# ltronchin/LatentAugment

Hardware: AMD Instinct MI355X
Metric: augmented images/sec (256^2, 20 latent steps) (higher is better)
Workload: dtype f32 (scaled split-fp16x2 on fp16 MFMA, fp32 accumulate); 1 GPU; SG2 config-f 256x256 2-ch, random-init G, batch=8/GPU, 20 latent steps; global_batch=8, parallelism=dp1

## Files before the change

### include/latentaug_hip.h

```cpp
#ifndef LATENTAUG_HIP_H
#define LATENTAUG_HIP_H

#include <stddef.h>

#ifdef __cplusplus
extern "C" {
#endif

#ifndef LA_STREAM_T
#define LA_STREAM_T
typedef struct ihipStream_t* la_stream_t;
#endif

#define LA_OK 0
#define LA_ERR_ARG (-1)
#define LA_ERR_HIP (-2)
#define LA_ERR_WORKSPACE (-3)

#define LA_ACT_LINEAR 1
#define LA_ACT_RELU 2
#define LA_ACT_LRELU 3

const char* la_last_error(void);
int la_abi_version(void);


int la_bias_act_f32(const float* x, const float* b, float* y, long n, long stepb, int nb, int act, float alpha,
                    float gain, float clamp, la_stream_t stream);

int la_bias_act_grad_f32(const float* dy, const float* yref, float* dx, float* db, long n, long stepb, int nb, int act,
                         float alpha, float gain, float clamp, la_stream_t stream);

int la_bias_act_ex_f32(const float* x, const float* b, const float* xref, const float* yref, const float* dy, float* out, long n,
                       long stepb, int nb, int grad, int act, float alpha, float gain, float clamp, la_stream_t stream);
int la_bias_sum_f32(const float* dx, float* db, long n, long stepb, int nb, la_stream_t stream);
int la_bias_act_ex_f16(const unsigned short* x, const unsigned short* b, const unsigned short* xref, const unsigned short* yref,
                       const unsigned short* dy, unsigned short* out, long n, long stepb, int nb, int grad, int act, float alpha, float gain,
                       float clamp, la_stream_t stream);
int la_bias_sum_f16(const unsigned short* dx, unsigned short* db, long n, long stepb, int nb, la_stream_t stream);
int la_bias_act_ex_f64(const double* x, const double* b, const double* xref, const double* yref, const double* dy, double* out, long n,
                       long stepb, int nb, int grad, int act, double alpha, double gain, double clamp, la_stream_t stream);
int la_bias_sum_f64(const double* dx, double* db, long n, long stepb, int nb, la_stream_t stream);

int la_upfirdn2d_out_size(int in_size, int up, int down, int pad0, int pad1, int taps);
int la_upfirdn2d_f32(const float* x, const float* f_host, float* y, int N, int C, int H, int W, int fh, int fw, int upx,
                     int upy, int downx, int downy, int padx0, int padx1, int pady0, int pady1, int flip, float gain,
                     la_stream_t stream);
int la_upfirdn2d_f16(const unsigned short* x, const float* f_host, unsigned short* y, int N, int C, int H, int W, int fh, int fw,
                     int upx, int upy, int downx, int downy, int padx0, int padx1, int pady0, int pady1, int flip, float gain,
                     la_stream_t stream);
int la_upfirdn2d_f64(const double* x, const float* f_host, double* y, int N, int C, int H, int W, int fh, int fw, int upx, int upy,
                     int downx, int downy, int padx0, int padx1, int pady0, int pady1, int flip, double gain, la_stream_t stream);

int la_filtered_lrelu_f32(const float* x, const float* fu, const float* fd, const float* b, const unsigned char* si, unsigned char* so,
                          float* y, int N, int C, int H, int W, int fu_h, int fu_w, int fd_h, int fd_w, int up, int down, int px0, int px1,
                          int py0, int py1, int sx, int sy, float gain, float slope, float clamp, int flip, int write_signs,
                          la_stream_t stream);
int la_filtered_lrelu_act_f32(float* x, const unsigned char* si, unsigned char* so, int N, int C, int H, int W, int sx, int sy, float gain,
                              float slope, float clamp, int write_signs, la_stream_t stream);
int la_filtered_lrelu_out_size(int in_size, int up, int down, int pad0, int pad1, int fu_taps, int fd_taps);
int la_filtered_lrelu_sign_shape(int H, int W, int fu_h, int fu_w, int fd_h, int fd_w, int up, int down, int px0, int px1, int py0, int py1,
                                 int* rows, int* row_bytes);


int la_conv2d_f32(const float* x, const float* w, float* y, void* ws, size_t ws_bytes, int B, int Cin, int H, int W, int Cout, int kh, int kw,
                  int Hout, int Wout, int stride, int pady, int padx, int groups, int flip_weight, int transpose, la_stream_t stream);
int la_conv2d_wgrad_f32(const float* x, const float* dy, float* dw, void* ws, size_t ws_bytes, int B, int Cin, int H, int W, int Cout,
                        int kh, int kw, int Hout, int Wout, int stride, int pady, int padx, int groups, int flip_weight, int transpose,
                        la_stream_t stream);
size_t la_conv2d_workspace_bytes(int op, int B, int Cin, int H, int W, int Cout, int kh, int kw, int Hout, int Wout, int stride, int groups,
                                 int transpose);
int la_conv2d_uses_engine(int op, int cout, int kh, int kw, int stride, int groups);
int la_conv2d_wgrad_slices(int B, int Cin, int H, int W, int Cout, int kh, int kw, int Hout, int Wout, int stride, int groups, int transpose);


int la_grid_sample_f32(const float* x, const float* grid, float* y, int N, int C, int H, int W, int Ho, int Wo, la_stream_t stream);
int la_grid_sample_f16(const unsigned short* x, const unsigned short* grid, unsigned short* y, int N, int C, int H, int W, int Ho, int Wo,
                       la_stream_t stream);
int la_grid_sample_f64(const double* x, const double* grid, double* y, int N, int C, int H, int W, int Ho, int Wo, la_stream_t stream);
int la_grid_sample_grad_f32(const float* dy, const float* x, const float* grid, float* dx, float* dgrid, int N, int C, int H, int W, int Ho,
                            int Wo, la_stream_t stream);
int la_grid_sample_grad_f16(const unsigned short* dy, const unsigned short* x, const unsigned short* grid, unsigned short* dx,
                            unsigned short* dgrid, float* ws, int N, int C, int H, int W, int Ho, int Wo, la_stream_t stream);
int la_grid_sample_grad_f64(const double* dy, const double* x, const double* grid, double* dx, double* dgrid, int N, int C, int H, int W,
                            int Ho, int Wo, la_stream_t stream);
long la_grid_sample_grad_workspace_floats(int N, int C, int H, int W);

int la_fma_f32(const float* a, const float* b, const float* c, float* y, const long* shape_host, const long* astride_host,
               const long* bstride_host, const long* cstride_host, la_stream_t stream);
int la_unbroadcast_sum_f32(const float* x, float* out, const long* shape_host, const long* out_shape_host, la_stream_t stream);


int la_pack_conv_weights_f32(const float* w, float* wf, float* wb, float* wsq, int cout, int cin, int ktaps,
                             la_stream_t stream);

int la_modconv3x3_fwd_f32(const float* x, long x_bstride, const float* wf, const void* wq, int precision, const float* s, int s_stride, const float* d,
                          int d_stride, const float* noise, long noise_bstride, float noise_strength, const float* bias,
                          int act, float alpha, float gain, float clamp, float* y, void* ws, size_t ws_bytes, int B, int cin, int cout, int res,
                          la_stream_t stream);

int la_modconv3x3_up2_fwd_f32(const float* x, long x_bstride, const float* wf, const void* wq, int precision, const float* s, int s_stride,
                              const float* d, int d_stride, const float* noise, long noise_bstride, float noise_strength,
                              const float* bias, int act, float alpha, float gain, float clamp, const float* fir_host,
                              float* scratch, float* y, void* ws, size_t ws_bytes, int B, int cin, int cout, int res, la_stream_t stream);

int la_modconv3x3_bwd_f32(const float* gz, const float* wb, const void* wq, int precision, const float* s, int s_stride, const float* xin,
                          long xin_bstride, float* gx, float* ds_part, void* ws, size_t ws_bytes, int B, int cin, int cout, int res,
                          la_stream_t stream);
int la_modconv3x3_up2_bwd_f32(const float* gz, const float* wb, const void* wq, int precision, const float* s, int s_stride, const float* xin,
                              long xin_bstride, const float* fir_host, float* scratch, float* gx, float* ds_part, void* ws, size_t ws_bytes, int B,
                              int cin, int cout, int res, la_stream_t stream);
int la_modconv_ds_tiles(int grid_res);
size_t la_modconv_workspace_bytes(int B, int cin, int cout, int res, int up);
#define LA_PREC_F32 0
#define LA_PREC_BF16X3 1
#define LA_PREC_BF16X2 2
#define LA_PREC_F16X2 3
size_t la_modconv_bf16_pack_bytes(int cin, int cout, int transpose, int nterm);
int la_pack_conv_weights_bf16_f32(const float* w, void* out, int cout, int cin, int ktaps, int transpose, int nterm,
                                  la_stream_t stream);


long la_pairwise_l2_workspace_floats(int n, long m);
int la_pairwise_l2_f32(const float* X, int n, const float* Y, long m, long K, float* D, float* mean_out,
                       float* workspace, la_stream_t stream);

int la_center_crop_f32(const float* src, float* dst, long planes, int R, int cc, int off, la_stream_t stream);

int la_adam_step_f32(float* p, const float* g, float* m, float* v, long n, int step, float lr, float beta1, float beta2,
                     float eps, la_stream_t stream);

int la_noise_normal_f32(float* out, long rows, long row_elems, unsigned long long seed, unsigned layer, long row0, la_stream_t stream);


int la_noise_uniform_f32(float* out, long rows, long row_elems, unsigned long long seed, unsigned stream_id, long row0, la_stream_t stream);

int la_elastic_field_f32(const float* noise, const float* taps_host, int ntaps, float alpha_x, float alpha_y, float* disp, float* ws, int B, int H,
                         int W, la_stream_t stream);

int la_warp_affine_f32(const float* x, const float* minv, const unsigned char* apply, float* y, int B, int C, int H, int W, int mode,
                       la_stream_t stream);

int la_warp_elastic_f32(const float* x, const float* disp, const unsigned char* apply, float* y, int B, int C, int H, int W, int mode,
                        la_stream_t stream);

typedef struct la_synth la_synth;
int la_synth_num_ws(int img_resolution);
int la_synth_num_params(int img_resolution);
size_t la_synth_workspace_bytes(int img_resolution, int img_channels, int w_dim, const int* channels, int max_batch);
int la_synth_create(int img_resolution, int img_channels, int w_dim, const int* channels, float conv_clamp,
                    const float* const* params, int nparams, const float* noise_strength_host, int nlayers,
                    const float* fir_host, int fir_h, int fir_w, int max_batch, void* workspace, size_t workspace_bytes,
                    la_stream_t stream, la_synth** out);
void la_synth_destroy(la_synth* h);
int la_synth_set_precision(la_synth* h, int precision);
int la_synth_set_operand_scale(la_synth* h, int from_data);
int la_synth_set_row_window(la_synth* h, int row_lo, int row_hi);
int la_synth_set_col_window(la_synth* h, int col_lo, int col_hi);
int la_synth_get_precision(const la_synth* h);
int la_synth_forward(la_synth* h, const float* ws, long ws_bstride, long ws_lstride, int B, int noise_mode,
                     const float* const* noises, float* img_out, la_stream_t stream);
int la_synth_backward(la_synth* h, const float* g_img, float* dws, la_stream_t stream);
const float* la_synth_image(const la_synth* h);
const float* la_synth_block_image(const la_synth* h, int block);
const float* la_synth_layer_output(const la_synth* h, int layer);
const float* la_synth_styles(const la_synth* h);
const float* la_synth_style_grads(const la_synth* h);
int la_synth_style_rows(const la_synth* h);

int la_fc_f32(const float* x, const float* W, const float* bias, float* y, int B, int in, int out, float lr_mul, int act,
              float alpha, float gain, la_stream_t stream);
int la_mapping_forward_f32(const float* z, int B, int z_dim, int w_dim, int num_layers, const float* const* weights,
                           const float* const* biases, float lr_mul, const float* w_avg, float truncation_psi,
                           int num_ws, float* tmp, float* ws_out, la_stream_t stream);

typedef struct la_disc la_disc;
int la_disc_num_params(int img_resolution);
size_t la_disc_workspace_bytes(int img_resolution, int img_channels, const int* channels, int max_batch);
int la_disc_create(int img_resolution, int img_channels, const int* channels, float conv_clamp, const float* const* params,
                   int nparams, const float* fir_host, int mbstd_group_size, int max_batch, void* workspace,
                   size_t workspace_bytes, la_stream_t stream, la_disc** out);
void la_disc_destroy(la_disc* h);
int la_disc_set_precision(la_disc* h, int precision);
int la_disc_forward(la_disc* h, const float* img, int B, la_stream_t stream);
int la_disc_loss(la_disc* h, float w_disc, int norm_batch, float* loss_out, la_stream_t stream);
int la_disc_backward(la_disc* h, const float* dlogits, float* g_img, int accumulate, la_stream_t stream);
const float* la_disc_logits(const la_disc* h);

#define LA_FEAT_CONV_RELU 0
#define LA_FEAT_TAP 1
#define LA_FEAT_MAXPOOL2 2
#define LA_FEAT_AVGPOOL2 3
#define LA_FEAT_FC_RELU 4
#define LA_FEAT_FC 5
typedef struct la_feat_op { int kind, cin, cout; } la_feat_op;
typedef struct la_feat la_feat;
size_t la_feat_workspace_bytes(int nops, const la_feat_op* ops, int in_ch, int in_res, int max_batch);
int la_feat_create(int nops, const la_feat_op* ops, const float* const* params, int nparams, int in_ch, int in_res,
                   int max_batch, void* workspace, size_t workspace_bytes, la_stream_t stream, la_feat** out);
void la_feat_destroy(la_feat* h);
int la_feat_num_features(const la_feat* h);
int la_feat_set_precision(la_feat* h, int precision);
int la_feat_forward(la_feat* h, const float* x, int N, float* feat_out, la_stream_t stream);
int la_feat_backward(la_feat* h, const float* gfeat, float* gx, la_stream_t stream);
int la_crop_repeat_f32(const float* img, float* xc, int B, int imgc, int R, int S, int y0, int x0, int rep, float scale,
                       float shift, la_stream_t stream);
int la_crop_repeat_grad_f32(const float* gxc, float* g_img, int B, int imgc, int R, int S, int y0, int x0, int rep,
                            float scale, la_stream_t stream);

#define LA_DET_AREA 0
#define LA_DET_BILINEAR 1
int la_detector_prep_f32(const float* img, float* out, int N, int C, int H, int W, int S, int rep, int mode, int quantize,
                         const float* scale, const float* shift, la_stream_t stream);
size_t la_fc_workspace_bytes(long N, long K, long O);
int la_fc_bias_act_f32(const float* x, const float* w, const float* b, float* y, long N, long K, long O, int act,
                       void* workspace, size_t workspace_bytes, la_stream_t stream);

typedef struct la_opt_config {
    int steps;
    float lr;
    float beta1, beta2, eps;
    float w_latent, w_pix, w_disc, w_lpips;
    int criterion_mode;
    int soft_aug;
    float alpha;
    int loop_noise_mode;
    int final_noise_mode;
    int norm_batch;
    int crop, crop_off;
} la_opt_config;
typedef struct la_latent_opt la_latent_opt;
size_t la_latent_opt_workspace_bytes(int img_resolution, int img_channels, int w_dim, const la_opt_config* cfg, long Mw,
                                     long Mx, int max_batch);
int la_latent_opt_create(la_synth* g, int img_resolution, int img_channels, int w_dim, const la_opt_config* cfg,
                         const float* bankW, long Mw, const float* bankXc, long Mx, int max_batch, void* workspace,
                         size_t workspace_bytes, la_latent_opt** out);
size_t la_latent_opt_workspace_bytes_ex(int img_resolution, int img_channels, int w_dim, const la_opt_config* cfg, long Mw,
                                        long Mx, int max_batch, int latent_space);
int la_latent_opt_create_ex(la_synth* g, int img_resolution, int img_channels, int w_dim, const la_opt_config* cfg,
                            const float* bankW, long Mw, const float* bankXc, long Mx, int max_batch, int latent_space,
                            void* workspace, size_t workspace_bytes, la_latent_opt** out);
void la_latent_opt_destroy(la_latent_opt* h);
int la_latent_opt_set_disc(la_latent_opt* h, la_disc* d);
size_t la_latent_opt_lpips_workspace_bytes(int img_channels, int F, int S, long Mf, int max_batch);
int la_latent_opt_set_lpips(la_latent_opt* h, la_feat* f, const float* bankF, long Mf, int S, float pre_scale,
                            float pre_shift, void* ws, size_t ws_bytes);
int la_latent_opt_set_lpips_preproc(la_latent_opt* h, const float* scale, const float* shift, int n);
int la_latent_opt_set_crop_pos(la_latent_opt* h, int x, int y);
int la_latent_opt_set_graph(la_latent_opt* h, int enable);
int la_latent_opt_graph_state(const la_latent_opt* h);
int la_latent_opt_set_trace(la_latent_opt* h, float* w_trace, float* img_trace);
int la_latent_opt_set_grad_trace(la_latent_opt* h, float* dw_trace);
int la_latent_opt_set_overlap(la_latent_opt* h, int enable);
int la_latent_opt_set_row_window(la_latent_opt* h, int row_lo, int row_hi);
int la_latent_opt_set_col_window(la_latent_opt* h, int col_lo, int col_hi);
int la_latent_opt_set_time_trace(la_latent_opt* h, int enable);
int la_latent_opt_get_times(la_latent_opt* h, float* ms);
int la_latent_opt_invalidate_banks(la_latent_opt* h);
int la_latent_opt_run(la_latent_opt* h, const float* w0, int B, const float* const* final_noises, float* img_out,
                      float* w_aug_out, float* losses_out, la_stream_t stream);

int la_feature_moments_f64(const float* x, long n, int D, double* raw_mean, double* raw_cov, la_stream_t stream);
size_t la_pr_workspace_floats(long nr, long nc);
int la_cdist_f16(const void* rows, long nr, const void* cols, long nc, int D, float* dist, float* ws, la_stream_t stream);
int la_pr_kth_f16(const void* rows, long nr, const void* cols, long nc, int D, int nhood_size, float* kth, float* ws,
                  la_stream_t stream);
int la_pr_member_f16(const void* rows, long nr, const void* cols, long nc, int D, const float* radius, unsigned char* member,
                     float* ws, la_stream_t stream);

size_t la_kid_workspace_bytes(long S, long mx, long my);
int la_kid_poly3_f32(const float* x, long nx, const float* y, long ny, int D, const int* ix, const int* iy, long S, long mx, long my,
                     double* sums, double* mmd2, double* kid, void* ws, size_t ws_bytes, la_stream_t stream);

size_t la_dc_workspace_bytes(long ng, long nr);
int la_dc_col_splits(long ng, long nr);
int la_dc_count_f16(const void* gen, long ng, const void* real, long nr, int D, const float* radius, int* count, float* nearest,
                    void* ws, size_t ws_bytes, la_stream_t stream);

int la_prof_begin(void);
int la_prof_end(double* total_ms, long* launches, double* flops, double* bytes);
int la_prof_set_stride(int stride);
long la_prof_total_launches(void);
int la_prof_num_classes(void);
int la_prof_end_classes(double* ms, long* launches, double* flops, double* bytes, int nclass);

#ifdef __cplusplus
}
#endif
#endif
```

### latentaugment_amd/csrc/la_conv.h

```cpp
#pragma once
#include <stddef.h>
#include <string.h>

#include "la_common.h"
#include "la_launch_args.h"

#define LA_EPI_RAW 0
#define LA_EPI_FWD 1
#define LA_EPI_BWD 2
#define LA_CONV_MAX_TAPS 9
#define LA_CONV_MAX_PHASES 4
#define LA_CONV_PHASE_TAPS 4

struct LaRgbFuse {
    int imgc;
    const float* w; const float* s; int s_stride; const float* bias; const float* skip;
    float* rgb_pre; float* img; float clamp;
};
struct LaSeamFuse {
    const float* demod; int demod_stride;
    const float* bias;
    const float* noise; long noise_bstride; float noise_strength;
    int act; float alpha, gain, clamp;
    float* ddn_part;
    float* pmax;
    float* xs_out;
    float xs_mult;
    int imgc;
    const float* g_img; const float* rgb_pre; float rgb_clamp;
    const float* wrgb; const float* s_rgb; int s_rgb_stride;
    float* dweff_part;
};

struct LaConvArgs {
    const float* in;
    const float* wgt;
    float* out;
    const float* in_scale;
    long in_bstride;
    int scale_stride;
    const float* in_mask_y;
    int in_mask_act; float in_mask_alpha, in_mask_gain, in_mask_clamp;
    float in_gain;
    int B, C, M, Hin, Win, Hout, Wout;
    int Gy, Gx;
    int in_sy, in_sx;
    int out_sy, out_sx, out_oy, out_ox;
    int out_pitch; long out_plane;
    int ntaps;
    int tap_dy[LA_CONV_MAX_TAPS], tap_dx[LA_CONV_MAX_TAPS], tap_w[LA_CONV_MAX_TAPS];
    int epi;
    const float* demod;
    int demod_stride;
    const float* noise;
    long noise_bstride;
    float noise_strength;
    const float* bias;
    int act;
    float alpha, gain, clamp;
    const float* addend;
    float* out2;
    float* fwd_xs_out;
    const float* fwd_xs_mult;
    const float* out_scale;
    int oscale_stride;
    const float* xin;
    long xin_bstride;
    float* ds_part;
    int tiles_per_sample;
    LaSeamFuse seam;
    LaRgbFuse rgb;
    void* ws;
    size_t ws_bytes;
    float* splitk_ws;
    int ksplit;
    const float* in_pmax;
    int in_pmax_nseg;
    const void* in_q;
    int precision;
    const void* wgt_bf16;
    long wgt_bf16_term_elems;
    const float* acc_scale_x;
    int acc_scale_fan;
    const float* acc_scale_w;
    int row_lo, row_hi;
    int col_lo, col_hi;
    int in_row_lo, in_row_hi;
#ifdef LA_DEV
    int dbg_stamp;
#endif
    int nphase;
    struct Phase {
        int Gy, Gx, out_oy, out_ox, ntaps; int tap_dy[LA_CONV_PHASE_TAPS], tap_dx[LA_CONV_PHASE_TAPS], tap_w[LA_CONV_PHASE_TAPS];
        int tile0;
        long ws_off;
    } ph[LA_CONV_MAX_PHASES];
};
static_assert(sizeof(LaConvArgs) == 1096 && offsetof(LaConvArgs, seam) == 416 && offsetof(LaConvArgs, rgb) == 568 && offsetof(LaConvArgs, ws) == 640,
              "LaConvArgs: an embedded record moved a kernel-parameter field");

static inline void la_conv_args_init(LaConvArgs& a) {
    memset(&a, 0, sizeof(a));
    a.in_sy = a.in_sx = a.out_sy = a.out_sx = 1;
    a.clamp = -1.f; a.gain = 1.f; a.act = LA_ACT_LINEAR;
}
static inline void la_conv_taps_kxk(LaConvArgs& a, int k, bool backward) {
    a.ntaps = k * k;
    for (int t = 0; t < a.ntaps; ++t) {
        const int dy = t / k - k / 2, dx = t % k - k / 2;
        a.tap_dy[t] = backward ? -dy : dy; a.tap_dx[t] = backward ? -dx : dx; a.tap_w[t] = t;
    }
}
static inline void la_conv_taps_3x3(LaConvArgs& a, bool backward) { la_conv_taps_kxk(a, 3, backward); }
static inline void la_conv_taps_3x3_corner(LaConvArgs& a) {
    a.ntaps = 9;
    for (int t = 0; t < 9; ++t) { a.tap_dy[t] = t / 3; a.tap_dx[t] = t % 3; a.tap_w[t] = t; }
}
static inline void la_conv_up2_phase(LaConvArgs& a, int hin, int py, int px, int ox_step, bool merged) {
    a.out_oy = py; a.out_ox = px * ox_step;
    a.Gy = py ? hin : hin + 1; a.Gx = px ? hin : hin + 1;
    int nt = 0;
    for (int ky = py; ky < 3; ky += 2)
        for (int kx = px; kx < 3; kx += 2) { a.tap_dy[nt] = -(ky / 2); a.tap_dx[nt] = -(kx / 2); a.tap_w[nt] = ky * 3 + kx; ++nt; }
    a.ntaps = nt;
    if (!merged) return;
    LaConvArgs::Phase& P = a.ph[a.nphase++];
    P.Gy = a.Gy; P.Gx = a.Gx; P.out_oy = py; P.out_ox = a.out_ox; P.ntaps = nt;
    for (int t = 0; t < nt; ++t) { P.tap_dy[t] = a.tap_dy[t]; P.tap_dx[t] = a.tap_dx[t]; P.tap_w[t] = a.tap_w[t]; }
}

int la_conv_flat_launch(const LaConvArgs& as, int MTsel, dim3 grid, bool split, hipStream_t stream);
int la_conv_halo_launch(const LaConvArgs& as, int MTsel, dim3 grid, hipStream_t stream);

long la_conv_bf16_pack_elems(int M, int C, int ktaps);
int la_pack_conv_weights_bf16(const float* w, void* out, int cout, int cin, int ktaps, int transpose, int nterm,
                              hipStream_t stream, float scale = 1.f, int m_pad = 0);
int la_conv_bf16_dispatch(const LaConvArgs& as, int MTsel, dim3 grid, bool split, hipStream_t stream);

long la_conv_splitk_floats(int B, int M, int C, int Gy, int Gx, int precision);
long la_conv_splitk_floats_phases(int B, int M, int C, int nphase, const int* Gy, const int* Gx, int precision);
size_t la_conv_presplit_bytes(int B, int C, int Hin, int Win);
size_t la_conv_split_pack_bytes(int M, int C, int ktaps);
int la_conv_prepare_input(LaConvArgs& a, hipStream_t stream);
int la_conv_act_grad_segments(long HW);
int la_conv_act_grad_pmax(const float* dy, const float* yref, float* dx, float* pm, int B, int C, long HW, int act, float alpha, float gain,
                          float clamp, hipStream_t stream);
int la_conv_xscale_from_pmax(const float* pmax, int nseg, const float* scale, int scale_stride, float mult, float* xscale, int B, int C,
                             hipStream_t stream);
int la_absmax_bits(const float* w, long n, unsigned* amax_bits, hipStream_t stream);
bool la_conv_bf16_uses_halo(const LaConvArgs& a);

int la_conv_tiles_per_sample(int Gy, int Gx);
int la_conv_launch(const LaConvArgs& a, hipStream_t stream);
```

### latentaugment_amd/csrc/la_conv.hip

```cpp
#include "la_conv.h"
#include <stdlib.h>
#include "la_conv_device.h"
#include <type_traits>

#define KC 16

int la_conv_tiles_per_sample(int Gy, int Gx) { return la_cdiv((long)Gy * Gx, NT); }

#define SPLITK_MAX_G 1156
static int choose_ksplit(bool bf, long tiles, int nck, float taps, double out_bytes) {
    int ks;
    if (bf) {
        float best = 1e30f;
        ks = 1;
        for (int k = 1; k <= nck && k <= 16; ++k) {
            const int per = la_cdiv(nck, k);
            const int kk = la_cdiv(nck, per);
            if (kk != k) continue;
            const float slots = (float)(tiles * kk) / 512.f;
            const float rounds = slots <= 1.f ? 1.f : slots;
            float cost = rounds * ((float)per * taps * 1.7f + 10.f);
            if (kk > 1) cost += 5.f + (float)((kk + 1) * out_bytes / 3.5e6);
            if (cost < best - 1e-3f) { best = cost; ks = kk; }
        }
        return ks;
    }
    ks = la_cdiv(768, tiles);
    if (ks > nck) ks = nck;
    if (ks < 2) return 1;
    const int per = la_cdiv(nck, ks);
    return la_cdiv(nck, per);
}

long la_conv_splitk_floats_phases(int B, int M, int C, int nphase, const int* Gy, const int* Gx, int precision) {
    const bool bf = precision != LA_PREC_F32;
    const int nck = la_cdiv(C, bf ? 32 : KC);
    if (nck < 2 || nphase < 1 || (nphase > 1 && !bf)) return 0;
    const int mtiles = la_cdiv(M, M >= 128 ? 128 : 64);
    long tiles = 0, Gsum = 0;
    for (int p = 0; p < nphase; ++p) {
        const long G = (long)Gy[p] * Gx[p];
        if (G > SPLITK_MAX_G) return 0;
        tiles += la_cdiv((long)B * G, NT);
        Gsum += G;
    }
    int ks = choose_ksplit(bf, tiles * mtiles, nck, nphase > 1 ? 2.25f : 9.f, 4.0 * B * M * (double)Gsum);
    const int ks1 = choose_ksplit(bf, tiles * mtiles, nck, 1.f, 4.0 * B * M * (double)Gsum);
    if (ks1 > ks) ks = ks1;
    return ks >= 2 ? (long)ks * B * M * Gsum : 0;
}
long la_conv_splitk_floats(int B, int M, int C, int Gy, int Gx, int precision) {
    return la_conv_splitk_floats_phases(B, M, C, 1, &Gy, &Gx, precision);
}

template <int MT, bool SPLIT>
__global__ __launch_bounds__(256) void la_conv_igemm_kernel(LaConvArgs a) {
    constexpr int TM = MT / 64;
    constexpr int A_F4 = (KC * MT / 4) / 256;
    __shared__ __attribute__((aligned(16))) float As[2][KC][MT];
    __shared__ __attribute__((aligned(16))) float Bs[2][KC][NT];
    __shared__ float red[4][MT];

    const int tid = threadIdx.x;
    const int lane = tid & 63, wid = tid >> 6;
    const int wm = wid >> 1, wn = wid & 1;
    int ntile = blockIdx.x;
    if (!SPLIT && (gridDim.x & 7) == 0) ntile = (blockIdx.x & 7) * (gridDim.x >> 3) + (blockIdx.x >> 3);
    const int m0 = blockIdx.y * MT;
    const int G = a.Gy * a.Gx;
    const int Ntot = SPLIT ? a.B * G : G;

    const int n_l = tid & (NT - 1);
    const int khalf = tid >> 7;
    const int nidx_l = ntile * NT + n_l;
    const bool nvalid = nidx_l < Ntot;
    int b_l = SPLIT ? (nvalid ? nidx_l / G : 0) : (int)blockIdx.z;
    const int g_l = SPLIT ? nidx_l - b_l * G : nidx_l;
    const int gy_l = nvalid ? g_l / a.Gx : 0;
    const int gx_l = nvalid ? g_l - gy_l * a.Gx : 0;
    const int iy0 = gy_l * a.in_sy, ix0 = gx_l * a.in_sx;
    const long HWin = (long)a.Hin * a.Win;
    const float* in_b = a.in + (long)b_l * a.in_bstride;
    const float* sc_b = a.in_scale ? a.in_scale + (long)b_l * a.scale_stride : nullptr;

    const int nck = (a.C + KC - 1) / KC;
    int ck_beg = 0, ck_end = nck;
    if (SPLIT) {
        const int per = (nck + a.ksplit - 1) / a.ksplit;
        ck_beg = blockIdx.z * per;
        ck_end = ck_beg + per < nck ? ck_beg + per : nck;
    }
    const int ci_beg = ck_beg * a.ntaps, ci_end = ck_end * a.ntaps;

    float breg[KC / 2];
    float4 areg[A_F4];

    auto prefetch = [&](int ci) {
        const int cc = ci / a.ntaps;
        const int t = ci - cc * a.ntaps;
        const int c0 = cc * KC;
        const int iy = iy0 + a.tap_dy[t], ix = ix0 + a.tap_dx[t];
        const bool ok = nvalid && iy >= 0 && iy < a.Hin && ix >= 0 && ix < a.Win;
        const long off = (long)iy * a.Win + ix;
#pragma unroll
        for (int j = 0; j < KC / 2; ++j) {
            const int c = c0 + khalf + 2 * j;
            float v = 0.f;
            if (ok && c < a.C) {
                v = in_b[(long)c * HWin + off];
                if (sc_b) v *= sc_b[c];
            }
            breg[j] = v;
        }
        const float* wslab = a.wgt + (long)a.tap_w[t] * a.C * a.M;
#pragma unroll
        for (int j = 0; j < A_F4; ++j) {
            const int idx = tid + 256 * j;
            const int row = idx / (MT / 4), col = (idx - row * (MT / 4)) * 4;
            const int c = c0 + row, m = m0 + col;
            float4 v = make_float4(0.f, 0.f, 0.f, 0.f);
            if (c < a.C && m < a.M) v = *reinterpret_cast<const float4*>(wslab + (long)c * a.M + m);
            areg[j] = v;
        }
    };
    auto stage = [&](int buf) {
#pragma unroll
        for (int j = 0; j < KC / 2; ++j) Bs[buf][khalf + 2 * j][n_l] = breg[j];
#pragma unroll
        for (int j = 0; j < A_F4; ++j) {
            const int idx = tid + 256 * j;
            const int row = idx / (MT / 4), col = (idx - row * (MT / 4)) * 4;
            *reinterpret_cast<float4*>(&As[buf][row][col]) = areg[j];
        }
    };

    f32x16 acc[TM][2];
#pragma unroll
    for (int i = 0; i < TM; ++i)
#pragma unroll
        for (int j = 0; j < 2; ++j)
#pragma unroll
            for (int r = 0; r < 16; ++r) acc[i][j][r] = 0.f;

    const int l31 = lane & 31, lh = lane >> 5;
    if (ci_beg < ci_end) {
        prefetch(ci_beg);
        stage(0);
    }
    __syncthreads();
    for (int ci = ci_beg; ci < ci_end; ++ci) {
        const int buf = (ci - ci_beg) & 1;
        if (ci + 1 < ci_end) prefetch(ci + 1);
#pragma unroll
        for (int kp = 0; kp < KC / 2; ++kp) {
            float av[TM], bv[2];
#pragma unroll
            for (int i = 0; i < TM; ++i) av[i] = As[buf][2 * kp + lh][wm * (MT / 2) + i * 32 + l31];
#pragma unroll
            for (int j = 0; j < 2; ++j) bv[j] = Bs[buf][2 * kp + lh][wn * 64 + j * 32 + l31];
#pragma unroll
            for (int i = 0; i < TM; ++i)
#pragma unroll
                for (int j = 0; j < 2; ++j)
                    acc[i][j] = __builtin_amdgcn_mfma_f32_32x32x2f32(av[i], bv[j], acc[i][j], 0, 0, 0);
        }
        if (ci + 1 < ci_end) stage(buf ^ 1);
        __syncthreads();
    }

    la_conv_epilogue<MT, SPLIT>(a, acc, red, ntile, m0, G, Ntot);
}

template <int PPB>
__global__ __launch_bounds__(256) void la_conv_splitk_finish_kernel(LaConvArgs a_in) {
    __shared__ float wpart[4];
    LaConvArgs a = a_in;
    if (a_in.nphase > 0) {
        const LaConvArgs::Phase& P = a_in.ph[blockIdx.z];
        a.Gy = P.Gy; a.Gx = P.Gx; a.out_oy = P.out_oy; a.out_ox = P.out_ox;
        a.splitk_ws = a_in.splitk_ws + P.ws_off;
    }
    constexpr int T = 256 / PPB;
    const int lane = threadIdx.x & 63;
    const int tp = threadIdx.x % T;
    const int m = blockIdx.x * PPB + threadIdx.x / T;
    const int b = blockIdx.y;
    const bool live = m < a.M;
    if (!live && PPB > 1) return;
    const int G = a.Gy * a.Gx;
    const int wpitch = (a.epi == LA_EPI_RAW && a.out_pitch > 0) ? a.out_pitch : a.Wout;
    const long HWout = (a.epi == LA_EPI_RAW && a.out_plane > 0) ? a.out_plane : (long)a.Hout * a.Wout;
    const long slice = (long)a.B * a.M * G;
    const float* wsp = a.splitk_ws + ((long)b * a.M + m) * G;
    float* out_p = a.out + ((long)b * a.M + m) * HWout;
    const float dmv = (a.epi == LA_EPI_FWD && a.demod) ? a.demod[(long)b * a.demod_stride + m] : 1.f;
    const float bv = (a.epi == LA_EPI_FWD && a.bias) ? a.bias[m] : 0.f;
    const float sc = (a.epi == LA_EPI_BWD && a.out_scale) ? a.out_scale[(long)b * a.oscale_stride + m] : 1.f;
    const float* xin_p = (a.epi == LA_EPI_BWD && a.xin) ? a.xin + (long)b * a.xin_bstride + (long)m * HWout : nullptr;
    const bool seam = a.epi == LA_EPI_BWD && a.seam.ddn_part != nullptr && xin_p != nullptr;
    const float dm0 = (seam && a.seam.demod) ? a.seam.demod[(long)b * a.seam.demod_stride + m] : 1.f;
    const float b0 = (seam && a.seam.bias) ? a.seam.bias[m] : 0.f;
    float part = 0.f, dd = 0.f, mx = 0.f;
    float* xs_row = (seam && a.seam.xs_out && lane == 0 && (PPB > 1 || threadIdx.x == 0)) ? a.seam.xs_out + (long)b * LA_XS_FAN + la_xs_sub((int)(threadIdx.x >> 6) * 5) : nullptr;
    float ymax = 0.f;
    if (a.epi == LA_EPI_FWD && a.fwd_xs_out && lane == 0) xs_row = a.fwd_xs_out + (long)b * LA_XS_FAN + la_xs_sub((int)(threadIdx.x >> 6) * 5);
    const float xs_seen = xs_row ? la_xs_peek(xs_row) : 0.f;
    const int imgc = seam ? (a.seam.imgc < 4 ? a.seam.imgc : 4) : 0;
    float we[4] = {0.f, 0.f, 0.f, 0.f}, dwe[4] = {0.f, 0.f, 0.f, 0.f};
    for (int c = 0; c < imgc; ++c) we[c] = a.seam.wrgb[(long)c * a.M + m] * a.seam.s_rgb[(long)b * a.seam.s_rgb_stride + m];
    auto run = [&](auto vec_tag) {
        constexpr int VEC = decltype(vec_tag)::value;
        typedef float vf __attribute__((ext_vector_type(VEC)));
        auto ld = [](const float* p) { return *reinterpret_cast<const vf*>(p); };
        for (int g = tp * VEC; g < G; g += T * VEC) {
            auto add = [](vf& s, const vf& p) {
#pragma unroll
                for (int e = 0; e < VEC; ++e) s[e] += p[e];
            };
            vf acc = ld(wsp + g);
            int k = 1;
            for (; k + 7 < a.ksplit; k += 8) {
                vf p[8];
#pragma unroll
                for (int u = 0; u < 8; ++u) p[u] = ld(wsp + (long)(k + u) * slice + g);
#pragma unroll
                for (int u = 0; u < 8; ++u) add(acc, p[u]);
            }
            if (k + 3 < a.ksplit) {
                vf p[4];
#pragma unroll
                for (int u = 0; u < 4; ++u) p[u] = ld(wsp + (long)(k + u) * slice + g);
#pragma unroll
                for (int u = 0; u < 4; ++u) add(acc, p[u]);
                k += 4;
            }
            for (; k < a.ksplit; ++k) { const vf p = ld(wsp + (long)k * slice + g); add(acc, p); }
            const int gy = g / a.Gx, gx = g - gy * a.Gx;
            const long pos = (long)(gy * a.out_sy + a.out_oy) * wpitch + gx * a.out_sx + a.out_ox;
            float v[VEC];
#pragma unroll
            for (int e = 0; e < VEC; ++e) v[e] = VEC == 1 ? acc[0] : acc[e];
            if (a.epi == LA_EPI_FWD) {
                vf nz = 0.f;
                if (a.noise) nz = ld(a.noise + (long)b * a.noise_bstride + pos);
#pragma unroll
                for (int e = 0; e < VEC; ++e) v[e] = la_conv_epi_fwd(a, v[e], dmv, nz[e] * a.noise_strength, bv);
                if (a.out2) {
                    const long o2 = ((long)b * a.M + m) * HWout + pos;
                    vf ad = 0.f;
                    if (a.addend) ad = ld(a.addend + o2);
                    vf w;
#pragma unroll
                    for (int e = 0; e < VEC; ++e) { w[e] = v[e] + ad[e]; ymax = fmaxf(ymax, fabsf(w[e])); }
                    *reinterpret_cast<vf*>(a.out2 + o2) = w;
                } else {
#pragma unroll
                    for (int e = 0; e < VEC; ++e) ymax = fmaxf(ymax, fabsf(v[e]));
                }
            } else if (a.epi == LA_EPI_BWD) {
                vf y = 0.f;
                if (xin_p) y = ld(xin_p + pos);
                vf gv[4], nz0 = 0.f;
#pragma unroll
                for (int c = 0; c < 4; ++c) {
                    gv[c] = 0.f;
                    if (c < imgc) {
                        const long o = ((long)b * imgc + c) * HWout + pos;
                        gv[c] = ld(a.seam.g_img + o);
                        if (a.seam.rgb_clamp >= 0.f) {
                            const vf pre = ld(a.seam.rgb_pre + o);
#pragma unroll
                            for (int e = 0; e < VEC; ++e) if (fabsf(pre[e]) > a.seam.rgb_clamp) gv[c][e] = 0.f;
                        }
                    }
                }
                if (seam && a.seam.noise) {
                    nz0 = ld(a.seam.noise + (long)b * a.seam.noise_bstride + pos);
#pragma unroll
                    for (int e = 0; e < VEC; ++e) nz0[e] *= a.seam.noise_strength;
                }
#pragma unroll
                for (int e = 0; e < VEC; ++e) {
                    part += v[e] * y[e];
                    v[e] *= sc;
#pragma unroll
                    for (int c = 0; c < 4; ++c)
                        if (c < imgc) { v[e] += we[c] * gv[c][e]; dwe[c] += gv[c][e] * y[e]; }
                    if (seam) {
                        const float g1 = v[e] * la_act_bwd_from_y(y[e], a.seam.act, a.seam.alpha, a.seam.gain, a.seam.clamp);
                        dd += g1 * (la_act_inv(y[e], a.seam.act, a.seam.alpha, a.seam.gain) - b0 - nz0[e]);
                        v[e] = g1 * dm0;
                        mx = fmaxf(mx, fabsf(v[e]));
                    }
                }
            }
            vf w;
#pragma unroll
            for (int e = 0; e < VEC; ++e) w[e] = v[e];
            *reinterpret_cast<vf*>(out_p + pos) = w;
        }
    };
    {
        size_t al = (size_t)a.splitk_ws | (size_t)a.out | (size_t)a.out2 | (size_t)a.addend | (size_t)a.noise | (size_t)a.xin;
        if (seam) al |= (size_t)a.seam.noise | (size_t)(imgc ? a.seam.g_img : nullptr) | (size_t)(imgc ? a.seam.rgb_pre : nullptr);
        const bool vec4 = a.out_sx == 1 && ((a.Gx | wpitch | a.out_ox) & 3) == 0 && ((HWout | a.noise_bstride | a.seam.noise_bstride | a.xin_bstride) & 3) == 0 &&
                          (al & 15) == 0 && (a_in.nphase == 0 || (a_in.ph[blockIdx.z].ws_off & 3) == 0);
        if (vec4) run(std::integral_constant<int, 4>{});
        else run(std::integral_constant<int, 1>{});
    }
    if (a.epi == LA_EPI_FWD && a.fwd_xs_out) {
#pragma unroll
        for (int o = 32; o > 0; o >>= 1) ymax = fmaxf(ymax, __shfl_xor(ymax, o, 64));
// ... 175 lines not shown
```

### latentaugment_amd/csrc/la_latent_opt.hip

```cpp
#include "la_common.h"

#include <math.h>
#include <stdlib.h>
#include <string.h>

#include "la_conv.h"
#include "la_criteria.h"
#include "la_feat.h"

struct la_latent_opt {
    la_synth* g;
    la_disc* d;
    la_opt_config cfg;
    int R, imgc, wdim, num_ws, maxB;
    int wplus;
    const float* bankW; long Mw;
    const float* bankX; long Mx;
    float *w_opt, *m, *v, *dw, *dws, *g_img, *colsumW, *colsumX, *yx, *yy, *xx, *xc, *losses;
    int colsums_valid;
    la_feat* f;
    const float* bankF; long Mf; int F, S, crop_x, crop_y;
    float pre_scale[4], pre_shift[4];
    float *l_xc, *l_feat, *l_gfeat, *l_gxc, *l_colsum, *l_yx, *l_yy, *l_xx;
    int l_colsum_valid;
    float* adam_tab;
    float* adam_tab_host;
    int adam_tab_valid;
    int* step_ctr;
    int* crop_dev;
    float* trace_dw;
    int graph_mode;
    int graph_B;
    int graph_win;
    int graph_refused;
    hipGraph_t graph;
    hipGraphExec_t graph_exec;
    hipGraph_t seg_graph[4];
    hipGraphExec_t seg_exec[4];
    int seg_valid;
    hipStream_t cap_stream;
    float* trace_w;
    float* trace_img;
    int wcol_lo, wcol_hi;
    int win_lo, win_hi;
    int overlap;
    hipStream_t side_stream;
    hipEvent_t ev_fork, ev_join;
    int time_trace, tev_steps;
    hipEvent_t* tev;
};
#define LA_TEV 7

static size_t carve(la_latent_opt* h, char* base) {
    LaCarver c{base};
    const size_t B = h->maxB, wd = h->wdim, cc2 = (size_t)h->cfg.crop * h->cfg.crop;
    const size_t wl = h->wplus ? (size_t)h->num_ws * wd : wd;
    h->w_opt = c.take(B * wl); h->m = c.take(B * wl); h->v = c.take(B * wl); h->dw = c.take(B * wl);
    h->dws = c.take(B * h->num_ws * wd);
    h->g_img = c.take(B * h->imgc * (size_t)h->R * h->R);
    h->colsumW = c.take((size_t)h->num_ws * wd);
    h->colsumX = c.take((size_t)h->imgc * cc2);
    const size_t mm = (size_t)(h->Mw > h->Mx ? h->Mw : h->Mx);
    h->yx = c.take(LA_YX_FLOATS(mm ? mm : 1, B)); h->yy = c.take(LA_YY_FLOATS(mm ? mm : 1)); h->xx = c.take(LA_XX_FLOATS(B));
    h->xc = c.take(B * h->imgc * cc2);
    h->losses = c.take((size_t)(h->cfg.steps > 0 ? h->cfg.steps : 1) * 4);
    h->adam_tab = c.take((size_t)(h->cfg.steps > 0 ? h->cfg.steps : 1) * 2);
    h->step_ctr = reinterpret_cast<int*>(c.take(16));
    h->crop_dev = h->step_ctr + 4;
    return c.off;
}

static size_t carve_lpips(la_latent_opt* h, char* base) {
    LaCarver c{base};
    const size_t n = (size_t)h->imgc * h->maxB;
    h->l_xc = c.take(n * 3 * h->S * h->S); h->l_gxc = c.take(n * 3 * h->S * h->S);
    h->l_feat = c.take(n * h->F); h->l_gfeat = c.take(n * h->F);
    h->l_colsum = c.take((size_t)h->imgc * h->F);
    h->l_yx = c.take(LA_YX_FLOATS(h->Mf, h->maxB)); h->l_yy = c.take(LA_YY_FLOATS(h->Mf)); h->l_xx = c.take(LA_XX_FLOATS(h->maxB));
    return c.off;
}

extern "C" size_t la_latent_opt_workspace_bytes_ex(int img_resolution, int img_channels, int w_dim, const la_opt_config* cfg,
                                                   long Mw, long Mx, int max_batch, int latent_space) {
    if (!cfg || (latent_space != 0 && latent_space != 1)) return 0;
    la_latent_opt h; memset(&h, 0, sizeof(h));
    h.cfg = *cfg; h.R = img_resolution; h.imgc = img_channels; h.wdim = w_dim; h.num_ws = la_synth_num_ws(img_resolution);
    h.maxB = max_batch; h.Mw = Mw; h.Mx = Mx; h.wplus = latent_space;
    return carve(&h, nullptr);
}

extern "C" size_t la_latent_opt_workspace_bytes(int img_resolution, int img_channels, int w_dim, const la_opt_config* cfg,
                                                long Mw, long Mx, int max_batch) {
    return la_latent_opt_workspace_bytes_ex(img_resolution, img_channels, w_dim, cfg, Mw, Mx, max_batch, 0);
}

extern "C" int la_latent_opt_create(la_synth* g, int img_resolution, int img_channels, int w_dim, const la_opt_config* cfg,
                                    const float* bankW, long Mw, const float* bankXc, long Mx, int max_batch,
                                    void* workspace, size_t workspace_bytes, la_latent_opt** out) {
    return la_latent_opt_create_ex(g, img_resolution, img_channels, w_dim, cfg, bankW, Mw, bankXc, Mx, max_batch, 0, workspace,
                                   workspace_bytes, out);
}

extern "C" int la_latent_opt_create_ex(la_synth* g, int img_resolution, int img_channels, int w_dim, const la_opt_config* cfg,
                                       const float* bankW, long Mw, const float* bankXc, long Mx, int max_batch, int latent_space,
                                       void* workspace, size_t workspace_bytes, la_latent_opt** out) {
    LA_CHECK_ARG(latent_space == 0 || latent_space == 1, "latent_opt_create: latent_space must be 0 (W) or 1 (W+)");
    LA_CHECK_ARG(latent_space == 0 || w_dim % 4 == 0, "latent_opt_create: W+ needs w_dim % 4 == 0");
    LA_CHECK_ARG(g && cfg && workspace && out, "latent_opt_create: null pointer");
    LA_CHECK_ARG(cfg->steps >= 0, "latent_opt_create: negative step count");
    LA_CHECK_ARG(cfg->w_latent == 0.f || (bankW && Mw >= 1), "latent_opt_create: w_latent > 0 needs the latent bank W");
    LA_CHECK_ARG(cfg->w_pix == 0.f || (bankXc && Mx >= 1), "latent_opt_create: w_pix > 0 needs the cropped image bank X");
    LA_CHECK_ARG(cfg->crop >= 1 && cfg->crop_off >= 0 && cfg->crop + cfg->crop_off <= img_resolution,
                 "latent_opt_create: centre crop does not fit the image");
    LA_CHECK_ARG(cfg->criterion_mode == 0 || cfg->criterion_mode == 1, "latent_opt_create: criterion_mode must be 0 or 1");
    la_latent_opt* h = (la_latent_opt*)malloc(sizeof(la_latent_opt));
    LA_CHECK_ARG(h, "latent_opt_create: out of host memory");
    memset(h, 0, sizeof(*h));
    h->g = g; h->cfg = *cfg; h->R = img_resolution; h->imgc = img_channels; h->wdim = w_dim;
    h->num_ws = la_synth_num_ws(img_resolution); h->maxB = max_batch; h->wplus = latent_space;
    h->bankW = bankW; h->Mw = cfg->w_latent != 0.f ? Mw : 0; h->bankX = bankXc; h->Mx = cfg->w_pix != 0.f ? Mx : 0;
    const size_t need = carve(h, (char*)workspace);
    if (need > workspace_bytes) { free(h); la_set_error("latent_opt_create: workspace too small"); return LA_ERR_WORKSPACE; }
    h->adam_tab_host = (float*)malloc(sizeof(float) * 2 * (size_t)(cfg->steps > 0 ? cfg->steps : 1));
    if (!h->adam_tab_host) { free(h); la_set_error("latent_opt_create: out of host memory"); return LA_ERR_ARG; }
    la_adam_fill_table(h->adam_tab_host, cfg->steps, cfg->beta1, cfg->beta2);
    h->graph_mode = 1;
    h->overlap = 2;
    h->win_lo = h->win_hi = 0; h->wcol_lo = h->wcol_hi = 0;
    *out = h;
    return LA_OK;
}

static void drop_graph(la_latent_opt* h) {
    if (h->graph_exec) { (void)hipGraphExecDestroy(h->graph_exec); h->graph_exec = nullptr; }
    if (h->graph) { (void)hipGraphDestroy(h->graph); h->graph = nullptr; }
    for (int k = 0; k < 4; ++k) {
        if (h->seg_exec[k]) { (void)hipGraphExecDestroy(h->seg_exec[k]); h->seg_exec[k] = nullptr; }
        if (h->seg_graph[k]) { (void)hipGraphDestroy(h->seg_graph[k]); h->seg_graph[k] = nullptr; }
    }
    h->seg_valid = 0;
    h->graph_B = 0; h->graph_win = 0;
}

extern "C" void la_latent_opt_destroy(la_latent_opt* h) {
    if (!h) return;
    drop_graph(h);
    if (h->tev) { for (int i = 0; i < h->tev_steps * LA_TEV; ++i) (void)hipEventDestroy(h->tev[i]); free(h->tev); }
    if (h->ev_fork) (void)hipEventDestroy(h->ev_fork);
    if (h->ev_join) (void)hipEventDestroy(h->ev_join);
    if (h->side_stream) (void)hipStreamDestroy(h->side_stream);
    if (h->cap_stream) (void)hipStreamDestroy(h->cap_stream);
    free(h->adam_tab_host);
    free(h);
}

extern "C" int la_latent_opt_set_overlap(la_latent_opt* h, int enable) {
    LA_CHECK_ARG(h, "latent_opt_set_overlap: null handle");
    const int mode = enable < 0 ? 0 : (enable > 2 ? 2 : enable);
    h->overlap = mode;
    drop_graph(h);
    return LA_OK;
}

extern "C" int la_latent_opt_set_row_window(la_latent_opt* h, int row_lo, int row_hi) {
    LA_CHECK_ARG(h && row_lo >= 0 && (row_hi == 0 ? row_lo == 0 : (row_hi > row_lo && row_hi <= h->R)), "latent_opt_set_row_window: bad window");
    if (row_lo != h->win_lo || row_hi != h->win_hi) drop_graph(h);
    h->win_lo = row_lo; h->win_hi = row_hi;
    return LA_OK;
}

extern "C" int la_latent_opt_set_col_window(la_latent_opt* h, int col_lo, int col_hi) {
    LA_CHECK_ARG(h && col_lo >= 0 && (col_hi == 0 ? col_lo == 0 : (col_hi > col_lo && col_hi <= h->R)), "latent_opt_set_col_window: bad window");
    if (col_lo != h->wcol_lo || col_hi != h->wcol_hi) drop_graph(h);
    h->wcol_lo = col_lo; h->wcol_hi = col_hi;
    return LA_OK;
}

extern "C" int la_latent_opt_set_trace(la_latent_opt* h, float* w_trace, float* img_trace) {
    LA_CHECK_ARG(h, "latent_opt_set_trace: null handle");
    h->trace_w = w_trace; h->trace_img = img_trace;
    return LA_OK;
}

extern "C" int la_latent_opt_set_time_trace(la_latent_opt* h, int enable) {
    LA_CHECK_ARG(h, "latent_opt_set_time_trace: null handle");
    if (enable && !h->tev && h->cfg.steps > 0) {
        h->tev = (hipEvent_t*)malloc(sizeof(hipEvent_t) * (size_t)h->cfg.steps * LA_TEV);
        LA_CHECK_ARG(h->tev, "latent_opt_set_time_trace: out of host memory");
        for (int i = 0; i < h->cfg.steps * LA_TEV; ++i) LA_HIP(hipEventCreate(&h->tev[i]));
        h->tev_steps = h->cfg.steps;
    }
    h->time_trace = enable ? 1 : 0;
    return LA_OK;
}

extern "C" int la_latent_opt_get_times(la_latent_opt* h, float* ms) {
    LA_CHECK_ARG(h && ms && h->tev, "latent_opt_get_times: no time trace recorded");
    for (int s = 0; s < h->tev_steps; ++s) {
        hipEvent_t* e = h->tev + (size_t)s * LA_TEV;
        LA_HIP(hipEventSynchronize(e[LA_TEV - 1]));
        float t[LA_TEV - 1];
        for (int k = 0; k + 1 < LA_TEV; ++k) LA_HIP(hipEventElapsedTime(&t[k], e[k], e[k + 1]));
        float* o = ms + (size_t)s * 5;
        o[0] = t[1]; o[2] = t[2]; o[1] = t[3]; o[3] = t[4];
        LA_HIP(hipEventElapsedTime(&o[4], e[0], e[LA_TEV - 1]));
    }
    return LA_OK;
}

extern "C" int la_latent_opt_set_grad_trace(la_latent_opt* h, float* dw_trace) {
    LA_CHECK_ARG(h, "latent_opt_set_grad_trace: null handle");
    h->trace_dw = dw_trace;
    return LA_OK;
}

extern "C" int la_latent_opt_invalidate_banks(la_latent_opt* h) {
    LA_CHECK_ARG(h, "latent_opt_invalidate_banks: null handle");
    h->colsums_valid = 0;
    h->l_colsum_valid = 0;
    return LA_OK;
}

extern "C" int la_latent_opt_graph_state(const la_latent_opt* h) {
    if (!h) return 0;
    return (h->graph_exec || h->seg_valid) ? 1 : (h->graph_refused ? -1 : 0);
}

extern "C" int la_latent_opt_set_graph(la_latent_opt* h, int enable) {
    LA_CHECK_ARG(h, "latent_opt_set_graph: null handle");
    h->graph_mode = enable ? 1 : 0;
    h->graph_refused = 0;
    if (!enable) drop_graph(h);
    return LA_OK;
}

extern "C" int la_latent_opt_set_disc(la_latent_opt* h, la_disc* d) {
    LA_CHECK_ARG(h, "latent_opt_set_disc: null handle");
    h->d = d;
    drop_graph(h);
    return LA_OK;
}

extern "C" size_t la_latent_opt_lpips_workspace_bytes(int img_channels, int F, int S, long Mf, int max_batch) {
    la_latent_opt h; memset(&h, 0, sizeof(h));
    h.imgc = img_channels; h.F = F; h.S = S; h.Mf = Mf; h.maxB = max_batch;
    return carve_lpips(&h, nullptr);
}

extern "C" int la_latent_opt_set_lpips(la_latent_opt* h, la_feat* f, const float* bankF, long Mf, int S, float pre_scale,
                                       float pre_shift, void* ws, size_t ws_bytes) {
    LA_CHECK_ARG(h && f && bankF && Mf >= 1 && S >= 1 && ws, "latent_opt_set_lpips: bad arguments");
    const int F = la_feat_num_features(f);
    LA_CHECK_ARG(ws_bytes >= la_latent_opt_lpips_workspace_bytes(h->imgc, F, S, Mf, h->maxB), "latent_opt_set_lpips: workspace too small");
    h->f = f; h->bankF = bankF; h->Mf = Mf; h->F = F; h->S = S; for (int k = 0; k < 4; ++k) { h->pre_scale[k] = pre_scale; h->pre_shift[k] = pre_shift; }
    carve_lpips(h, (char*)ws);
    h->l_colsum_valid = 0;
    drop_graph(h);
    return LA_OK;
}

extern "C" int la_latent_opt_set_lpips_preproc(la_latent_opt* h, const float* scale, const float* shift, int n) {
    LA_CHECK_ARG(h && scale && shift && n >= 1 && n <= 4, "latent_opt_set_lpips_preproc: bad arguments");
    for (int k = 0; k < 4; ++k) { h->pre_scale[k] = scale[k < n ? k : n - 1]; h->pre_shift[k] = shift[k < n ? k : n - 1]; }
    drop_graph(h);
    return LA_OK;
}

extern "C" int la_latent_opt_set_crop_pos(la_latent_opt* h, int x, int y) {
    LA_CHECK_ARG(h && x >= 0 && y >= 0, "latent_opt_set_crop_pos: bad arguments");
    h->crop_x = x; h->crop_y = y;
    return LA_OK;
}

__global__ void la_lpips_gfeat_kernel(const float* __restrict__ feat, const float* __restrict__ colsum, float* __restrict__ g, int B,
                                      int F, float coef2, float mrows, long total) {
    const long i = (long)blockIdx.x * blockDim.x + threadIdx.x;
    if (i >= total) return;
    const long n = i / F; const int k = (int)(i - n * F);
    const int c = (int)(n / B);
    g[i] = coef2 * (mrows * feat[i] - colsum[(long)c * F + k]);
}

__global__ void la_set_int2_kernel(int* __restrict__ dst, int a, int b) { dst[0] = a; dst[1] = b; }

static int refresh_colsums(la_latent_opt* h, hipStream_t stream) {
    int rc;
    const long cc2 = (long)h->cfg.crop * h->cfg.crop;
    if (h->Mw && (rc = la_bank_colsum(h->bankW, h->Mw, (long)h->num_ws * h->wdim, h->colsumW, stream))) return rc;
    if (h->Mx)
        for (int c = 0; c < h->imgc; ++c)
            if ((rc = la_bank_colsum(h->bankX + (long)c * h->Mx * cc2, h->Mx, cc2, h->colsumX + (long)c * cc2, stream)))
                return rc;
    return LA_OK;
}

extern "C" int la_latent_opt_run(la_latent_opt* h, const float* w0, int B, const float* const* final_noises,
                                 float* img_out, float* w_aug_out, float* losses_out, hipStream_t stream) {
    LA_CHECK_ARG(h && w0 && img_out && w_aug_out, "latent_opt_run: null pointer");
    LA_CHECK_ARG(B >= 1 && B <= h->maxB, "latent_opt_run: batch exceeds max_batch");
    const la_opt_config& c = h->cfg;
    LA_CHECK_ARG(c.final_noise_mode != 2 || final_noises, "latent_opt_run: explicit final noise requested but not given");
    const int wd = h->wdim, cc = c.crop, off = c.crop_off;
    const long cc2 = (long)cc * cc;
    const long nw = (long)B * wd * (h->wplus ? h->num_ws : 1);
    const float nb = (float)(c.norm_batch > 0 ? c.norm_batch : B);
    int rc;
    LA_HIP(hipMemcpyAsync(h->w_opt, w0, nw * sizeof(float), hipMemcpyDeviceToDevice, stream));
    LA_HIP(hipMemsetAsync(h->m, 0, nw * sizeof(float), stream));
    LA_HIP(hipMemsetAsync(h->v, 0, nw * sizeof(float), stream));
    LA_HIP(hipMemsetAsync(h->step_ctr, 0, 16 * sizeof(int), stream));
    if (c.steps > 0 && !h->adam_tab_valid) {
        LA_HIP(hipMemcpyAsync(h->adam_tab, h->adam_tab_host, sizeof(float) * 2 * (size_t)c.steps, hipMemcpyHostToDevice, stream));
        LA_HIP(hipStreamSynchronize(stream));
        h->adam_tab_valid = 1;
    }
    hipLaunchKernelGGL(la_set_int2_kernel, dim3(1), dim3(1), 0, stream, h->crop_dev, h->crop_y, h->crop_x);
    const bool use_disc = c.w_disc != 0.f;
    LA_CHECK_ARG(!use_disc || h->d, "latent_opt_run: w_disc != 0 but no discriminator attached (la_latent_opt_set_disc)");
    const bool use_lpips = c.w_lpips != 0.f;
    LA_CHECK_ARG(!use_lpips || h->f, "latent_opt_run: w_lpips != 0 but no feature engine attached (la_latent_opt_set_lpips)");
    if (use_disc && use_lpips && h->overlap && !h->side_stream) {
        LA_HIP(hipStreamCreateWithFlags(&h->side_stream, hipStreamNonBlocking));
        LA_HIP(hipEventCreateWithFlags(&h->ev_fork, hipEventDisableTiming));
        LA_HIP(hipEventCreateWithFlags(&h->ev_join, hipEventDisableTiming));
    }
    LA_CHECK_ARG(!use_lpips || (h->crop_x + h->S <= h->R && h->crop_y + h->S <= h->R), "latent_opt_run: LPIPS crop outside the image");
    const bool img_crit = c.w_pix != 0.f || use_disc || use_lpips;
    const float lp_coef = use_lpips ? c.w_lpips / ((float)h->imgc * (float)h->Mf * nb) : 0.f;
    const bool want_losses = losses_out != nullptr;
    if (!h->colsums_valid) {
        if ((rc = refresh_colsums(h, stream))) return rc;
        h->colsums_valid = 1;
    }
    if (use_lpips && !h->l_colsum_valid) {
        for (int ch = 0; ch < h->imgc; ++ch)
            if ((rc = la_bank_colsum(h->bankF + (long)ch * h->Mf * h->F, h->Mf, h->F, h->l_colsum + (long)ch * h->F, stream))) return rc;
        h->l_colsum_valid = 1;
    }
    auto inside = [&](int y0, int y1, int x0, int x1) {
        return y0 >= h->win_lo && y1 <= h->win_hi && (h->wcol_hi <= 0 || (x0 >= h->wcol_lo && x1 <= h->wcol_hi));
    };
    const bool win_covers = (c.w_pix == 0.f || inside(off, off + cc, off, off + cc)) &&
                            (!use_lpips || inside(h->crop_y, h->crop_y + h->S, h->crop_x, h->crop_x + h->S));
    const bool windowed = h->win_hi > 0 && !use_disc && !h->trace_img && win_covers;
    struct WinGuard {
        la_synth* g; ~WinGuard() { (void)la_synth_set_row_window(g, 0, 0); (void)la_synth_set_col_window(g, 0, 0); }
    } win_guard{h->g};
    if ((rc = la_synth_set_row_window(h->g, windowed ? h->win_lo : 0, windowed ? h->win_hi : 0))) return rc;
    if ((rc = la_synth_set_col_window(h->g, windowed ? h->wcol_lo : 0, windowed ? h->wcol_hi : 0))) return rc;
    if (want_losses && c.steps > 0) LA_HIP(hipMemsetAsync(h->losses, 0, (size_t)c.steps * 4 * sizeof(float), stream));
    const float lat_coef = h->Mw ? c.w_latent / ((float)h->Mw * nb * (float)h->num_ws * (float)wd) : 0.f;
    const float pix_coef = h->Mx ? c.w_pix / ((float)h->imgc * (float)h->Mx * nb * (float)cc2) : 0.f;

    auto run_step = [&](float* L, hipStream_t st, int step_index = -1, int seg = 15) -> int {
        int rc;
        const bool segA = seg & 1, segP = seg & 2, segD = seg & 4, segZ = seg & 8;
        hipEvent_t* tev = (h->time_trace && h->tev && L && step_index >= 0 && step_index < h->tev_steps) ? h->tev + (size_t)step_index * LA_TEV : nullptr;
        auto mark = [&](int k) { if (tev) (void)hipEventRecord(tev[k], st); };
        const float* img = la_synth_image(h->g);
        if (segA) {
            mark(0);
            const long wb = h->wplus ? (long)h->num_ws * wd : wd, wl = h->wplus ? wd : 0;
            if ((rc = la_synth_forward(h->g, h->w_opt, wb, wl, B, c.loop_noise_mode, nullptr, nullptr, st))) return rc;
            img = la_synth_image(h->g);
            mark(1);
            if (L) {
                if (h->Mw && (rc = la_l2_mean_from_bank(h->bankW, h->Mw, (long)h->num_ws * wd, h->w_opt, B, wb, h->wplus ? 0 : wd, h->yx,
                                                        h->yy, h->xx, lat_coef, L + 0, 0, st)))
                    return rc;
            }
            mark(2);
            if (L) {
                if (h->Mx) {
                    if ((rc = la_center_crop_f32(img, h->xc, (long)B * h->imgc, h->R, cc, off, st))) return rc;
                    for (int ch = 0; ch < h->imgc; ++ch)
                        if ((rc = la_l2_mean_from_bank(h->bankX + (long)ch * h->Mx * cc2, h->Mx, cc2, h->xc + (long)ch * cc2, B,
                                                       (long)h->imgc * cc2, 0, h->yx, h->yy, h->xx, pix_coef, L + 1, ch > 0, st)))
                            return rc;
                }
            }
        }
        const float* dws = nullptr;
        if (img_crit) {
            if (segA) {
                if (c.w_pix != 0.f &&
                    (rc = la_pix_grad(img, h->colsumX, h->g_img, B, h->imgc, h->R, cc, off, -2.f * pix_coef, (float)h->Mx, st)))
                    return rc;
                mark(3);
            }
            const bool fork = seg == 15 && h->overlap == 2 && use_disc && use_lpips && !L && !tev && !la_prof_enabled() && h->side_stream && h->ev_fork && h->ev_join;
            hipStream_t sl = fork ? h->side_stream : st;
            if (fork) {
                LA_HIP(hipEventRecord(h->ev_fork, st));
                LA_HIP(hipStreamWaitEvent(h->side_stream, h->ev_fork, 0));
            }
            if (use_disc && segD) {
                if ((rc = la_disc_forward(h->d, img, B, st))) return rc;
                if ((rc = la_disc_loss(h->d, c.w_disc, c.norm_batch, L ? L + 2 : nullptr, st))) return rc;
                if ((rc = la_disc_backward(h->d, nullptr, h->g_img, c.w_pix != 0.f, st))) return rc;
            }
            if (segD) mark(4);
            if (use_lpips) {
                const int N = h->imgc * B;
                const long FF = h->F;
                if (segP) {
                    if (c.w_pix == 0.f && !use_disc) LA_HIP(hipMemsetAsync(h->g_img, 0, sizeof(float) * (size_t)B * h->imgc * h->R * h->R, st));
                    if ((rc = la_crop_repeat(img, h->l_xc, B, h->imgc, h->R, h->S, h->crop_y, h->crop_x, h->crop_dev, 3, h->pre_scale, h->pre_shift, sl))) return rc;
                    if ((rc = la_feat_forward(h->f, h->l_xc, N, h->l_feat, sl))) return rc;
                    if (L) {
                        for (int ch = 0; ch < h->imgc; ++ch)
                            if ((rc = la_l2_mean_from_bank(h->bankF + (long)ch * h->Mf * FF, h->Mf, FF, h->l_feat + (long)ch * B * FF, B, FF, 0,
                                                           h->l_yx, h->l_yy, h->l_xx, lp_coef, L + 3, ch > 0, st)))
                                return rc;
                    }
                    const long total = (long)N * FF;
                    hipLaunchKernelGGL(la_lpips_gfeat_kernel, dim3(la_cdiv(total, 256)), dim3(256), 0, sl, h->l_feat, h->l_colsum, h->l_gfeat,
                                       B, (int)FF, -2.f * lp_coef, (float)h->Mf, total);
                    if ((rc = la_feat_backward(h->f, h->l_gfeat, h->l_gxc, sl))) return rc;
                }
                if (fork) {
                    LA_HIP(hipEventRecord(h->ev_join, h->side_stream));
                    LA_HIP(hipStreamWaitEvent(st, h->ev_join, 0));
                }
                if (segZ && (rc = la_crop_repeat_grad(h->l_gxc, h->g_img, B, h->imgc, h->R, h->S, h->crop_y, h->crop_x, h->crop_dev, 3, h->pre_scale, st)))
                    return rc;
            }
            if (segZ) {
                mark(5);
                if ((rc = la_synth_backward(h->g, h->g_img, h->dws, st))) return rc;
            }
            dws = h->dws;
        } else if (segZ) { mark(3); mark(4); mark(5); }
        if (!segZ) return LA_OK;
        if (h->wplus)
            rc = la_wplus_step_tail(dws, h->Mw ? h->colsumW : nullptr, h->dw, h->w_opt, h->m, h->v, B, h->num_ws, wd, -2.f * lat_coef,
                                    (float)h->Mw, c.lr, c.beta1, c.beta2, c.eps, h->adam_tab, h->step_ctr, h->step_ctr + 8, st);
        else
            rc = la_step_tail(dws, h->Mw ? h->colsumW : nullptr, h->dw, h->w_opt, h->m, h->v, B, h->num_ws, wd, -2.f * lat_coef, (float)h->Mw,
                              c.lr, c.beta1, c.beta2, c.eps, h->adam_tab, h->step_ctr, h->step_ctr + 8, st);
        mark(6);
        return rc;
    };

    const bool tracing = h->trace_w || h->trace_img || h->trace_dw;
    const bool replay = h->graph_mode == 1 && !want_losses && !tracing && c.steps > 0 && !la_prof_enabled();
    int first_graph_step = 1;
    const bool split = replay && h->overlap == 1 && use_disc && use_lpips && h->side_stream && h->ev_fork && h->ev_join;
    auto capture = [&](int seg, hipGraph_t* g, hipGraphExec_t* e) -> bool {
        bool ok = hipStreamBeginCapture(h->cap_stream, hipStreamCaptureModeRelaxed) == hipSuccess;
        if (ok) {
            const int rcs = run_step(nullptr, h->cap_stream, -1, seg);
            const hipError_t er = hipStreamEndCapture(h->cap_stream, g);
            ok = rcs == LA_OK && er == hipSuccess && *g;
        }
        if (ok) ok = hipGraphInstantiate(e, *g, nullptr, nullptr, 0) == hipSuccess;
        return ok;
    };
    const bool have = split ? (h->seg_valid != 0) : (h->graph_exec != nullptr);
    if (replay && (!have || h->graph_B != B || h->graph_win != (int)windowed)) {
        drop_graph(h);
        if ((rc = run_step(nullptr, stream))) return rc;
        first_graph_step = 2;
        bool ok = c.steps >= 2;
        if (ok && !h->cap_stream) ok = hipStreamCreateWithFlags(&h->cap_stream, hipStreamNonBlocking) == hipSuccess;
        if (ok && split) {
            for (int k = 0; k < 4 && ok; ++k) ok = capture(1 << k, &h->seg_graph[k], &h->seg_exec[k]);
            if (ok) h->seg_valid = 1;
        } else if (ok) ok = capture(15, &h->graph, &h->graph_exec);
        if (ok) { h->graph_B = B; h->graph_win = (int)windowed; }
        else { drop_graph(h); (void)hipGetLastError(); if (c.steps >= 2) { h->graph_mode = 0; h->graph_refused = 1; } }
    }
    for (int step = first_graph_step; step <= c.steps; ++step) {
        if (replay && split && h->seg_valid && h->graph_B == B) {
            LA_HIP(hipGraphLaunch(h->seg_exec[0], stream));
            LA_HIP(hipEventRecord(h->ev_fork, stream));
            LA_HIP(hipStreamWaitEvent(h->side_stream, h->ev_fork, 0));
            LA_HIP(hipGraphLaunch(h->seg_exec[1], h->side_stream));
            LA_HIP(hipEventRecord(h->ev_join, h->side_stream));
            LA_HIP(hipGraphLaunch(h->seg_exec[2], stream));
            LA_HIP(hipStreamWaitEvent(stream, h->ev_join, 0));
            LA_HIP(hipGraphLaunch(h->seg_exec[3], stream));
        } else if (replay && !split && h->graph_exec && h->graph_B == B) LA_HIP(hipGraphLaunch(h->graph_exec, stream));
        else {
            if ((rc = run_step(want_losses ? h->losses + (size_t)(step - 1) * 4 : nullptr, stream, step - 1))) return rc;
            if (h->trace_img)
                LA_HIP(hipMemcpyAsync(h->trace_img + (size_t)(step - 1) * B * h->imgc * h->R * h->R, la_synth_image(h->g),
                                      sizeof(float) * (size_t)B * h->imgc * h->R * h->R, hipMemcpyDeviceToDevice, stream));
            if (h->trace_w) LA_HIP(hipMemcpyAsync(h->trace_w + (size_t)(step - 1) * nw, h->w_opt, sizeof(float) * nw, hipMemcpyDeviceToDevice, stream));
            if (h->trace_dw) LA_HIP(hipMemcpyAsync(h->trace_dw + (size_t)(step - 1) * nw, h->dw, sizeof(float) * nw, hipMemcpyDeviceToDevice, stream));
        }
    }
    if ((rc = h->wplus ? la_wplus_gate(h->w_opt, w0, w_aug_out, B, h->num_ws, wd, c.alpha, c.soft_aug, stream)
                       : la_broadcast_mix(h->w_opt, w0, w_aug_out, B, h->num_ws, wd, c.alpha, c.soft_aug, stream)))
        return rc;
    if ((rc = la_synth_set_row_window(h->g, 0, 0)) || (rc = la_synth_set_col_window(h->g, 0, 0))) return rc;
    if ((rc = la_synth_forward(h->g, w_aug_out, (long)h->num_ws * wd, wd, B, c.final_noise_mode, final_noises, img_out, stream)))
        return rc;
    if (losses_out && c.steps > 0)
        LA_HIP(hipMemcpyAsync(losses_out, h->losses, (size_t)c.steps * 4 * sizeof(float), hipMemcpyDeviceToDevice, stream));
    return LA_OK;
}
```

### latentaugment_amd/csrc/la_synth.hip

```cpp
#include "la_common.h"

#include <math.h>
#include <stdlib.h>
#include <string.h>

#include "la_conv.h"
#include "la_modconv.h"
#include "la_style.h"
#include "la_upfirdn2d.h"

#define MAX_BLOCKS 12

struct ConvLayer {
    int cin, cout, res, up, widx;
    const float *affine_w, *affine_b, *weight, *bias, *noise_const;
    float noise_strength;
    float *wf, *wb, *wsq;
    void *wqf, *wqb;
    float* y;
    float *dsp, *ddnp;
    int s_off, d_off, style_idx;
    const float* noise_used;
    long noise_bstride;
};

struct RgbLayer {
    int cin, res, widx;
    const float *affine_w, *affine_b, *weight, *bias;
    int s_off, style_idx;
    float *rgb_pre, *img, *g_img;
    float* dwep;
};

struct la_synth {
    int R, imgc, wdim, nblocks, num_ws, maxB;
    int channels[MAX_BLOCKS];
    float clamp;
    const float* cst;
    int nconv;
    ConvLayer conv[2 * MAX_BLOCKS];
    RgbLayer rgb[MAX_BLOCKS];
    float fir[16];
    LaStyleTable st;
    LaDemodTable dt;
    int S, Dt;
    float *s_all, *d_all, *ds_all;
    float *zT, *G0, *G1, *aff_part;
    void* cws;
    size_t cws_bytes;
    float* pmax;
    float* pmax3;
    float* pmax2;
    float* xs_fwd;
    float* xs_bwd;
    float* xs_mult;
    int lastB;
    int precision;
    float* final_img;
    int win_lo, win_hi;
    int wcol_lo, wcol_hi;
    int fw_c0, fw_c1;
    int fw_lo[2 * MAX_BLOCKS], fw_hi[2 * MAX_BLOCKS];
};

static LaLayerEpi layer_epi(const la_synth* h, const ConvLayer& L) {
    return LaLayerEpi{h->d_all + L.d_off, h->Dt, L.noise_used, L.noise_bstride, L.noise_strength, L.bias, LA_ACT_LRELU, 0.2f, sqrtf(2.f), h->clamp};
}
static LaModconv layer_conv(const la_synth* h, const ConvLayer& L, int B, bool backward) {
    return LaModconv{backward ? L.wb : L.wf, backward ? L.wqb : L.wqf, h->precision, h->s_all + L.s_off, h->S, B, L.cin, L.cout, L.res, h->cws, h->cws_bytes};
}
static LaRgbFuse layer_rgb(const la_synth* h, const RgbLayer& T, const float* skip, float* img) {
    return LaRgbFuse{h->imgc, T.weight, h->s_all + T.s_off, h->S, T.bias, skip, T.rgb_pre, img, h->clamp};
}

static inline int zt_xhalf(int res) { return (res / 2 + 1 + 3) & ~3; }
static int layout(la_synth* h, void* workspace, size_t cap, size_t* need) {
    LaCarver c{(char*)workspace, 0, cap};
    const size_t mb = h->maxB;
    size_t gmax = 0, ztmax = 0, dsp = 0, ddn = 0, dwe = 0;
    size_t skf = 0;
    for (int k = 0; k < h->nconv; ++k) {
        ConvLayer& L = h->conv[k];
        const size_t wn = (size_t)L.cin * L.cout;
        L.wf = c.take(9 * wn); L.wb = c.take(9 * wn); L.wsq = c.take(wn);
        L.wqf = c.take((la_modconv_bf16_pack_bytes(L.cin, L.cout, 0, 3) + 3) / 4);
        L.wqb = c.take((la_modconv_bf16_pack_bytes(L.cin, L.cout, 1, 3) + 3) / 4);
        const size_t hw = (size_t)L.res * L.res;
        L.y = c.take(mb * L.cout * hw);
        if (mb * L.cout * hw > gmax) gmax = mb * L.cout * hw;
        if (mb * L.cin * hw > gmax && !L.up) gmax = mb * L.cin * hw;
        if (L.up) {
            const size_t z = mb * L.cout * (size_t)(L.res + 1) * (size_t)(2 * zt_xhalf(L.res));
            if (z > ztmax) ztmax = z;
        }
        const int gin = L.up ? L.res / 2 : L.res;
        {
            const size_t sl0 = (size_t)la_seam_slabs((long)hw), t1 = (size_t)la_conv_tiles_per_sample(L.res, L.res);
            L.dsp = c.take(mb * L.cin * (size_t)la_conv_tiles_per_sample(gin, gin));
            L.ddnp = c.take(mb * L.cout * (sl0 > t1 ? sl0 : t1));
        }
        const size_t t = mb * L.cin * (size_t)la_conv_tiles_per_sample(gin, gin);
        if (t > dsp) dsp = t;
        const size_t sl = mb * L.cout * (size_t)la_seam_slabs((long)hw);
        if (sl > ddn) ddn = sl;
        const size_t sk = la_modconv_workspace_bytes((int)mb, L.cin, L.cout, L.res, L.up);
        if (sk > skf) skf = sk;
    }
    for (int k = 0; k < h->nblocks; ++k) {
        RgbLayer& T = h->rgb[k];
        const size_t hw = (size_t)T.res * T.res;
        T.rgb_pre = c.take(mb * h->imgc * hw);
        T.img = c.take(mb * h->imgc * hw);
        T.g_img = c.take(mb * h->imgc * hw);
        {
            const size_t sl0 = (size_t)la_seam_slabs((long)hw), t1 = (size_t)la_conv_tiles_per_sample(T.res, T.res);
            T.dwep = c.take(mb * h->imgc * T.cin * (sl0 > t1 ? sl0 : t1));
        }
        const size_t sl = mb * h->imgc * T.cin * (size_t)la_seam_slabs((long)hw);
        if (sl > dwe) dwe = sl;
    }
    h->s_all = c.take(mb * h->S);
    h->ds_all = c.take(mb * h->S);
    h->d_all = c.take(mb * h->Dt);
    h->zT = c.take(ztmax);
    h->G0 = c.take(gmax);
    h->G1 = c.take(gmax);
    h->aff_part = c.take((size_t)la_affine_bwd_chunks(h->st) * mb * h->wdim);
    h->cws = c.take((skf + 3) / 4);
    h->cws_bytes = skf;
    {
        size_t pmx = 0;
        for (int k = 0; k < h->nconv; ++k) {
            const ConvLayer& L = h->conv[k];
            const size_t a = (size_t)L.cout * (L.up ? la_fir4x4_segments(L.res, L.res) : 1), b2 = (size_t)L.cout * la_seam_slabs((long)L.res * L.res);
            if (a > pmx) pmx = a;
            if (b2 > pmx) pmx = b2;
        }
        h->pmax = c.take(mb * pmx);
    }
    {
        size_t f2 = 0;
        for (int k = 0; k < h->nconv; ++k) {
            const ConvLayer& L = h->conv[k];
            if (L.up) { const size_t n = mb * L.cout * (size_t)la_conv_tiles_per_sample(L.res, L.res); if (n > f2) f2 = n; }
        }
        h->pmax2 = c.take(f2 ? f2 : 16);
        size_t f3 = 0;
        for (int k = 0; k < h->nconv; ++k) {
            const ConvLayer& L = h->conv[k];
            if (!L.up) { const size_t n = mb * L.cout * (size_t)la_conv_tiles_per_sample(L.res, L.res); if (n > f3) f3 = n; }
        }
        h->pmax3 = c.take(f3 ? f3 : 16);
    }
    h->xs_fwd = c.take((size_t)h->nconv * mb * LA_XS_FAN);
    h->xs_bwd = c.take((size_t)h->nconv * mb * LA_XS_FAN);
    h->xs_mult = c.take((size_t)h->nconv * mb + 16);
    *need = c.off;
    return LA_OK;
}

static int describe(la_synth* h, int R, int imgc, int wdim, const int* channels, int maxB) {
    LA_CHECK_ARG(R >= 4 && (R & (R - 1)) == 0 && R <= 4096, "synth: resolution must be a power of two >= 4");
    LA_CHECK_ARG(imgc >= 1 && imgc <= 4, "synth: img_channels must be 1..4");
    LA_CHECK_ARG(wdim >= 1 && maxB >= 1, "synth: bad w_dim / batch");
    memset(h, 0, sizeof(*h));
    h->R = R; h->imgc = imgc; h->wdim = wdim; h->maxB = maxB;
    int nb = 0;
    for (int r = 4; r <= R; r *= 2) ++nb;
    LA_CHECK_ARG(nb <= MAX_BLOCKS, "synth: too many blocks");
    h->nblocks = nb;
    int nconv = 0, widx = 0, S = 0, Dt = 0, nst = 0;
    for (int k = 0; k < nb; ++k) {
        const int res = 4 << k;
        const int co = channels[k];
        LA_CHECK_ARG(co >= 4 && co % 4 == 0, "synth: channel counts must be multiples of 4");
        h->channels[k] = co;
        if (k > 0) {
            ConvLayer& L = h->conv[nconv++];
            L.cin = channels[k - 1]; L.cout = co; L.res = res; L.up = 1; L.widx = widx++;
        }
        ConvLayer& L1 = h->conv[nconv++];
        L1.cin = co; L1.cout = co; L1.res = res; L1.up = 0; L1.widx = widx++;
        RgbLayer& T = h->rgb[k];
        T.cin = co; T.res = res; T.widx = widx;
    }
    h->nconv = nconv;
    h->num_ws = widx + 1;
    LA_CHECK_ARG(nconv + nb <= LA_MAX_STYLE_LAYERS, "synth: too many style layers");
    for (int k = 0; k < nconv; ++k) {
        ConvLayer& L = h->conv[k];
        L.s_off = S; L.d_off = Dt; L.style_idx = nst;
        h->st.row_start[nst] = S; h->st.widx[nst] = L.widx; h->st.post_gain[nst] = 1.f;
        h->dt.row_start[k] = Dt; h->dt.cin[k] = L.cin; h->dt.s_off[k] = S;
        S += L.cin; Dt += L.cout; ++nst;
    }
    for (int k = 0; k < nb; ++k) {
        RgbLayer& T = h->rgb[k];
        T.s_off = S; T.style_idx = nst;
        h->st.row_start[nst] = S; h->st.widx[nst] = T.widx; h->st.post_gain[nst] = 1.f / sqrtf((float)T.cin);
        S += T.cin; ++nst;
    }
    h->st.nlayers = nst; h->st.total_rows = S; h->st.row_start[nst] = S;
    h->dt.nlayers = nconv; h->dt.total_rows = Dt; h->dt.row_start[nconv] = Dt;
    h->S = S; h->Dt = Dt;
    return LA_OK;
}

extern "C" int la_synth_num_ws(int img_resolution) {
    int nb = 0;
    for (int r = 4; r <= img_resolution; r *= 2) ++nb;
    return 2 * nb;
}

extern "C" int la_synth_num_params(int img_resolution) {
    int nb = 0;
    for (int r = 4; r <= img_resolution; r *= 2) ++nb;
    return 1 + 5 + 4 + (nb - 1) * 14;
}

extern "C" size_t la_synth_workspace_bytes(int img_resolution, int img_channels, int w_dim, const int* channels,
                                           int max_batch) {
    la_synth* h = (la_synth*)malloc(sizeof(la_synth));
    if (!h) return 0;
    size_t need = 0;
    if (describe(h, img_resolution, img_channels, w_dim, channels, max_batch) == LA_OK) layout(h, nullptr, 0, &need);
    free(h);
    return need;
}

extern "C" int la_synth_create(int img_resolution, int img_channels, int w_dim, const int* channels, float conv_clamp,
                               const float* const* params, int nparams, const float* noise_strength, int nlayers,
                               const float* fir_host, int fir_h, int fir_w, int max_batch, void* workspace,
                               size_t workspace_bytes, hipStream_t stream, la_synth** out) {
    LA_CHECK_ARG(params && noise_strength && fir_host && workspace && out, "synth_create: null pointer");
    LA_CHECK_ARG(fir_h == 4 && fir_w == 4, "synth_create: resample filter must be 4x4 (setup_filter([1,3,3,1]))");
    la_synth* h = (la_synth*)malloc(sizeof(la_synth));
    LA_CHECK_ARG(h, "synth_create: out of host memory");
    int rc = describe(h, img_resolution, img_channels, w_dim, channels, max_batch);
    if (rc) { free(h); return rc; }
    if (nparams != la_synth_num_params(img_resolution) || nlayers != h->nconv) {
        free(h); la_set_error("synth_create: parameter list length mismatch"); return LA_ERR_ARG;
    }
    for (int i = 0; i < nparams; ++i)
        if (!params[i]) { free(h); la_set_error("synth_create: null parameter tensor"); return LA_ERR_ARG; }
    size_t need = 0;
    layout(h, workspace, workspace_bytes, &need);
    if (need > workspace_bytes) { free(h); la_set_error("synth_create: workspace too small"); return LA_ERR_WORKSPACE; }
    h->clamp = conv_clamp;
    h->win_lo = h->win_hi = 0; h->wcol_lo = h->wcol_hi = 0; h->fw_c0 = h->fw_c1 = 0;
    if (hipMemsetAsync(workspace, 0, need, stream) != hipSuccess) { free(h); la_set_error("synth_create: clearing the workspace failed"); return LA_ERR_HIP; }
    memcpy(h->fir, fir_host, sizeof(float) * 16);
    int p = 0, ci = 0;
    for (int k = 0; k < h->nblocks; ++k) {
        if (k == 0) h->cst = params[p++];
        const int nl = (k == 0) ? 1 : 2;
        for (int q = 0; q < nl; ++q) {
            ConvLayer& L = h->conv[ci];
            L.affine_w = params[p++]; L.affine_b = params[p++]; L.weight = params[p++]; L.bias = params[p++];
            L.noise_const = params[p++];
            L.noise_strength = noise_strength[ci];
            h->st.aw[L.style_idx] = L.affine_w; h->st.ab[L.style_idx] = L.affine_b;
            h->dt.wsq[ci] = L.wsq;
            rc = la_pack_conv_weights(L.weight, L.wf, L.wb, L.wsq, L.cout, L.cin, 9, stream);
            if (!rc) rc = la_pack_conv_weights_bf16_f32(L.weight, L.wqf, L.cout, L.cin, 9, 0, 3, stream);
            if (!rc) rc = la_pack_conv_weights_bf16_f32(L.weight, L.wqb, L.cout, L.cin, 9, 1, 3, stream);
            if (rc) { free(h); return rc; }
            ++ci;
        }
        RgbLayer& T = h->rgb[k];
        T.affine_w = params[p++]; T.affine_b = params[p++]; T.weight = params[p++]; T.bias = params[p++];
        h->st.aw[T.style_idx] = T.affine_w; h->st.ab[T.style_idx] = T.affine_b;
    }
    h->lastB = 0;
    *out = h;
    return LA_OK;
}

extern "C" void la_synth_destroy(la_synth* h) { free(h); }

extern "C" int la_synth_set_precision(la_synth* h, int precision) {
    LA_CHECK_ARG(h && precision >= 0 && precision <= 3, "synth_set_precision: precision must be 0..3");
    h->precision = precision;
    return LA_OK;
}
extern "C" int la_synth_get_precision(const la_synth* h) { return h ? h->precision : -1; }
extern "C" int la_synth_set_operand_scale(la_synth* h, int from_data) {
    LA_CHECK_ARG(h && (from_data == 0 || from_data == 1), "synth_set_operand_scale: 0 or 1");
    return LA_OK;
}

extern "C" int la_synth_set_row_window(la_synth* h, int row_lo, int row_hi) {
    LA_CHECK_ARG(h && row_lo >= 0 && (row_hi == 0 ? row_lo == 0 : (row_hi > row_lo && row_hi <= h->R)), "synth_set_row_window: bad window");
    h->win_lo = row_lo; h->win_hi = row_hi;
    return LA_OK;
}

extern "C" int la_synth_set_col_window(la_synth* h, int col_lo, int col_hi) {
    LA_CHECK_ARG(h && col_lo >= 0 && (col_hi == 0 ? col_lo == 0 : (col_hi > col_lo && col_hi <= h->R)), "synth_set_col_window: bad window");
    h->wcol_lo = col_lo; h->wcol_hi = col_hi;
    return LA_OK;
}

#ifdef LA_DEV
extern "C" const float* la_synth_dev_zt(const la_synth* h) { return h ? h->zT : nullptr; }
#endif
extern "C" const float* la_synth_image(const la_synth* h) { return h ? h->final_img : nullptr; }
extern "C" const float* la_synth_block_image(const la_synth* h, int k) { return (h && k >= 0 && k < h->nblocks) ? h->rgb[k].img : nullptr; }
extern "C" const float* la_synth_layer_output(const la_synth* h, int k) { return (h && k >= 0 && k < h->nconv) ? h->conv[k].y : nullptr; }
extern "C" const float* la_synth_styles(const la_synth* h) { return h ? h->s_all : nullptr; }
extern "C" const float* la_synth_style_grads(const la_synth* h) { return h ? h->ds_all : nullptr; }
extern "C" int la_synth_style_rows(const la_synth* h) { return h ? h->S : 0; }

extern "C" int la_synth_forward(la_synth* h, const float* ws, long ws_bstride, long ws_lstride, int B, int noise_mode,
                                const float* const* noises, float* img_out, hipStream_t stream) {
    LA_CHECK_ARG(h && ws, "synth_forward: null pointer");
    LA_CHECK_ARG(B >= 1 && B <= h->maxB, "synth_forward: batch exceeds the max_batch the workspace was sized for");
    LA_CHECK_ARG(noise_mode >= 0 && noise_mode <= 2, "synth_forward: noise_mode must be 0 (none), 1 (const), 2 (explicit)");
    LA_CHECK_ARG(noise_mode != 2 || noises, "synth_forward: explicit noise requested but no noise tensors given");
    int rc;
    if ((rc = la_affine_forward(h->st, ws, ws_bstride, ws_lstride, B, h->wdim, h->s_all, stream))) return rc;
    if ((rc = la_demod_forward(h->dt, h->s_all, h->S, B, h->d_all, stream))) return rc;
    h->lastB = B;
    const bool f16 = h->precision == LA_PREC_F16X2;
    static const bool zt_dense = la_dev_env("LA_NO_ZT_PITCH") != nullptr;
    if (f16 && (rc = la_xscale_from_bounds(h->dt, h->s_all, h->S, h->cst, h->channels[0] * 16, h->xs_fwd, h->xs_mult, B, stream, h->xs_bwd))) return rc;
    auto fwd_row = [&](int conv_index) { return (f16 && conv_index < h->nconv) ? h->xs_fwd + (long)conv_index * B * LA_XS_FAN : nullptr; };
    auto fwd_mult = [&](int conv_index) { return (f16 && conv_index < h->nconv) ? h->xs_mult + (long)conv_index * B : nullptr; };
    int wlo[2 * MAX_BLOCKS], whi[2 * MAX_BLOCKS], ilo[MAX_BLOCKS], ihi[MAX_BLOCKS];
    for (int i = 0; i < h->nconv; ++i) wlo[i] = whi[i] = 0;
    for (int i = 0; i < MAX_BLOCKS; ++i) ilo[i] = ihi[i] = 0;
    if (h->win_hi > 0 && h->precision != LA_PREC_F32 && !zt_dense) {
        int img_lo = h->win_lo, img_hi = h->win_hi, up_lo = 0, up_hi = 0;
        for (int k = h->nblocks - 1, c1 = h->nconv - 1; k >= 1; --k, c1 -= 2) {
            const int res = 4 << k;
            if (res < 64) break;
            int lo = img_lo, hi = img_hi;
            if (up_hi > 0) { lo = up_lo < lo ? up_lo : lo; hi = up_hi > hi ? up_hi : hi; }
            la_span_tiles(lo, hi, 4, res);
            if (lo <= 0 && hi >= res) break;
            wlo[c1] = lo; whi[c1] = hi;
            ilo[k] = img_lo; ihi[k] = img_hi;
            int l0 = lo, h0 = hi;
            la_span_grow(l0, h0, 1, 1, res);
            wlo[c1 - 1] = l0; whi[c1 - 1] = h0;
            la_modconv3x3_up2_fwd_rows(res, l0, h0, &up_lo, &up_hi);
            img_lo = (img_lo - 2) >> 1; if (img_lo < 0) img_lo = 0;
            img_hi = (img_hi >> 1) + 1; if (img_hi > res / 2) img_hi = res / 2;
        }
    }
    for (int i = 0; i < h->nconv; ++i) { h->fw_lo[i] = wlo[i]; h->fw_hi[i] = whi[i]; }
    int c1lo = 0, c1hi = 0, c0lo = 0, c0hi = 0;
    h->fw_c0 = h->fw_c1 = 0;
    if (h->wcol_hi > 0 && whi[h->nconv - 1] > 0 && h->R >= 64) {
        c1lo = h->wcol_lo; c1hi = h->wcol_hi;
        la_span_tiles(c1lo, c1hi, 32, h->R);
        if (h->wcol_lo - 1 >= c1lo && h->wcol_hi + 1 <= c1hi && (c1lo > 0 || c1hi < h->R)) {
            c0lo = c1lo; c0hi = c1hi;
            la_span_grow(c0lo, c0hi, 1, 1, h->R);
            h->fw_c0 = c1lo; h->fw_c1 = c1hi;
        } else c1lo = c1hi = 0;
    }
    int ci = 0;
    const float* x = h->cst;
    long x_bstride = 0;
    for (int k = 0; k < h->nblocks; ++k) {
        const int res = 4 << k;
        const int nl = (k == 0) ? 1 : 2;
        RgbLayer& T = h->rgb[k];
        float* const rgb_dst = (k == h->nblocks - 1 && img_out) ? img_out : T.img;
        const bool fuse_rgb = la_modconv3x3_fwd_fuses_rgb(h->precision, B, h->conv[ci + nl - 1].cin, h->conv[ci + nl - 1].cout, res);
        const float* skip = nullptr;
        if (k > 0 && fuse_rgb) {
            RgbLayer& P = h->rgb[k - 1];
            if ((rc = la_upfirdn2d_ex(P.img, T.g_img, B, h->imgc, res / 2, res / 2, h->fir, la_fir_up2(), stream)))
                return rc;
            skip = T.g_img;
        }
        for (int q = 0; q < nl; ++q, ++ci) {
            ConvLayer& L = h->conv[ci];
            L.noise_used = nullptr; L.noise_bstride = 0;
            if (L.noise_strength != 0.f) {
                if (noise_mode == 1) L.noise_used = L.noise_const;
                else if (noise_mode == 2) { L.noise_used = noises[ci]; L.noise_bstride = (long)res * res; LA_CHECK_ARG(L.noise_used, "synth_forward: missing noise tensor"); }
            }
            const LaRgbFuse rf = layer_rgb(h, T, skip, rgb_dst);
            LaModconvFwdOpts o;
            o.xscale = fwd_row(ci); o.xs_out = fwd_row(ci + 1); o.xs_mult = fwd_mult(ci + 1);
            o.win.row_lo = wlo[ci]; o.win.row_hi = whi[ci];
            if (!L.up) {
                if (fuse_rgb && q == nl - 1) o.rgb = &rf;
                if (ci == h->nconv - 1) { o.win.col_lo = c1lo; o.win.col_hi = c1hi; }
                rc = la_modconv3x3_fwd_ex(x, x_bstride, layer_conv(h, L, B, false), layer_epi(h, L), L.y, stream, o);
            } else {
                if (!zt_dense) { o.scratch_pitch = 2 * zt_xhalf(res); o.scratch_xhalf = zt_xhalf(res); }
                if (ci == h->nconv - 2) { o.win.col_lo = c0lo; o.win.col_hi = c0hi; }
                rc = la_modconv3x3_up2_fwd_ex(x, x_bstride, layer_conv(h, L, B, false), layer_epi(h, L), h->fir, h->zT, L.y, stream, o);
            }
            if (rc) return rc;
            x = L.y; x_bstride = (long)L.cout * res * res;
        }
        if (!fuse_rgb) {
            const float* skip_lo = k > 0 ? h->rgb[k - 1].img : nullptr;
            const bool iw = ihi[k] > 0 && (long)res * res > 4096;
            if ((rc = la_torgb_forward(x, layer_rgb(h, T, nullptr, rgb_dst), B, T.cin, res, res, stream, nullptr, iw ? ilo[k] : 0, iw ? ihi[k] : 0,
                                       skip_lo, h->fir)))
                return rc;
        }
        if (k == h->nblocks - 1) h->final_img = rgb_dst;
    }
    return LA_OK;
}

extern "C" int la_synth_backward(la_synth* h, const float* g_img, float* dws, hipStream_t stream) {
    LA_CHECK_ARG(h && g_img && dws, "synth_backward: null pointer");
    LA_CHECK_ARG(h->lastB >= 1, "synth_backward: no forward pass to differentiate");
    const int B = h->lastB;
    int rc;
    const float* gi = g_img;
    int ci = h->nconv - 1;
    const float* gx_next = nullptr;
    LaStyleFinish fin; memset(&fin, 0, sizeof(fin));
    fin.imgc = h->imgc; fin.d_stride = h->Dt; fin.s_stride = h->S; fin.ds_stride = h->S;
    auto fin_conv = [&](const ConvLayer& L, int ntiles, int nslabs) {
        LaStyleFinish::Conv& c = fin.conv[fin.nconv++];
        c.ds_part = L.dsp; c.ddn_part = L.ddnp; c.d = h->d_all + L.d_off; c.s = h->s_all + L.s_off; c.wsq = L.wsq;
        c.ds_out = h->ds_all + L.s_off; c.ntiles = ntiles; c.nslabs = nslabs; c.cin = L.cin; c.cout = L.cout;
    };
    static const bool no_fuse = la_dev_env("LA_NO_SEAM_FUSE") != nullptr;
    static const bool no_fuse2 = la_dev_env("LA_NO_SEAM2_FUSE") != nullptr;
    const bool f16 = h->precision == LA_PREC_F32 ? false : h->precision == LA_PREC_F16X2;
    static const bool no_xs = la_dev_env("LA_NO_XS_HANDOFF") != nullptr;
    const bool xs_hand = f16 && !no_xs;
    const float up_mult = la_modconv_up2_bwd_xs_mult(h->fir);
    auto xs_slot = [&](int conv_index) { return xs_hand ? h->xs_bwd + (long)conv_index * B * LA_XS_FAN : nullptr; };
    bool seam2_done = false;
    bool pyramid_done = false;
    const bool bw = xs_hand && !no_fuse && !no_fuse2 && h->precision != LA_PREC_F32;
    for (int k = h->nblocks - 1; k >= 0; --k) {
        const int res = 4 << k;
        const long HW = (long)res * res;
        const bool win = bw && k > 0 && h->fw_hi[ci] > 0;
        LaBwdRows rw1 = {}, rw0 = {};
        if (win && k == h->nblocks - 1 && h->fw_c1 > 0) {
            rw1.out.col_lo = rw0.in.col_lo = h->fw_c0; rw1.out.col_hi = rw0.in.col_hi = h->fw_c1;
        }
        if (win) {
            rw1.in.row_lo = h->fw_lo[ci]; rw1.in.row_hi = h->fw_hi[ci];
            rw1.out.row_lo = h->fw_lo[ci - 1]; rw1.out.row_hi = h->fw_hi[ci - 1];
            la_span_tiles(rw1.out.row_lo, rw1.out.row_hi, 4, res);
            rw0.in.row_lo = rw1.out.row_lo; rw0.in.row_hi = rw1.out.row_hi;
            if (ci - 2 >= 0 && h->fw_hi[ci - 2] > 0) { rw0.out.row_lo = h->fw_lo[ci - 2]; rw0.out.row_hi = h->fw_hi[ci - 2]; }
        }
        RgbLayer& T = h->rgb[k];
        ConvLayer& L1 = h->conv[ci];
        const int slabs = la_seam_slabs(HW);
        const int tiles1 = la_modconv_ds_tiles(res);
        const int nseg1 = seam2_done ? tiles1 : slabs;
        LaSeamArgs s;
        if (!seam2_done) {
            memset(&s, 0, sizeof(s));
            s.y = L1.y; s.gx_next = gx_next; s.gz = h->G0; s.HW = HW; s.C = L1.cout;
            la_seam_set_epi(s, layer_epi(h, L1));
            s.ddn_part = L1.ddnp;
            s.g_img = gi; s.rgb_pre = T.rgb_pre; s.rgb_clamp = h->clamp; s.wrgb = T.weight;
            s.s_rgb = h->s_all + T.s_off; s.s_stride = h->S; s.dweff_part = T.dwep;
            if (xs_hand) { s.xs_out = xs_slot(ci); s.xs_mult = 1.f; }
            else if (f16) s.pmax_out = h->pmax;
            if (win) { s.p_lo = (long)rw1.in.row_lo * res; s.p_hi = (long)rw1.in.row_hi * res; }
            if ((rc = la_seam_backward(s, B, h->imgc, stream))) return rc;
        }
        {
            LaStyleFinish::Rgb& r = fin.rgb[fin.nrgb++];
            r.dweff_part = T.dwep; r.wrgb = T.weight; r.ds_out = h->ds_all + T.s_off; r.nslabs = nseg1; r.C = T.cin;
        }
        const bool fuse_seam = k > 0 && h->precision != LA_PREC_F32 && !no_fuse;
        {
            const float* xin = (k == 0) ? h->cst : h->conv[ci - 1].y;
            const long xin_bs = (k == 0) ? 0 : (long)L1.cin * HW;
            LaSeamFuse sf; memset(&sf, 0, sizeof(sf));
            if (fuse_seam) {
                const ConvLayer& L0f = h->conv[ci - 1];
                la_seam_set_epi(sf, layer_epi(h, L0f));
                sf.ddn_part = L0f.ddnp;
                sf.pmax = f16 ? h->pmax2 : nullptr;
                if (xs_hand) { sf.xs_out = xs_slot(ci - 1); sf.xs_mult = up_mult; }
            }
            LaModconvBwdOpts o;
            o.in_pmax = f16 ? (seam2_done ? h->pmax3 : h->pmax) : nullptr; o.in_nseg = nseg1;
            o.seam = fuse_seam ? &sf : nullptr; o.xscale = xs_slot(ci); o.rows = win ? &rw1 : nullptr;
            if ((rc = la_modconv3x3_bwd_ex(h->G0, layer_conv(h, L1, B, true), xin, xin_bs, h->G1, L1.dsp, stream, o))) return rc;
            fin_conv(L1, tiles1, nseg1);
        }
        --ci;
        if (k == 0) break;
        ConvLayer& L0 = h->conv[ci];
        if (!fuse_seam) {
            memset(&s, 0, sizeof(s));
            s.y = L0.y; s.gx_next = h->G1; s.gz = h->G1; s.HW = HW; s.C = L0.cout;
            la_seam_set_epi(s, layer_epi(h, L0));
            s.ddn_part = L0.ddnp;
            if (xs_hand) { s.xs_out = xs_slot(ci); s.xs_mult = up_mult; }
            else if (f16) s.pmax_out = h->pmax;
            if ((rc = la_seam_backward(s, B, 0, stream))) return rc;
        }
        RgbLayer& P = h->rgb[k - 1];
        if (!pyramid_done) {
            if ((rc = la_upfirdn2d_ex(gi, P.g_img, B, h->imgc, res, res, h->fir, la_fir_down2_adjoint(), stream))) return rc;
            if (k >= 2 && res / 2 <= 256) {
                float* outs[MAX_BLOCKS];
                for (int q = k - 2; q >= 0; --q) outs[k - 2 - q] = h->rgb[q].g_img;
                if ((rc = la_image_grad_pyramid(P.g_img, outs, k - 1, B * h->imgc, res / 2, h->fir, stream))) return rc;
                pyramid_done = true;
            }
        }
        const bool fuse_seam2 = h->precision != LA_PREC_F32 && !no_fuse2;
        {
            const int hin = res / 2;
            const int tiles = la_modconv_ds_tiles(hin);
            const int nseg0 = fuse_seam ? tiles1 : slabs;
            LaSeamFuse sf2; memset(&sf2, 0, sizeof(sf2));
            if (fuse_seam2) {
                const ConvLayer& Lb = h->conv[ci - 1];
                la_seam_set_epi(sf2, layer_epi(h, Lb));
                sf2.ddn_part = Lb.ddnp;
                sf2.pmax = f16 ? h->pmax3 : nullptr;
                if (xs_hand) { sf2.xs_out = xs_slot(ci - 1); sf2.xs_mult = 1.f; }
                sf2.imgc = h->imgc; sf2.g_img = P.g_img; sf2.rgb_pre = P.rgb_pre; sf2.rgb_clamp = h->clamp;
                sf2.wrgb = P.weight; sf2.s_rgb = h->s_all + P.s_off; sf2.s_rgb_stride = h->S; sf2.dweff_part = P.dwep;
            }
            LaModconvBwdOpts o;
            o.in_pmax = f16 ? (fuse_seam ? h->pmax2 : h->pmax) : nullptr; o.in_nseg = nseg0;
            o.seam = fuse_seam2 ? &sf2 : nullptr; o.xscale = xs_slot(ci); o.rows = win ? &rw0 : nullptr;
            if ((rc = la_modconv3x3_up2_bwd_ex(h->G1, layer_conv(h, L0, B, true), h->conv[ci - 1].y, (long)L0.cin * hin * hin, h->fir, h->zT, h->G0, L0.dsp,
                                               stream, o)))
                return rc;
            fin_conv(L0, tiles, nseg0);
        }
        --ci;
        gx_next = h->G0;
        gi = P.g_img;
        seam2_done = fuse_seam2;
    }
    if ((rc = la_style_backward_all(fin, B, stream))) return rc;
    return la_affine_backward(h->st, h->ds_all, B, h->wdim, dws, h->num_ws, h->aff_part, stream);
}
```

### latentaugment_amd/latent_aug.py

```python
import ctypes as C
import math
import os
import random

import numpy as np
import torch

from . import _lib
from .synthesis import DiscriminatorEngine, FeatureEngine, MappingEngine, SynthesisEngine


def center_crop_geometry(load_size):
    crop = int(np.sqrt((load_size * load_size) / 2))
    return crop, int(round((load_size - crop) / 2.0))


def get_params(load_size, crop_size, preprocess='center_random_crop'):
    assert preprocess in ['center_random_crop', 'random_crop']
    new = load_size
    if preprocess == 'center_random_crop':
        new = int(np.sqrt((load_size * load_size) / 2))
    x = random.randint(0, max(0, new - crop_size))
    y = random.randint(0, max(0, new - crop_size))
    return {'crop_pos': (x, y)}


def write_png_gray(path, a):
    import struct
    import zlib
    a = np.ascontiguousarray(a, dtype=np.uint8)
    h, w = a.shape
    raw = b''.join(b'\x00' + a[y].tobytes() for y in range(h))

    def chunk(tag, data):
        return struct.pack('>I', len(data)) + tag + data + struct.pack('>I', zlib.crc32(tag + data) & 0xffffffff)
    with open(path, 'wb') as f:
        f.write(b'\x89PNG\r\n\x1a\n' + chunk(b'IHDR', struct.pack('>IIBBBBB', w, h, 8, 0, 0, 0, 0)) + chunk(b'IDAT', zlib.compress(raw, 6)) +
                chunk(b'IEND', b''))


def _preproc3(p):
    scale, shift = p
    scale = tuple(float(v) for v in scale) if hasattr(scale, '__len__') else (float(scale),) * 3
    shift = tuple(float(v) for v in shift) if hasattr(shift, '__len__') else (float(shift),) * 3
    assert len(scale) == 3 and len(shift) == 3
    return scale, shift


def write_curve_png(path, values, width=480, height=320, margin=24):
    v = np.asarray(list(values), dtype=np.float64)
    img = np.full([height, width], 255, dtype=np.uint8)
    x0, x1, y0, y1 = margin, width - margin - 1, margin, height - margin - 1
    img[y0, x0:x1 + 1] = img[y1, x0:x1 + 1] = 0
    img[y0:y1 + 1, x0] = img[y0:y1 + 1, x1] = 0
    if v.size and np.isfinite(v).any():
        v = np.where(np.isfinite(v), v, np.nan)
        lo, hi = float(np.nanmin(v)), float(np.nanmax(v))
        span = hi - lo if hi > lo else 1.0
        xs = np.full(v.size, (x0 + x1) // 2) if v.size == 1 else np.round(x0 + 4 + (x1 - x0 - 8) * np.arange(v.size) / (v.size - 1)).astype(int)
        ys = np.round(y1 - 4 - (y1 - y0 - 8) * (np.nan_to_num(v, nan=lo) - lo) / span).astype(int)
        for i in range(v.size):
            img[max(ys[i] - 2, 0):ys[i] + 3, max(xs[i] - 2, 0):xs[i] + 3] = 0
            if i + 1 < v.size:
                n = int(max(abs(xs[i + 1] - xs[i]), abs(ys[i + 1] - ys[i]), 1))
                for t in range(n + 1):
                    img[int(round(ys[i] + (ys[i + 1] - ys[i]) * t / n)), int(round(xs[i] + (xs[i + 1] - xs[i]) * t / n))] = 64
    write_png_gray(path, img)


def shard_bounds(batch, world_size, rank):
    per = (batch + world_size - 1) // world_size
    lo = min(rank * per, batch)
    hi = min(lo + per, batch)
    return lo, hi, per


def sharded(group=None):
    import torch.distributed as dist
    if not (dist.is_available() and dist.is_initialized()):
        return False
    return dist.get_world_size(group) > 1 or os.environ.get('LATENTAUG_FORCE_SHARDED') == '1'


def gather_shards(local, per, batch, group=None):
    import torch.distributed as dist
    world = dist.get_world_size(group)
    dev = local.device
    stage = dev.type == 'cuda' and dist.get_backend(group) == 'gloo'
    pad = torch.zeros([per] + list(local.shape[1:]), dtype=local.dtype, device='cpu' if stage else dev)
    pad[:local.shape[0]] = local
    out = torch.empty([world * per] + list(local.shape[1:]), dtype=local.dtype, device=pad.device)
    dist.all_gather_into_tensor(out, pad, group=group)
    return out[:batch].to(dev)


def broadcast_controls(crop_pos, group=None, device=None, host_group=None):
    import torch.distributed as dist
    ctl = [None]
    if dist.get_rank(group) == 0:
        ctl[0] = (int(crop_pos[0]), int(crop_pos[1]), random.getrandbits(48))
    src = dist.get_global_rank(group, 0) if group is not None else 0
    if host_group is not None:
        dist.broadcast_object_list(ctl, src=src, group=host_group, device=torch.device('cpu'))
        return ctl[0]
    on_host = dist.get_backend(group) == 'gloo' or device is None
    dist.broadcast_object_list(ctl, src=src, group=group, device=torch.device('cpu') if on_host else device)
    return ctl[0]


def host_control_group(group=None, device=None):
    import torch.distributed as dist
    if group is not None or dist.get_backend() == 'gloo' or os.environ.get('LATENTAUG_CTL_DEVICE') == '1':
        return None
    if not dist.is_gloo_available():
        return None
    try:
        g = dist.new_group(backend='gloo')
    except Exception as e:
        print(f'[latentaugment_amd] no gloo control group ({type(e).__name__}: {e}); control broadcast stays on the device path')
        g = None
    ok = torch.tensor([1 if g is not None else 0], device=device if device is not None else torch.device('cuda', torch.cuda.current_device()), dtype=torch.int32)
    dist.all_reduce(ok, op=dist.ReduceOp.MIN)
    return g if int(ok.item()) == 1 else None


class InMemoryLatentCodes:

    def __init__(self, codes):
        self.codes = dict(codes)

    def lookup(self, fname):
        return np.asarray(self.codes[fname], dtype=np.float32)


LATENT_SPACES = {'w': 0, 'w+': 1}


class LatentAug:
    def __init__(self, phase, opt, save_dir, gpu_ids, generator=None, discriminator=None, banks=None, latent_codes=None,
                 feature_net=None, group=None, _shared=None):
        self.save_dir = save_dir
        self.phase = phase
        self.group = group
        self._ctl_group = None
        if not gpu_ids:
            raise _lib.LatentAugHipError(
                'LatentAug (MI355X path) needs a GPU id in gpu_ids_aug; the CPU restatement lives in oracle/ and is '
                'test infrastructure only')
        if len(gpu_ids) > 1:
            raise _lib.LatentAugHipError(
                'one process drives one GPU: launch one rank per GPU (torch.distributed / RCCL) instead of passing '
                'several gpu_ids to a single process')
        self.device = torch.device('cuda', gpu_ids[0])
        self.res = opt.img_resolution
        self.batch_size = opt.batch_size
        self.modalities = [m for m in str(opt.modalities_aug).split(',') if m]
        self.num_epochs = opt.opt_num_epochs
        self.opt_lr = opt.opt_lr
        self.truncation_psi = opt.truncation_psi
        self.w_pix, self.w_lpips, self.w_latent, self.w_disc = opt.w_pix, opt.w_lpips, opt.w_latent, opt.w_disc
        self.crop_size = opt.crop_size_aug
        self.preprocess = opt.preprocess_aug
        self.soft_aug, self.alpha = bool(opt.soft_aug), opt.alpha
        self.verbose_log = opt.verbose_log
        self.criterion_mode = getattr(opt, 'criterion_mode', 'gemm')
        self.final_noise_mode = getattr(opt, 'final_noise_mode', 'random')
        self.precision = getattr(opt, 'precision', 'f16x2')
        space = getattr(opt, 'latent_space', None)
        self.latent_space = 'w' if space is None else str(space).lower()
        if self.latent_space not in LATENT_SPACES:
            raise _lib.LatentAugHipError(f'opt.latent_space = {space!r}: expected one of {sorted(LATENT_SPACES)}')
        self.wplus = self.latent_space == 'w+'
        self._script_path = None
        if self.w_lpips > 0 and feature_net is None:
            cands = [getattr(opt, 'lpips_script_path', None)]
            if getattr(opt, 'lpips_script', 'lpips_script') == 'lpips_script' and getattr(opt, 'model_dir', None):
                cands.append(os.path.join(opt.model_dir, 'vgg16.pt'))
            self._script_path = next((c for c in cands if c and os.path.isfile(c)), None)
            if self._script_path is None:
                raise NotImplementedError(
                    'w_lpips > 0 needs `feature_net=` (op list for synthesis.FeatureEngine, e.g. vgg16_lpips_ops(...)) or a local copy '
                    "of NVIDIA's TorchScript vgg16.pt at opt.lpips_script_path / <model_dir>/vgg16.pt (the reference downloads it, "
                    "util_latent_aug.py:36; there is no network here), and banks['fea'] or the interim image zip to build them from")
        if generator is None:
            from . import formats
            path = formats.find_network_pkl(opt.model_dir, opt.dataset_aug, opt.dataset_name_aug, self.modalities,
                                            opt.exp_stylegan, opt.network_pkl_stylegan)
            print(f'Loading stylegan from "{path}"...')
            nets_ = formats.load_network_pkl(path)
            generator = nets_['G_ema']
            if discriminator is None:
                discriminator = nets_.get('D')
        max_local = self.batch_size
        try:
            import torch.distributed as dist
            if sharded(group):
                max_local = (self.batch_size + dist.get_world_size(group) - 1) // dist.get_world_size(group)
        except (RuntimeError, ValueError):
            pass
        max_local = int(getattr(opt, 'max_local_batch', 0) or max_local)
        self.engine = SynthesisEngine.from_generator(generator, self.device, max_local, precision=self.precision)
        assert self.engine.img_resolution == self.res, 'opt.img_resolution does not match the generator'
        assert self.engine.img_channels == len(self.modalities), 'one image channel per modality expected'
        self.num_ws, self.w_dim = self.engine.num_ws, self.engine.w_dim
        self.z_dim = getattr(generator, 'z_dim', self.w_dim)
        self._generator = generator
        self._mapping = None
        self.stats_dataset_w = latent_codes
        self.stats_loss = {}
        self.stats_time = {}
        self._verbose_flag = bool(opt.verbose_log)

        if banks is None and _shared is None and getattr(opt, 'interim_dir', None) and getattr(opt, 'dataset_aug', None):
            from . import formats
            root = os.path.join(opt.interim_dir, opt.dataset_aug)
            cache_dir = os.path.join(root, 'cache_dir')
            banks = {}
            wzip = os.path.join(root, str(getattr(opt, 'dataset_w_name', '')) + '.zip')
            if self.stats_dataset_w is None and os.path.isfile(wzip):
                self.stats_dataset_w = formats.LatentCodeDataset(os.path.join(root, opt.dataset_w_name + '.zip'),
                                                                 split=self.phase, w_dim=self.w_dim, num_ws=self.num_ws)
            if self.w_latent > 0:
                banks['W'] = formats.compute_stats(self.stats_dataset_w, 'latent', cache_dir, step=opt.step_w).get_all_torch()
            if self.w_pix > 0:
                ds = formats.ImgDataset(os.path.join(root, opt.dataset_name_aug + '.zip'), split=self.phase,
                                        modalities=self.modalities, resolution=self.res)
                banks['X'] = formats.compute_stats(ds, 'img', cache_dir, step=opt.step_img).get_all_torch()
        banks = banks or {}
        if _shared is not None:
            banks = dict(_shared['banks'])
        lib = _lib.load()
        self._lib = lib
        crop, off = center_crop_geometry(self.res)
        self.center_crop, self.center_off = crop, off
        self.W = None
        self.Xc = None
        Mw = Mx = 0
        if self.w_latent > 0:
            W = banks['W'].to(device=self.device, dtype=torch.float32).contiguous()
            assert W.shape[1:] == (self.num_ws, self.w_dim)
            self.W, Mw = W, W.shape[0]
        if self.w_pix > 0 and _shared is not None:
            self.Xc = _shared['Xc']
            Mx = self.Xc.shape[1]
        elif self.w_pix > 0:
            X = banks['X'].to(device=self.device, dtype=torch.float32).contiguous()
            assert X.shape[1:] == (len(self.modalities), self.res, self.res)
            Mx = X.shape[0]
            xc = torch.empty([Mx, X.shape[1], crop, crop], device=self.device, dtype=torch.float32)
            with torch.cuda.device(self.device):
                _lib.check(lib.la_center_crop_f32(_lib.ptr(X), _lib.ptr(xc), Mx * X.shape[1], self.res, crop, off,
                                                  _lib.stream_ptr()), 'la_center_crop')
            self.Xc = xc.permute(1, 0, 2, 3).contiguous()
            del X, xc
        cfg = _lib.OptConfig(steps=int(self.num_epochs), lr=float(self.opt_lr), beta1=0.9, beta2=0.999, eps=1e-8,
                             w_latent=float(self.w_latent), w_pix=float(self.w_pix), w_disc=float(self.w_disc),
                             w_lpips=float(self.w_lpips),
                             criterion_mode={'gemm': 0, 'collapsed': 1}[self.criterion_mode],
                             soft_aug=int(self.soft_aug), alpha=float(self.alpha), loop_noise_mode=1,
                             final_noise_mode={'none': 0, 'const': 1, 'random': 2}[self.final_noise_mode],
                             norm_batch=int(getattr(opt, 'norm_batch', 0) or 0), crop=crop, crop_off=off)
        self._cfg = cfg
        space = LATENT_SPACES[self.latent_space]
        nbytes = lib.la_latent_opt_workspace_bytes_ex(self.res, self.engine.img_channels, self.w_dim, C.byref(cfg), Mw, Mx,
                                                      max_local, space)
        self._workspace = torch.empty([max(nbytes, 64)], dtype=torch.uint8, device=self.device)
        h = C.c_void_p()
        _lib.check(lib.la_latent_opt_create_ex(self.engine.handle, self.res, self.engine.img_channels, self.w_dim,
                                               C.byref(cfg), _lib.ptr(self.W), Mw, _lib.ptr(self.Xc), Mx, max_local, space,
                                               _lib.ptr(self._workspace), self._workspace.numel(), C.byref(h)),
                   'la_latent_opt_create')
        self._h = h
        self._max_local = max_local
        self._opt, self._discriminator, self._feature_net = opt, discriminator, feature_net
        self.stream_lanes = getattr(opt, 'stream_lanes', 'auto')
        assert self.stream_lanes in ('auto', 1, 2), "opt.stream_lanes: 'auto', 1 or 2"
        self._lanes = None
        self._lane_stream = None
        self.lanes_active = False
        self.lanes_concurrent = True
        self._lanes_check = bool(getattr(opt, 'lanes_selfcheck', True))
        self.lanes_selfcheck = None
        self.hip_graph = bool(getattr(opt, 'hip_graph', True))
        _lib.check(lib.la_latent_opt_set_graph(h, int(self.hip_graph)), 'la_latent_opt_set_graph')
        oc = getattr(opt, 'overlap_criteria', True)
        self.overlap_criteria = int(oc) if not isinstance(oc, bool) else (2 if oc else 0)
        _lib.check(lib.la_latent_opt_set_overlap(h, self.overlap_criteria), 'la_latent_opt_set_overlap')
        self.loop_window = None
        if getattr(opt, 'loop_window', True) and self.w_disc <= 0 and (self.w_pix > 0 or self.w_lpips > 0) and \
                (self.w_lpips <= 0 or self.preprocess in ('center_crop', 'center_random_crop')):
            self.loop_window = (off, off + crop)
            _lib.check(lib.la_latent_opt_set_row_window(h, off, off + crop), 'la_latent_opt_set_row_window')
            if getattr(opt, 'loop_window_columns', True):
                _lib.check(lib.la_latent_opt_set_col_window(h, off, off + crop), 'la_latent_opt_set_col_window')
        self.disc = None
        if self.w_disc > 0:
            if discriminator is None:
                raise _lib.LatentAugHipError('w_disc > 0 needs the discriminator (pass `discriminator=` or a network pickle)')
            self.disc = DiscriminatorEngine(discriminator, self.device, max_local, precision=self.precision)
            assert self.disc.img_resolution == self.res and self.disc.img_channels == self.engine.img_channels
            _lib.check(lib.la_latent_opt_set_disc(h, self.disc.handle), 'la_latent_opt_set_disc')

        self.feat = None
        if self.w_lpips > 0:
            imgc = self.engine.img_channels
            if feature_net is not None:
                self.feat = FeatureEngine(feature_net, self.device, in_res=self.crop_size, max_batch=imgc * max_local,
                                          precision=self.precision)
            else:
                print(f'Loading VGG16 from: {self._script_path}')
                self.feat = FeatureEngine.from_torchscript(self._script_path, self.device, in_res=self.crop_size,
                                                           max_batch=imgc * max_local, precision=self.precision)
                if not hasattr(opt, 'lpips_preproc'):
                    opt.lpips_preproc = (self.feat.pre_scale, self.feat.pre_shift)
            if 'fea' not in banks:
                if not (getattr(opt, 'interim_dir', None) and getattr(opt, 'dataset_aug', None)):
                    raise _lib.LatentAugHipError("w_lpips > 0 needs banks['fea'] or the interim image zip to build them from")
                banks['fea'] = self._build_feature_banks(opt)
            fea = banks['fea']
            assert len(fea) == imgc
            if _shared is not None and _shared.get('Fbank') is not None:
                self.Fbank = _shared['Fbank']
            else:
                self.Fbank = torch.stack([t.to(device=self.device, dtype=torch.float32) for t in fea]).contiguous()
            assert self.Fbank.shape[2] == self.feat.num_features, 'feature bank does not match the feature net'
            Mf = self.Fbank.shape[1]
            scale, shift = _preproc3(getattr(opt, 'lpips_preproc', (1.0, 0.0)))
            nb = lib.la_latent_opt_lpips_workspace_bytes(imgc, self.feat.num_features, self.crop_size, Mf, max_local)
            self._lpips_ws = torch.empty([nb], dtype=torch.uint8, device=self.device)
            _lib.check(lib.la_latent_opt_set_lpips(h, self.feat.handle, _lib.ptr(self.Fbank), Mf, self.crop_size, float(scale[0]),
                                                   float(shift[0]), _lib.ptr(self._lpips_ws), nb), 'la_latent_opt_set_lpips')
            _lib.check(lib.la_latent_opt_set_lpips_preproc(h, (C.c_float * 3)(*scale), (C.c_float * 3)(*shift), 3),
                       'la_latent_opt_set_lpips_preproc')
        if _shared is None and self.lanes_eligible(self._max_local):
            self.build_lanes()

    def _build_feature_banks(self, opt):
        from . import formats
        root = os.path.join(opt.interim_dir, opt.dataset_aug)
        ds = formats.ImgDataset(os.path.join(root, opt.dataset_name_aug + '.zip'), split=self.phase, modalities=self.modalities,
                                resolution=self.res)
        raw = getattr(opt, 'lpips_bank_range', 'unit') == 'raw'
        scale, shift = _preproc3(getattr(opt, 'lpips_preproc', (1.0, 0.0)))
        sc_t = torch.tensor(scale, device=self.device).reshape(1, 3, 1, 1)
        sh_t = torch.tensor(shift, device=self.device).reshape(1, 3, 1, 1)
        out = []
        for mode_id, mode in enumerate(self.modalities):
            def feature_fn(x, mode_id=mode_id):
                t = torch.from_numpy(x[:, mode_id:mode_id + 1]).to(self.device)
                if not raw:
                    t = t / 127.5 - 1
                ax, ay = self.crop_window(get_params(self.res, self.crop_size, self.preprocess)['crop_pos'])
                t = t[:, :, ay:ay + self.crop_size, ax:ax + self.crop_size].repeat(1, 3, 1, 1) * sc_t + sh_t
                return self.feat.forward(t.contiguous()).cpu().numpy()
            tag = f'{mode}-{self.crop_size}'
            if not (raw and (scale, shift) == ((1.0,) * 3, (0.0,) * 3) and getattr(opt, 'lpips_cache_compat', False)):
                def fmt(v):
                    return f'{v[0]:g}' if v[0] == v[1] == v[2] else '_'.join(f'{t:g}' for t in v)
                tag += f"-{'raw' if raw else 'unit'}-s{fmt(scale)}-b{fmt(shift)}-w{self.feat.weights_digest}"
            st = formats.compute_stats(ds, 'features_jit', os.path.join(root, 'cache_dir'), cache_tag=tag,
                                       step=opt.step_img, feature_fn=feature_fn)
            out.append(st.get_all_torch())
        return out

    def __del__(self):
        h = getattr(self, '_h', None)
        if h:
            self._lib.la_latent_opt_destroy(h)
            self._h = None

    def broadcasting(self, latent):
        return latent.repeat([1, self.num_ws, 1])

    @staticmethod
    def reverse_broadcasting(latent):
        return latent[:, :1, :]

    def crop_window(self, crop_pos):
        x1, y1 = crop_pos
        off = self.center_off if self.preprocess in ('center_crop', 'center_random_crop') else 0
        return off + int(x1), off + int(y1)

    @property
    def latent_rows(self):
        return self.num_ws if self.wplus else 1

    def run_local(self, w, final_noises=None, want_losses=False, crop_pos=None, trace=None, out=None):
        if self.feat is not None:
            if crop_pos is None:
                crop_pos = getattr(self, 'crop_params', None)
                crop_pos = crop_pos['crop_pos'] if crop_pos else get_params(self.res, self.crop_size, self.preprocess)['crop_pos']
            ax, ay = self.crop_window(crop_pos)
            _lib.check(self._lib.la_latent_opt_set_crop_pos(self._h, ax, ay), 'la_latent_opt_set_crop_pos')
        w = w.to(device=self.device, dtype=torch.float32).contiguous()
        b = w.shape[0]
        assert w.ndim == 3 and w.shape[1:] == (self.latent_rows, self.w_dim), \
            f'latent_space {self.latent_space!r} takes w [b, {self.latent_rows}, {self.w_dim}], got {tuple(w.shape)}'
        if out is not None:
            img, w_aug = out
            assert img.shape == (b, self.engine.img_channels, self.res, self.res) and w_aug.shape == (b, self.num_ws, self.w_dim)
            assert img.is_contiguous() and w_aug.is_contiguous() and img.dtype == w_aug.dtype == torch.float32
        else:
            img = torch.empty([b, self.engine.img_channels, self.res, self.res], device=self.device, dtype=torch.float32)
            w_aug = torch.empty([b, self.num_ws, self.w_dim], device=self.device, dtype=torch.float32)
        losses = torch.zeros([max(self.num_epochs, 1), 4], device=self.device) if want_losses else None
        fn = None
        if self._cfg.final_noise_mode == 2:
            if final_noises is None:
                final_noises = self.engine.make_noises(b)
            fn = self.engine.noise_pointer_array(final_noises)
        tw = ti = tg = None
        want_img = trace is not None and 'img' in trace.get('want', ('w', 'img'))
        if trace is not None and self.num_epochs > 0:
            wshape = [self.num_epochs, b] + ([self.num_ws] if self.wplus else []) + [self.w_dim]
            tw = torch.empty(wshape, device=self.device, dtype=torch.float32)
            if want_img:
                ti = torch.empty([self.num_epochs, b, self.engine.img_channels, self.res, self.res], device=self.device, dtype=torch.float32)
            if 'grad' in trace.get('want', ()):
                tg = torch.empty(wshape, device=self.device, dtype=torch.float32)
        with torch.cuda.device(self.device):
            if tw is not None:
                _lib.check(self._lib.la_latent_opt_set_trace(self._h, _lib.ptr(tw), _lib.ptr(ti)), 'la_latent_opt_set_trace')
                _lib.check(self._lib.la_latent_opt_set_grad_trace(self._h, _lib.ptr(tg)), 'la_latent_opt_set_grad_trace')
            try:
                _lib.check(self._lib.la_latent_opt_run(self._h, _lib.ptr(w), b, fn, _lib.ptr(img), _lib.ptr(w_aug),
                                                       _lib.ptr(losses), _lib.stream_ptr()), 'la_latent_opt_run')
            finally:
                if tw is not None:
                    _lib.check(self._lib.la_latent_opt_set_trace(self._h, None, None), 'la_latent_opt_set_trace')
                    _lib.check(self._lib.la_latent_opt_set_grad_trace(self._h, None), 'la_latent_opt_set_grad_trace')
        if tw is not None:
            trace['w'] = tw
            if ti is not None:
                trace['img'] = ti
            if tg is not None:
                trace['grad'] = tg
        self._keep = final_noises
        return img, w_aug, losses

    def lanes_eligible(self, b):
        if self.stream_lanes == 1 or b != self._max_local or b < 4 or b % 2:
            return False
        if self.w_disc > 0 and b % 8:
            return False
        if self.stream_lanes == 2 or self.w_lpips <= 0:
            return True
        return self.w_disc > 0 and self.overlap_criteria >= 1

    def build_lanes(self):
        import copy
        half = self._max_local // 2
        opt = copy.copy(self._opt)
        opt.batch_size, opt.max_local_batch, opt.norm_batch = half, half, self._max_local
        opt.verbose_log, opt.stream_lanes = False, 1
        opt.overlap_criteria = 1 if self.overlap_criteria == 2 else self.overlap_criteria
        shared = {'banks': {'W': self.W, 'fea': list(self.Fbank) if self.feat is not None else None}, 'Xc': self.Xc,
                  'Fbank': self.Fbank if self.feat is not None else None}
        self._lanes = [LatentAug(self.phase, opt, self.save_dir, [self.device.index], generator=self._generator,
                                 discriminator=self._discriminator, banks={}, latent_codes=self.stats_dataset_w,
                                 feature_net=self._feature_net, _shared=shared) for _ in range(2)]
        self._lane_stream = torch.cuda.Stream(device=self.device)

    def run_lanes(self, w, final_noises=None, crop_pos=None, concurrent=True):
        if self._lanes is None:
            self.build_lanes()
        w = w.to(device=self.device, dtype=torch.float32).contiguous()
        b = w.shape[0]
        assert b == self._max_local and b % 2 == 0, 'stream lanes take the full (even) local batch'
        if crop_pos is None and self.feat is not None:
            crop_pos = getattr(self, 'crop_params', None)
            crop_pos = crop_pos['crop_pos'] if crop_pos else get_params(self.res, self.crop_size, self.preprocess)['crop_pos']
        if self._cfg.final_noise_mode == 2 and final_noises is None:
            final_noises = self.engine.make_noises(b)
        parts, outs, fns = [], [], []
        for k in (0, 1):
            parts.append(w[k::2].contiguous())
            outs.append((torch.empty([b // 2, self.engine.img_channels, self.res, self.res], device=self.device, dtype=torch.float32),
                         torch.empty([b // 2, self.num_ws, self.w_dim], device=self.device, dtype=torch.float32)))
            fns.append([t[k::2].contiguous() if t is not None else None for t in final_noises] if final_noises is not None else None)
        main = torch.cuda.current_stream(self.device)
        side = self._lane_stream if concurrent else main
        if concurrent:
            side.wait_stream(main)
        self._lanes[0].run_local(parts[0], fns[0], crop_pos=crop_pos, out=outs[0])
        with torch.cuda.stream(side):
            self._lanes[1].run_local(parts[1], fns[1], crop_pos=crop_pos, out=outs[1])
        if concurrent:
            main.wait_stream(side)
        img = torch.empty([b, self.engine.img_channels, self.res, self.res], device=self.device, dtype=torch.float32)
        w_aug = torch.empty([b, self.num_ws, self.w_dim], device=self.device, dtype=torch.float32)
        for k in (0, 1):
            img[k::2] = outs[k][0]
            w_aug[k::2] = outs[k][1]
        self._keep_lanes = (parts, outs, fns)
        return img, w_aug, None

    def run_batch(self, w, final_noises=None):
        self.lanes_active = self.lanes_eligible(w.shape[0])
        if not self.lanes_active:
            return self.run_local(w, final_noises)
        if self.lanes_selfcheck is None and self.lanes_concurrent:
            return self._lanes_first_batch(w, final_noises)
        return self.run_lanes(w, final_noises, concurrent=self.lanes_concurrent)

    def _lanes_first_batch(self, w, final_noises):
        if not self._lanes_check:
            self.lanes_selfcheck = 'off'
            return self.run_lanes(w, final_noises, concurrent=True)
        if self._lanes is None:
            self.build_lanes()
        if self._cfg.final_noise_mode == 2 and final_noises is None:
            final_noises = self.engine.make_noises(w.shape[0])
        crop_pos = None
        if self.feat is not None:
            cp = getattr(self, 'crop_params', None)
            crop_pos = cp['crop_pos'] if cp else get_params(self.res, self.crop_size, self.preprocess)['crop_pos']
        ref_img, ref_w, _ = self.run_lanes(w, final_noises, crop_pos=crop_pos, concurrent=False)
        img, w_aug, _ = self.run_lanes(w, final_noises, crop_pos=crop_pos, concurrent=True)
        if torch.equal(img, ref_img) and torch.equal(w_aug, ref_w):
            self.lanes_selfcheck = 'bit-identical'
            return img, w_aug, None
        import warnings
        dw = float((w_aug - ref_w).abs().max())
        self.lanes_selfcheck = 'differs: lanes serial from now on'
        self.lanes_concurrent = False
        warnings.warn(f'latentaugment_amd: the two stream lanes side by side did not reproduce the lanes one after the other on the first '
                      f'batch (max |dw| {dw:.3e}); this handle runs them one after the other from now on (opt.stream_lanes = 1 avoids the '
                      f'lanes altogether)')
        return ref_img, ref_w, None

    def _log_first_batch(self, losses, elapsed, trace, fname, times=None):
        import json
        import pickle
        L = losses.cpu().numpy()
        active = [('loss_latent', 0, self._cfg.w_latent), ('loss_disc', 2, self._cfg.w_disc), ('loss_pix', 1, self._cfg.w_pix),
                  ('loss_lpips', 3, self._cfg.w_lpips)]
        for e in range(self.num_epochs):
            st = {name: float(L[e, col]) for name, col, wgt in active if wgt > 0}
            st['loss'] = float(-L[e, 0] - L[e, 1] - L[e, 3] + L[e, 2])
            self.stats_loss[f'epoch_{e}'] = st
            if times is not None:
                self.stats_time[f'epoch_{e}'] = {'time_latent': float(times[e, 0]), 'time_disc': float(times[e, 1]), 'time_pix': float(times[e, 2]),
                                                 'time_lpips': float(times[e, 3]), 'time_epoch': float(times[e, 4])}
            else:
                self.stats_time[f'epoch_{e}'] = {'time_epoch': elapsed / max(self.num_epochs, 1)}
            desc = ''.join(f'{k} {v:<4.2f} ' for k, v in st.items()) + '||| ' + ''.join(f'{k} {v:<4.3f} ' for k, v in self.stats_time[f'epoch_{e}'].items())
            print(f'epoch {e + 1:>4d}/{self.num_epochs}, {desc}')
        if self.save_dir and self.num_epochs > 0:
            os.makedirs(self.save_dir, exist_ok=True)
            for stats, title in ((self.stats_loss, 'losses'), (self.stats_time, 'times [s]')):
                ticks = list(stats.values())
                for key in ticks[0].keys():
                    write_curve_png(os.path.join(self.save_dir, f'{title}_{key}.png'), [x[key] for x in ticks])
                with open(os.path.join(self.save_dir, f'{title}.jsonl'), 'w') as f:
                    f.write(json.dumps(stats, indent=2) + '\n')
            if trace and 'w' in trace and fname:
                base = os.path.splitext(os.path.basename(str(fname[0])))[0]
                tw, ti = trace['w'].cpu().numpy(), trace['img'].cpu().numpy()
                w_in = trace.get('w_in')
                for e in range(self.num_epochs):
                    with open(os.path.join(self.save_dir, f'w_{base}_{e}.pkl'), 'wb') as f:
                        pickle.dump((w_in if w_in is not None else tw[e]).squeeze(), f, pickle.HIGHEST_PROTOCOL)
                    with open(os.path.join(self.save_dir, f'w_opt_{base}_{e}.pkl'), 'wb') as f:
                        pickle.dump(tw[e].squeeze(), f, pickle.HIGHEST_PROTOCOL)
                    if ti.shape[2] >= 2:
                        row = np.concatenate([ti[e, 0, 0], ti[e, 0, 1]], axis=1)
                    else:
                        row = ti[e, 0, 0]
                    row = ((np.clip(row, -1.0, 1.0) + 1) / 2 * 255.0).astype(np.uint8)
                    write_png_gray(os.path.join(self.save_dir, f'{base}_{e}.png'), row)

    def forward(self, w, fname=None, final_noises=None):
        if w.ndim == 2:
            w = self.z_to_w(w)
        self.crop_params = get_params(self.res, self.crop_size, self.preprocess)
        import torch.distributed as dist
        if sharded(self.group):
            B = w.shape[0]
            rank = dist.get_rank(self.group)
            lo, hi, per = shard_bounds(B, dist.get_world_size(self.group), rank)
            cx, cy, noise_seed = broadcast_controls(self.crop_params['crop_pos'], self.group, self.device, self._host_group())
            self._last_controls = (cx, cy, noise_seed)
            self.crop_params = {'crop_pos': (cx, cy)}
            timers = getattr(self, 'shard_timers', None)
            if timers is not None:
                ev = tuple(torch.cuda.Event(enable_timing=True) for _ in range(3))
                ev[0].record()
            if hi > lo:
                if final_noises is not None:
                    fn = [t[lo:hi].contiguous() if t is not None else None for t in final_noises]
                elif self._cfg.final_noise_mode == 2:
                    fn = self.engine.make_noises(B, batch_seed=noise_seed, rows=(lo, hi))
                else:
                    fn = None
                if self._verbose_flag and rank == 0:
                    img, w_aug = self._run_verbose(w[lo:hi], fn, fname[lo:hi] if fname is not None else None)
                else:
                    img, w_aug, _ = self.run_batch(w[lo:hi], fn)
                self._verbose_flag = False
            else:
                img = torch.empty([0, self.engine.img_channels, self.res, self.res], device=self.device)
                w_aug = torch.empty([0, self.num_ws, self.w_dim], device=self.device)
            flat = torch.cat([img.reshape(img.shape[0], -1), w_aug.reshape(w_aug.shape[0], -1)], dim=1)
            if timers is not None:
                ev[1].record()
            full = gather_shards(flat, per, B, self.group)
            if timers is not None:
                ev[2].record()
                timers.append(ev)
            n_img = self.engine.img_channels * self.res * self.res
            img = full[:, :n_img].reshape(B, self.engine.img_channels, self.res, self.res)
            w_aug = full[:, n_img:].reshape(B, self.num_ws, self.w_dim)
            return img, w_aug
        if self._verbose_flag:
            img, w_aug = self._run_verbose(w, final_noises, fname)
            self._verbose_flag = False
            return img, w_aug
        img, w_aug, _ = self.run_batch(w, final_noises)
        return img, w_aug

    def _run_verbose(self, w, final_noises, fname):
        import time
        trace = {} if w.shape[0] == 1 else None
        torch.cuda.synchronize(self.device)
        _lib.check(self._lib.la_latent_opt_set_time_trace(self._h, 1), 'la_latent_opt_set_time_trace')
        t0 = time.time()
        try:
            img, w_aug, losses = self.run_local(w, final_noises, want_losses=True, trace=trace)
            torch.cuda.synchronize(self.device)
            elapsed = time.time() - t0
            times = None
            if self.num_epochs > 0:
                buf = (C.c_float * (5 * self.num_epochs))()
                _lib.check(self._lib.la_latent_opt_get_times(self._h, buf), 'la_latent_opt_get_times')
                times = np.asarray(buf, dtype=np.float64).reshape(self.num_epochs, 5) * 1e-3
        finally:
            _lib.check(self._lib.la_latent_opt_set_time_trace(self._h, 0), 'la_latent_opt_set_time_trace')
        if trace is not None:
            trace['w_in'] = w.detach().cpu().numpy()
        self._log_first_batch(losses, elapsed, trace, fname, times)
        return img, w_aug

    def _host_group(self):
        if self._ctl_group is None:
            self._ctl_group = host_control_group(self.group, self.device) or False
        return self._ctl_group or None

    @property
    def graph_state(self):
        if self.lanes_active and self._lanes:
            return min(l.graph_state for l in self._lanes)
        return int(self._lib.la_latent_opt_graph_state(self._h))

    __call__ = forward

    @property
    def mapping(self):
        if self._mapping is None:
            self._mapping = MappingEngine(self._generator, self.device)
            self.z_dim = self._mapping.z_dim
        return self._mapping

    def z_to_w(self, z):
        ws = self.mapping.forward(z.to(self.device), self.num_ws, self.truncation_psi)
        return ws if self.wplus else self.reverse_broadcasting(ws)

    def forward_ganrand(self, z, noises=None):
        import torch.distributed as dist
        if sharded(self.group):
            B = z.shape[0]
            rank = dist.get_rank(self.group)
            lo, hi, per = shard_bounds(B, dist.get_world_size(self.group), rank)
            _, _, noise_seed = broadcast_controls((0, 0), self.group, self.device, self._host_group())
            gloo = dist.get_backend(self.group) == 'gloo'
            zb = z.detach().to('cpu' if gloo else self.device, torch.float32).contiguous()
            dist.broadcast(zb, src=dist.get_global_rank(self.group, 0) if self.group is not None else 0, group=self.group)
            n_img = self.engine.img_channels * self.res * self.res
            if hi > lo:
                ws = self.mapping.forward(zb[lo:hi].to(self.device), self.num_ws, self.truncation_psi)
                if noises is not None:
                    fn = [t[lo:hi].contiguous() if t is not None else None for t in noises]
                elif self.final_noise_mode == 'random':
                    fn = self.engine.make_noises(B, batch_seed=noise_seed, rows=(lo, hi))
                else:
                    fn = None
                img = self.engine.forward(ws, noise_mode=self.final_noise_mode, noises=fn)
                flat = torch.cat([img.reshape(hi - lo, -1), ws.reshape(hi - lo, -1)], dim=1)
            else:
                flat = torch.empty([0, n_img + self.num_ws * self.w_dim], device=self.device)
            full = gather_shards(flat, per, B, self.group)
            return (full[:, :n_img].reshape(B, self.engine.img_channels, self.res, self.res),
                    full[:, n_img:].reshape(B, self.num_ws, self.w_dim))
        ws = self.mapping.forward(z.to(self.device), self.num_ws, self.truncation_psi)
        img = self.engine.forward(ws, noise_mode=self.final_noise_mode, noises=noises)
        return img, ws


def define_latentaugment(module_name, phase, opt, save_dir, gpu_ids=[], **inject):
    if module_name == 'latent_aug':
        return LatentAug(phase, opt, save_dir, gpu_ids, **inject)
    raise NotImplementedError('Module name [%s] is not recognized' % module_name)
```

### latentaugment_amd/synthesis.py

```python
import ctypes as C
import math

import numpy as np
import torch

from . import _lib

_CONV_KEYS = ('affine.weight', 'affine.bias', 'weight', 'bias', 'noise_const')
_RGB_KEYS = ('affine.weight', 'affine.bias', 'weight', 'bias')
NOISE_MODES = {'none': 0, 'const': 1, 'random': 2}
PRECISIONS = {'f32': 0, 'bf16x3': 1, 'bf16x2': 2, 'f16x2': 3}


def _state_dict_of(G):
    sd = G if isinstance(G, dict) else G.state_dict()
    if any(k.startswith('synthesis.') for k in sd):
        sd = {k[len('synthesis.'):]: v for k, v in sd.items() if k.startswith('synthesis.')}
    return sd


class SynthesisEngine:
    def __init__(self, state_dict, device, max_batch, conv_clamp=256.0, precision='f32'):
        lib = _lib.load()
        self.device = torch.device(device)
        if self.device.type != 'cuda':
            raise _lib.LatentAugHipError('SynthesisEngine needs a ROCm device (no CPU fallback)')
        sd = state_dict
        res_list = sorted({int(k.split('.')[0][1:]) for k in sd if k.startswith('b')})
        assert res_list and res_list[0] == 4, 'expected synthesis blocks b4..bR'
        self.img_resolution = res_list[-1]
        self.block_resolutions = res_list
        self.channels = [int(sd[f'b{r}.conv1.weight'].shape[0]) for r in res_list]
        self.img_channels = int(sd[f'b{res_list[-1]}.torgb.weight'].shape[0])
        self.w_dim = int(sd['b4.conv1.affine.weight'].shape[1])
        self.num_ws = lib.la_synth_num_ws(self.img_resolution)
        self.max_batch = int(max_batch)
        self.conv_clamp = float(-1.0 if conv_clamp is None else conv_clamp)

        def dev(name):
            t = sd[name].detach().to(device=self.device, dtype=torch.float32).contiguous()
            self._keep.append(t)
            return t

        self._keep = []
        params = []
        strengths = []
        self.layer_resolutions = []
        for r in res_list:
            if r == 4:
                params.append(dev('b4.const'))
            layers = ('conv1',) if r == 4 else ('conv0', 'conv1')
            for ln in layers:
                for k in _CONV_KEYS:
                    params.append(dev(f'b{r}.{ln}.{k}'))
                strengths.append(float(sd[f'b{r}.{ln}.noise_strength']))
                self.layer_resolutions.append(r)
            for k in _RGB_KEYS:
                t = dev(f'b{r}.torgb.{k}')
                if k == 'weight':
                    t = t.reshape(t.shape[0], t.shape[1]).contiguous()
                    self._keep.append(t)
                params.append(t)
        fkey = f'b{res_list[-1]}.resample_filter'
        fir = sd[fkey].detach().cpu().float().numpy() if fkey in sd else None
        if fir is None:
            f1 = np.array([1, 3, 3, 1], dtype=np.float32)
            fir = np.outer(f1, f1) / 64.0
        assert fir.shape == (4, 4), 'resample filter must be the 4x4 setup_filter([1,3,3,1])'
        self._fir = np.ascontiguousarray(fir, dtype=np.float32)
        self.noise_strengths = strengths
        self.num_layers = len(strengths)

        chan = (C.c_int * len(self.channels))(*self.channels)
        nbytes = lib.la_synth_workspace_bytes(self.img_resolution, self.img_channels, self.w_dim, chan, self.max_batch)
        assert nbytes > 0
        self._workspace = torch.empty([nbytes], dtype=torch.uint8, device=self.device)
        self.workspace_bytes = nbytes
        pp = (C.c_void_p * len(params))(*[p.data_ptr() for p in params])
        ns = (C.c_float * len(strengths))(*strengths)
        h = C.c_void_p()
        with torch.cuda.device(self.device):
            _lib.check(lib.la_synth_create(self.img_resolution, self.img_channels, self.w_dim, chan, self.conv_clamp, pp,
                                           len(params), ns, len(strengths), self._fir.ctypes.data, 4, 4, self.max_batch,
                                           _lib.ptr(self._workspace), nbytes, _lib.stream_ptr(), C.byref(h)),
                       'la_synth_create')
        self._h = h
        self._lib = lib
        self.set_precision(precision)

    operand_scale = 'data (producer-lowered slot rows)'

    def operand_headroom(self, ws):
        ws = ws.to(self.device, torch.float32).contiguous()
        self.forward(ws, noise_mode='const')
        b = ws.shape[0]
        s = self.styles(b).abs()
        cins = [self.channels[0]] + [self.channels[self.block_resolutions.index(r)] for r in self.layer_resolutions[:-1]]
        ratio, off = float('inf'), cins[0]
        for k in range(1, len(self.layer_resolutions)):
            sk = s[:, off:off + cins[k]]
            xm = self.layer_output(k - 1, b).abs().amax(dim=(2, 3))
            r = (xm * sk).amax(dim=1) / (self.conv_clamp * sk.amax(dim=1)).clamp_min(1e-30)
            ratio = min(ratio, float(r.min()))
            off += cins[k]
        return ratio

    def set_precision(self, precision):
        _lib.check(self._lib.la_synth_set_precision(self._h, PRECISIONS[precision]), 'la_synth_set_precision')
        self.precision = precision

    @classmethod
    def from_generator(cls, G, device, max_batch, conv_clamp=None, precision='f32'):
        if conv_clamp is None and not isinstance(G, dict):
            try:
                conv_clamp = getattr(G.synthesis, f'b{G.img_resolution}').conv1.conv_clamp
            except AttributeError:
                conv_clamp = 256.0
        return cls(_state_dict_of(G), device, max_batch, conv_clamp=256.0 if conv_clamp is None else conv_clamp,
                   precision=precision)

    def __del__(self):
        h = getattr(self, '_h', None)
        if h:
            self._lib.la_synth_destroy(h)
            self._h = None

    @property
    def handle(self):
        return self._h

    def make_noises(self, batch, generator=None, batch_seed=None, rows=None):
        lo, hi = (0, batch) if rows is None else rows
        assert 0 <= lo <= hi <= batch
        out = []
        lib = _lib.load()
        for li, (r, ns) in enumerate(zip(self.layer_resolutions, self.noise_strengths)):
            if ns == 0.0:
                out.append(None)
            elif batch_seed is None:
                assert rows is None
                out.append(torch.randn([batch, r, r], device=self.device, generator=generator))
            else:
                t = torch.empty([hi - lo, r, r], device=self.device, dtype=torch.float32)
                with torch.cuda.device(self.device):
                    _lib.check(lib.la_noise_normal_f32(_lib.ptr(t), hi - lo, r * r, int(batch_seed) & 0xFFFFFFFFFFFFFFFF, li, lo,
                                                       _lib.stream_ptr()), 'la_noise_normal_f32')
                out.append(t)
        return out

    def noise_pointer_array(self, noises):
        if noises is None:
            return None
        assert len(noises) == self.num_layers
        for t, r, ns in zip(noises, self.layer_resolutions, self.noise_strengths):
            if t is None:
                assert ns == 0.0, 'a layer with noise_strength != 0 needs its noise tensor'
                continue
            assert t.is_cuda and t.dtype == torch.float32 and t.is_contiguous() and t.shape[-2:] == (r, r)
        return (C.c_void_p * len(noises))(*[t.data_ptr() if t is not None else None for t in noises])

    def forward(self, ws, noise_mode='const', noises=None, out=None):
        _lib.require_gpu(ws)
        ws = ws.contiguous().float()
        if ws.ndim == 2:
            ws = ws[:, None]
        B = ws.shape[0]
        assert ws.shape[2] == self.w_dim and ws.shape[1] in (1, self.num_ws)
        lstride = 0 if ws.shape[1] == 1 else self.w_dim
        mode = NOISE_MODES[noise_mode]
        if mode == 2 and noises is None:
            noises = self.make_noises(B)
        np_arr = self.noise_pointer_array(noises) if mode == 2 else None
        img = out if out is not None else torch.empty([B, self.img_channels, self.img_resolution, self.img_resolution],
                                                      device=self.device, dtype=torch.float32)
        with torch.cuda.device(self.device):
            _lib.check(self._lib.la_synth_forward(self._h, _lib.ptr(ws), ws.shape[1] * self.w_dim, lstride, B, mode, np_arr,
                                                  _lib.ptr(img), _lib.stream_ptr()), 'la_synth_forward')
        self._last_noises = noises
        return img

    def backward(self, g_img):
        g_img = g_img.contiguous().float()
        B = g_img.shape[0]
        dws = torch.empty([B, self.num_ws, self.w_dim], device=self.device, dtype=torch.float32)
        with torch.cuda.device(self.device):
            _lib.check(self._lib.la_synth_backward(self._h, _lib.ptr(g_img), _lib.ptr(dws), _lib.stream_ptr()),
                       'la_synth_backward')
        return dws

    def _view(self, p, shape):
        n = int(np.prod(shape))
        base = self._workspace.data_ptr()
        off = p - base
        assert 0 <= off and off + 4 * n <= self.workspace_bytes
        return self._workspace[off:off + 4 * n].view(torch.float32).reshape(shape)

    def layer_output(self, k, batch):
        r = self.layer_resolutions[k]
        block = self.block_resolutions.index(r)
        return self._view(self._lib.la_synth_layer_output(self._h, k), [batch, self.channels[block], r, r])

    def styles(self, batch):
        rows = self._lib.la_synth_style_rows(self._h)
        return self._view(self._lib.la_synth_styles(self._h), [batch, rows])

    def style_grads(self, batch):
        rows = self._lib.la_synth_style_rows(self._h)
        return self._view(self._lib.la_synth_style_grads(self._h), [batch, rows])


class _SynthesisFn(torch.autograd.Function):
    @staticmethod
    def forward(ctx, ws, engine, noise_mode, noises):
        ctx.engine = engine
        ctx.ws_shape = ws.shape
        return engine.forward(ws, noise_mode=noise_mode, noises=noises)

    @staticmethod
    def backward(ctx, g_img):
        dws = ctx.engine.backward(g_img)
        shape = ctx.ws_shape
        if len(shape) == 2:
            dws = dws.sum(dim=1)
        elif shape[1] == 1:
            dws = dws.sum(dim=1, keepdim=True)
        return dws, None, None, None


def synthesis(engine, ws, noise_mode='const', noises=None):
    return _SynthesisFn.apply(ws, engine, noise_mode, noises)


class MappingEngine:

    def __init__(self, G, device, lr_multiplier=0.01):
        self._lib = _lib.load()
        self.device = torch.device(device)
        sd = G if isinstance(G, dict) else G.state_dict()
        sd = {k[len('mapping.'):]: v for k, v in sd.items() if k.startswith('mapping.')}
        n = 0
        while f'fc{n}.weight' in sd:
            n += 1
        if n == 0:
            raise _lib.LatentAugHipError('generator has no mapping.fc* tensors: z input / rand_aug needs the mapping network')
        self.num_layers = n
        self.weights = [sd[f'fc{i}.weight'].detach().to(self.device, torch.float32).contiguous() for i in range(n)]
        self.biases = [sd[f'fc{i}.bias'].detach().to(self.device, torch.float32).contiguous() for i in range(n)]
        self.z_dim = int(self.weights[0].shape[1])
        self.w_dim = int(self.weights[-1].shape[0])
        self.w_avg = sd['w_avg'].detach().to(self.device, torch.float32).contiguous() if 'w_avg' in sd else None
        self.lr_multiplier = float(lr_multiplier)
        self._wp = (C.c_void_p * n)(*[t.data_ptr() for t in self.weights])
        self._bp = (C.c_void_p * n)(*[t.data_ptr() for t in self.biases])

    def forward(self, z, num_ws, truncation_psi=1.0):
        _lib.require_gpu(z)
        z = z.contiguous().float()
        B = z.shape[0]
        assert z.shape[1] == self.z_dim
        tmp = torch.empty([2 * B * max(self.z_dim, self.w_dim)], device=self.device, dtype=torch.float32)
        ws = torch.empty([B, num_ws, self.w_dim], device=self.device, dtype=torch.float32)
        with torch.cuda.device(self.device):
            _lib.check(self._lib.la_mapping_forward_f32(_lib.ptr(z), B, self.z_dim, self.w_dim, self.num_layers, self._wp,
                                                        self._bp, self.lr_multiplier, _lib.ptr(self.w_avg),
                                                        float(truncation_psi), num_ws, _lib.ptr(tmp), _lib.ptr(ws),
                                                        _lib.stream_ptr()), 'la_mapping_forward')
        return ws


class DiscriminatorEngine:

    def __init__(self, D, device, max_batch, conv_clamp=256.0, precision='f32', mbstd_group_size=4):
        lib = _lib.load()
        self._lib = lib
        self.device = torch.device(device)
        if self.device.type != 'cuda':
            raise _lib.LatentAugHipError('DiscriminatorEngine needs a ROCm device (no CPU fallback)')
        sd = D if isinstance(D, dict) else D.state_dict()
        res_list = sorted({int(k.split('.')[0][1:]) for k in sd if k.startswith('b') and k.split('.')[0][1:].isdigit()})
        assert res_list[0] == 4 and len(res_list) >= 2, 'expected discriminator blocks b4..bR'
        R = res_list[-1]
        self.img_resolution = R
        self.img_channels = int(sd[f'b{R}.fromrgb.weight'].shape[1])
        ch = {r: int(sd[f'b{r}.conv0.weight'].shape[1]) for r in res_list if r > 4}
        ch[4] = int(sd['b4.conv.weight'].shape[0])
        self.channels = [ch[r] for r in res_list]
        self._keep = []

        def dev(name):
            t = sd[name].detach().to(device=self.device, dtype=torch.float32).contiguous()
            self._keep.append(t)
            return t

        params = []
        for r in reversed(res_list[1:]):
            if r == R:
                params += [dev(f'b{r}.fromrgb.weight'), dev(f'b{r}.fromrgb.bias')]
            params += [dev(f'b{r}.conv0.weight'), dev(f'b{r}.conv0.bias'), dev(f'b{r}.conv1.weight'), dev(f'b{r}.conv1.bias'),
                       dev(f'b{r}.skip.weight')]
        params += [dev('b4.conv.weight'), dev('b4.conv.bias'), dev('b4.fc.weight'), dev('b4.fc.bias'), dev('b4.out.weight'),
                   dev('b4.out.bias')]
        assert len(params) == lib.la_disc_num_params(R)
        f1 = np.array([1, 3, 3, 1], dtype=np.float32)
        self._fir = np.ascontiguousarray(np.outer(f1, f1) / 64.0, dtype=np.float32)
        chan = (C.c_int * len(self.channels))(*self.channels)
        self.max_batch = int(max_batch)
        nbytes = lib.la_disc_workspace_bytes(R, self.img_channels, chan, self.max_batch)
        assert nbytes > 0
        self._workspace = torch.empty([nbytes], dtype=torch.uint8, device=self.device)
        pp = (C.c_void_p * len(params))(*[p.data_ptr() for p in params])
        h = C.c_void_p()
        clamp = float(-1.0 if conv_clamp is None else conv_clamp)
        with torch.cuda.device(self.device):
            _lib.check(lib.la_disc_create(R, self.img_channels, chan, clamp, pp, len(params), self._fir.ctypes.data,
                                          int(mbstd_group_size), self.max_batch, _lib.ptr(self._workspace), nbytes,
                                          _lib.stream_ptr(), C.byref(h)), 'la_disc_create')
        self._h = h
        _lib.check(lib.la_disc_set_precision(h, PRECISIONS[precision]), 'la_disc_set_precision')

    def __del__(self):
        h = getattr(self, '_h', None)
        if h:
            self._lib.la_disc_destroy(h)
            self._h = None

    @property
    def handle(self):
        return self._h

    def forward(self, img):
        _lib.require_gpu(img)
        img = img.contiguous().float()
        B = img.shape[0]
        with torch.cuda.device(self.device):
            _lib.check(self._lib.la_disc_forward(self._h, _lib.ptr(img), B, _lib.stream_ptr()), 'la_disc_forward')
            p = self._lib.la_disc_logits(self._h)
            off = p - self._workspace.data_ptr()
            return self._workspace[off:off + 4 * B].view(torch.float32).clone().reshape(B, 1)

    def backward(self, dlogits):
        dl = dlogits.contiguous().float().reshape(-1)
        B = dl.shape[0]
        g = torch.empty([B, self.img_channels, self.img_resolution, self.img_resolution], device=self.device)
        with torch.cuda.device(self.device):
            _lib.check(self._lib.la_disc_backward(self._h, _lib.ptr(dl), _lib.ptr(g), 0, _lib.stream_ptr()), 'la_disc_backward')
        return g


FEAT_CONV, FEAT_TAP, FEAT_MAXPOOL, FEAT_AVGPOOL, FEAT_FC_RELU, FEAT_FC = 0, 1, 2, 3, 4, 5
RESIZE_MODES = {'area': 0, 'bilinear': 1}


class FeatureEngine:

    def __init__(self, ops, device, in_res, max_batch, in_ch=3, precision='f32'):
        lib = _lib.load()
        self._lib = lib
        self.device = torch.device(device)
        if self.device.type != 'cuda':
            raise _lib.LatentAugHipError('FeatureEngine needs a ROCm device (no CPU fallback)')
        self._keep = []
        desc, params = [], []
        c = in_ch
        for op in ops:
            if op[0] == 'conv':
                w = op[1].detach().to(self.device, torch.float32).contiguous()
                b = op[2].detach().to(self.device, torch.float32).contiguous()
                assert w.shape[1] == c and w.shape[2:] == (3, 3)
                desc.append(_lib.FeatOp(FEAT_CONV, c, w.shape[0]))
                c = w.shape[0]
                params += [w, b]
            elif op[0] == 'tap':
                lin = op[1].detach().to(self.device, torch.float32).contiguous()
                assert lin.shape == (c,)
                desc.append(_lib.FeatOp(FEAT_TAP, c, c))
                params.append(lin)
            elif op[0] in ('maxpool', 'avgpool'):
                desc.append(_lib.FeatOp(FEAT_MAXPOOL if op[0] == 'maxpool' else FEAT_AVGPOOL, c, c))
            elif op[0] == 'fc':
                w = op[1].detach().to(self.device, torch.float32).contiguous()
                b = op[2].detach().to(self.device, torch.float32).contiguous()
                assert w.ndim == 2 and b.shape == (w.shape[0],)
                desc.append(_lib.FeatOp(FEAT_FC_RELU if op[3] else FEAT_FC, w.shape[1], w.shape[0]))
                c = w.shape[0]
                params += [w, b]
            else:
                raise ValueError(op[0])
        self._keep = params
        import hashlib
        hsh = hashlib.sha1()
        for op in ops:
            hsh.update(op[0].encode())
            for t in op[1:]:
                hsh.update(t.detach().to('cpu', torch.float32).contiguous().numpy().tobytes() if torch.is_tensor(t) else repr(t).encode())
        self.weights_digest = hsh.hexdigest()[:10]
        self.in_ch, self.in_res, self.max_batch = in_ch, in_res, int(max_batch)
        arr = (_lib.FeatOp * len(desc))(*desc)
        nbytes = lib.la_feat_workspace_bytes(len(desc), arr, in_ch, in_res, self.max_batch)
        assert nbytes > 0, 'invalid feature-net description: ' + (lib.la_last_error() or b'?').decode()
        self._workspace = torch.empty([nbytes], dtype=torch.uint8, device=self.device)
        pp = (C.c_void_p * len(params))(*[p.data_ptr() for p in params])
        h = C.c_void_p()
        with torch.cuda.device(self.device):
            _lib.check(lib.la_feat_create(len(desc), arr, pp, len(params), in_ch, in_res, self.max_batch,
                                          _lib.ptr(self._workspace), nbytes, _lib.stream_ptr(), C.byref(h)), 'la_feat_create')
        self._h = h
        self.num_features = lib.la_feat_num_features(h)
        _lib.check(lib.la_feat_set_precision(h, PRECISIONS[precision]), 'la_feat_set_precision')

    @classmethod
    def from_torchscript(cls, src, device, in_res, max_batch, precision='f32', probe_seed=0, rtol=2e-3):
        cands = vgg16_from_torchscript(src)
        g = torch.Generator().manual_seed(probe_seed)
        probe = torch.rand([2, 1, in_res, in_res], generator=g).repeat(1, 3, 1, 1) * 255.0
        with torch.no_grad():
            try:
                want = cands[0].source(probe, resize_images=False, return_lpips=True)
            except (RuntimeError, TypeError):
                want = cands[0].source(probe)
        want = want.reshape(2, -1).to(torch.float32)
        errs = []
        for c in cands:
            eng = cls(c.ops, device, in_res, max_batch=max(max_batch, 2), precision='f32')
            if eng.num_features != want.shape[1]:
                errs.append(float('inf'))
                continue
            x = probe * torch.tensor(c.pre_scale).reshape(1, 3, 1, 1) + torch.tensor(c.pre_shift).reshape(1, 3, 1, 1)
            got = eng.forward(x.to(eng.device)).cpu()
            err = float((got - want).norm() / want.norm().clamp_min(1e-30))
            errs.append(err)
            if err <= rtol:
                if precision != 'f32' or max_batch != eng.max_batch:
                    eng = cls(c.ops, device, in_res, max_batch=max_batch, precision=precision)
                eng.pre_scale, eng.pre_shift, eng.lin_is_sqrt = c.pre_scale, c.pre_shift, c.lin_is_sqrt
                return eng
            del eng
        raise _lib.LatentAugHipError('TorchScript feature net: no mapping of its tensors onto the VGG16-LPIPS op list reproduces the '
                                     f"module's own output (relative errors of the candidates: {errs}); refusing to guess")

    def __del__(self):
        h = getattr(self, '_h', None)
        if h:
            self._lib.la_feat_destroy(h)
            self._h = None

    @property
    def handle(self):
        return self._h

    def forward(self, x):
        _lib.require_gpu(x)
        x = x.contiguous().float()
        N = x.shape[0]
        assert x.shape[1:] == (self.in_ch, self.in_res, self.in_res)
        f = torch.empty([N, self.num_features], device=self.device, dtype=torch.float32)
        with torch.cuda.device(self.device):
            _lib.check(self._lib.la_feat_forward(self._h, _lib.ptr(x), N, _lib.ptr(f), _lib.stream_ptr()), 'la_feat_forward')
        self._x = x
        return f

    def backward(self, gfeat):
        gfeat = gfeat.contiguous().float()
        gx = torch.empty_like(self._x)
        with torch.cuda.device(self.device):
            _lib.check(self._lib.la_feat_backward(self._h, _lib.ptr(gfeat), _lib.ptr(gx), _lib.stream_ptr()), 'la_feat_backward')
        return gx


def vgg16_lpips_ops(state_dict, lins):
    conv_ids = [0, 2, 5, 7, 10, 12, 14, 17, 19, 21, 24, 26, 28]
    tap_after = {2: 0, 7: 1, 14: 2, 21: 3, 28: 4}
    pool_after = {2, 7, 14, 21}
    ops = []
    for i in conv_ids:
        ops.append(('conv', state_dict[f'features.{i}.weight'], state_dict[f'features.{i}.bias']))
        if i in tap_after:
            ops.append(('tap', lins[tap_after[i]]))
        if i in pool_after:
            ops.append(('maxpool',))
    return ops


class ScriptedFeatureNet:

    def __init__(self, ops, pre_scale, pre_shift, lin_is_sqrt, source):
        self.ops, self.pre_scale, self.pre_shift, self.lin_is_sqrt, self.source = ops, pre_scale, pre_shift, lin_is_sqrt, source


def _script_tensors(module):
    sd = module.state_dict()
    return [(k, v.detach().to('cpu', torch.float32)) for k, v in sd.items() if torch.is_tensor(v) and v.is_floating_point()]


def vgg16_from_torchscript(src, map_location='cpu'):
    module = src if isinstance(src, torch.jit.ScriptModule) else torch.jit.load(src, map_location=map_location)
    module = module.eval()
    items = _script_tensors(module)
    convs, used = [], set()
    for idx, (k, v) in enumerate(items):
        if v.ndim == 4 and v.shape[2:] == (3, 3):
            bias = None
            cand = k[:-len('weight')] + 'bias' if k.endswith('weight') else None
            for j, (kj, vj) in enumerate(items):
                if j in used or vj.ndim != 1 or vj.shape[0] != v.shape[0]:
                    continue
                if (cand is not None and kj == cand) or (cand is None and j == idx + 1):
                    bias, _ = vj, used.add(j)
                    break
            if bias is None and idx + 1 < len(items) and items[idx + 1][1].ndim == 1 and items[idx + 1][1].shape[0] == v.shape[0]:
                bias = items[idx + 1][1]
                used.add(idx + 1)
# ... 200 lines not shown
```

Baseline: 87.91 images/s.

## Run both stream lanes through a paired native loop with block-split graph parts

Result: no change. 87.81 images/s (-0.1%).

```diff
diff --git a/include/latentaug_hip.h b/include/latentaug_hip.h
--- a/include/latentaug_hip.h
+++ b/include/latentaug_hip.h
@@ -158,6 +158,9 @@
 int la_synth_set_row_window(la_synth* h, int row_lo, int row_hi);
 int la_synth_set_col_window(la_synth* h, int col_lo, int col_hi);
 int la_synth_get_precision(const la_synth* h);
+int la_synth_set_launch_blocks(la_synth* h, int k_lo, int k_hi);
+int la_synth_num_blocks(const la_synth* h);
+int la_synth_split_block(const la_synth* h);
 int la_synth_forward(la_synth* h, const float* ws, long ws_bstride, long ws_lstride, int B, int noise_mode,
                      const float* const* noises, float* img_out, la_stream_t stream);
 int la_synth_backward(la_synth* h, const float* g_img, float* dws, la_stream_t stream);
@@ -259,6 +262,11 @@
 int la_latent_opt_invalidate_banks(la_latent_opt* h);
 int la_latent_opt_run(la_latent_opt* h, const float* w0, int B, const float* const* final_noises, float* img_out,
                       float* w_aug_out, float* losses_out, la_stream_t stream);
+int la_latent_opt_run_pair(la_latent_opt* ha, la_latent_opt* hb, const float* w0_a, const float* w0_b, int B,
+                           const float* const* final_noises_a, const float* const* final_noises_b, float* img_out_a, float* img_out_b,
+                           float* w_aug_out_a, float* w_aug_out_b, float* losses_out_a, float* losses_out_b, la_stream_t stream_a,
+                           la_stream_t stream_b, int schedule);
+int la_latent_opt_parts_state(const la_latent_opt* h);
 
 int la_feature_moments_f64(const float* x, long n, int D, double* raw_mean, double* raw_cov, la_stream_t stream);
 size_t la_pr_workspace_floats(long nr, long nc);
diff --git a/latentaugment_amd/csrc/la_conv.h b/latentaugment_amd/csrc/la_conv.h
--- a/latentaugment_amd/csrc/la_conv.h
+++ b/latentaugment_amd/csrc/la_conv.h
@@ -151,4 +151,5 @@
 bool la_conv_bf16_uses_halo(const LaConvArgs& a);
 
 int la_conv_tiles_per_sample(int Gy, int Gx);
+int la_conv_splitk_max_points();
 int la_conv_launch(const LaConvArgs& a, hipStream_t stream);
diff --git a/latentaugment_amd/csrc/la_conv.hip b/latentaugment_amd/csrc/la_conv.hip
--- a/latentaugment_amd/csrc/la_conv.hip
+++ b/latentaugment_amd/csrc/la_conv.hip
@@ -8,6 +8,7 @@
 int la_conv_tiles_per_sample(int Gy, int Gx) { return la_cdiv((long)Gy * Gx, NT); }
 
 #define SPLITK_MAX_G 1156
+int la_conv_splitk_max_points() { return SPLITK_MAX_G; }
 static int choose_ksplit(bool bf, long tiles, int nck, float taps, double out_bytes) {
     int ks;
     if (bf) {
diff --git a/latentaugment_amd/csrc/la_latent_opt.hip b/latentaugment_amd/csrc/la_latent_opt.hip
--- a/latentaugment_amd/csrc/la_latent_opt.hip
+++ b/latentaugment_amd/csrc/la_latent_opt.hip
@@ -38,6 +38,11 @@
     hipGraph_t seg_graph[4];
     hipGraphExec_t seg_exec[4];
     int seg_valid;
+    hipGraph_t part_graph[3];
+    hipGraphExec_t part_exec[3];
+    int part_valid;
+    hipEvent_t* pair_ev;
+    int pair_nev;
     hipStream_t cap_stream;
     float* trace_w;
     float* trace_img;
@@ -139,6 +144,11 @@
         if (h->seg_graph[k]) { (void)hipGraphDestroy(h->seg_graph[k]); h->seg_graph[k] = nullptr; }
     }
     h->seg_valid = 0;
+    for (int k = 0; k < 3; ++k) {
+        if (h->part_exec[k]) { (void)hipGraphExecDestroy(h->part_exec[k]); h->part_exec[k] = nullptr; }
+        if (h->part_graph[k]) { (void)hipGraphDestroy(h->part_graph[k]); h->part_graph[k] = nullptr; }
+    }
+    h->part_valid = 0;
     h->graph_B = 0; h->graph_win = 0;
 }
 
@@ -146,6 +156,7 @@
     if (!h) return;
     drop_graph(h);
     if (h->tev) { for (int i = 0; i < h->tev_steps * LA_TEV; ++i) (void)hipEventDestroy(h->tev[i]); free(h->tev); }
+    if (h->pair_ev) { for (int i = 0; i < h->pair_nev; ++i) (void)hipEventDestroy(h->pair_ev[i]); free(h->pair_ev); }
     if (h->ev_fork) (void)hipEventDestroy(h->ev_fork);
     if (h->ev_join) (void)hipEventDestroy(h->ev_join);
     if (h->side_stream) (void)hipStreamDestroy(h->side_stream);
@@ -294,16 +305,46 @@
     return LA_OK;
 }
 
-extern "C" int la_latent_opt_run(la_latent_opt* h, const float* w0, int B, const float* const* final_noises,
-                                 float* img_out, float* w_aug_out, float* losses_out, hipStream_t stream) {
-    LA_CHECK_ARG(h && w0 && img_out && w_aug_out, "latent_opt_run: null pointer");
-    LA_CHECK_ARG(B >= 1 && B <= h->maxB, "latent_opt_run: batch exceeds max_batch");
-    const la_opt_config& c = h->cfg;
-    LA_CHECK_ARG(c.final_noise_mode != 2 || final_noises, "latent_opt_run: explicit final noise requested but not given");
-    const int wd = h->wdim, cc = c.crop, off = c.crop_off;
-    const long cc2 = (long)cc * cc;
-    const long nw = (long)B * wd * (h->wplus ? h->num_ws : 1);
+namespace {
+struct LoopRun {
+    la_latent_opt* h = nullptr;
+    const float* w0; int B; const float* const* final_noises; float *img_out, *w_aug_out, *losses_out;
+    hipStream_t stream;
+    int wd, cc, off;
+    long cc2, nw;
+    bool use_disc, use_lpips, img_crit, want_losses, windowed, replay, split;
+    float lp_coef, lat_coef, pix_coef;
+    int first_graph_step = 1;
+    int k_split = 0, nblocks = 0;
+
+    ~LoopRun() {
+        if (!h) return;
+        (void)la_synth_set_row_window(h->g, 0, 0); (void)la_synth_set_col_window(h->g, 0, 0); (void)la_synth_set_launch_blocks(h->g, 0, 0);
+    }
+    int begin(la_latent_opt* handle, const float* w0_, int B_, const float* const* final_noises_, float* img_out_, float* w_aug_out_,
+              float* losses_out_, hipStream_t stream_);
+    int run_step(float* L, hipStream_t st, int step_index = -1, int seg = 15, int part = 0);
+    bool capture(int seg, int part, hipGraph_t* g, hipGraphExec_t* e);
+    int prepare(bool want_parts);
+    int enqueue_step(int step);
+    int finish();
+    bool parts_ready() const { return replay && !split && h->part_valid && h->graph_B == B; }
+};
+}
+
+int LoopRun::begin(la_latent_opt* handle, const float* w0_, int B_, const float* const* final_noises_, float* img_out_, float* w_aug_out_,
+                   float* losses_out_, hipStream_t stream_) {
+    LA_CHECK_ARG(handle && w0_ && img_out_ && w_aug_out_, "latent_opt_run: null pointer");
+    LA_CHECK_ARG(B_ >= 1 && B_ <= handle->maxB, "latent_opt_run: batch exceeds max_batch");
+    const la_opt_config& c = handle->cfg;
+    LA_CHECK_ARG(c.final_noise_mode != 2 || final_noises_, "latent_opt_run: explicit final noise requested but not given");
+    h = handle; w0 = w0_; B = B_; final_noises = final_noises_; img_out = img_out_; w_aug_out = w_aug_out_; losses_out = losses_out_;
+    stream = stream_;
+    wd = h->wdim; cc = c.crop; off = c.crop_off;
+    cc2 = (long)cc * cc;
+    nw = (long)B * wd * (h->wplus ? h->num_ws : 1);
     const float nb = (float)(c.norm_batch > 0 ? c.norm_batch : B);
+    nblocks = la_synth_num_blocks(h->g); k_split = la_synth_split_block(h->g);
     int rc;
     LA_HIP(hipMemcpyAsync(h->w_opt, w0, nw * sizeof(float), hipMemcpyDeviceToDevice, stream));
     LA_HIP(hipMemsetAsync(h->m, 0, nw * sizeof(float), stream));
@@ -315,9 +356,9 @@
         h->adam_tab_valid = 1;
     }
     hipLaunchKernelGGL(la_set_int2_kernel, dim3(1), dim3(1), 0, stream, h->crop_dev, h->crop_y, h->crop_x);
-    const bool use_disc = c.w_disc != 0.f;
+    use_disc = c.w_disc != 0.f;
     LA_CHECK_ARG(!use_disc || h->d, "latent_opt_run: w_disc != 0 but no discriminator attached (la_latent_opt_set_disc)");
-    const bool use_lpips = c.w_lpips != 0.f;
+    use_lpips = c.w_lpips != 0.f;
     LA_CHECK_ARG(!use_lpips || h->f, "latent_opt_run: w_lpips != 0 but no feature engine attached (la_latent_opt_set_lpips)");
     if (use_disc && use_lpips && h->overlap && !h->side_stream) {
         LA_HIP(hipStreamCreateWithFlags(&h->side_stream, hipStreamNonBlocking));
@@ -325,9 +366,9 @@
         LA_HIP(hipEventCreateWithFlags(&h->ev_join, hipEventDisableTiming));
     }
     LA_CHECK_ARG(!use_lpips || (h->crop_x + h->S <= h->R && h->crop_y + h->S <= h->R), "latent_opt_run: LPIPS crop outside the image");
-    const bool img_crit = c.w_pix != 0.f || use_disc || use_lpips;
-    const float lp_coef = use_lpips ? c.w_lpips / ((float)h->imgc * (float)h->Mf * nb) : 0.f;
-    const bool want_losses = losses_out != nullptr;
+    img_crit = c.w_pix != 0.f || use_disc || use_lpips;
+    lp_coef = use_lpips ? c.w_lpips / ((float)h->imgc * (float)h->Mf * nb) : 0.f;
+    want_losses = losses_out != nullptr;
     if (!h->colsums_valid) {
         if ((rc = refresh_colsums(h, stream))) return rc;
         h->colsums_valid = 1;
@@ -342,120 +383,129 @@
     };
     const bool win_covers = (c.w_pix == 0.f || inside(off, off + cc, off, off + cc)) &&
                             (!use_lpips || inside(h->crop_y, h->crop_y + h->S, h->crop_x, h->crop_x + h->S));
-    const bool windowed = h->win_hi > 0 && !use_disc && !h->trace_img && win_covers;
-    struct WinGuard {
-        la_synth* g; ~WinGuard() { (void)la_synth_set_row_window(g, 0, 0); (void)la_synth_set_col_window(g, 0, 0); }
-    } win_guard{h->g};
+    windowed = h->win_hi > 0 && !use_disc && !h->trace_img && win_covers;
+    if ((rc = la_synth_set_launch_blocks(h->g, 0, 0))) return rc;
     if ((rc = la_synth_set_row_window(h->g, windowed ? h->win_lo : 0, windowed ? h->win_hi : 0))) return rc;
     if ((rc = la_synth_set_col_window(h->g, windowed ? h->wcol_lo : 0, windowed ? h->wcol_hi : 0))) return rc;
     if (want_losses && c.steps > 0) LA_HIP(hipMemsetAsync(h->losses, 0, (size_t)c.steps * 4 * sizeof(float), stream));
-    const float lat_coef = h->Mw ? c.w_latent / ((float)h->Mw * nb * (float)h->num_ws * (float)wd) : 0.f;
-    const float pix_coef = h->Mx ? c.w_pix / ((float)h->imgc * (float)h->Mx * nb * (float)cc2) : 0.f;
-
-    auto run_step = [&](float* L, hipStream_t st, int step_index = -1, int seg = 15) -> int {
-        int rc;
-        const bool segA = seg & 1, segP = seg & 2, segD = seg & 4, segZ = seg & 8;
-        hipEvent_t* tev = (h->time_trace && h->tev && L && step_index >= 0 && step_index < h->tev_steps) ? h->tev + (size_t)step_index * LA_TEV : nullptr;
-        auto mark = [&](int k) { if (tev) (void)hipEventRecord(tev[k], st); };
-        const float* img = la_synth_image(h->g);
-        if (segA) {
-            mark(0);
-            const long wb = h->wplus ? (long)h->num_ws * wd : wd, wl = h->wplus ? wd : 0;
-            if ((rc = la_synth_forward(h->g, h->w_opt, wb, wl, B, c.loop_noise_mode, nullptr, nullptr, st))) return rc;
-            img = la_synth_image(h->g);
-            mark(1);
-            if (L) {
-                if (h->Mw && (rc = la_l2_mean_from_bank(h->bankW, h->Mw, (long)h->num_ws * wd, h->w_opt, B, wb, h->wplus ? 0 : wd, h->yx,
-                                                        h->yy, h->xx, lat_coef, L + 0, 0, st)))
-                    return rc;
+    lat_coef = h->Mw ? c.w_latent / ((float)h->Mw * nb * (float)h->num_ws * (float)wd) : 0.f;
+    pix_coef = h->Mx ? c.w_pix / ((float)h->imgc * (float)h->Mx * nb * (float)cc2) : 0.f;
+    const bool tracing = h->trace_w || h->trace_img || h->trace_dw;
+    replay = h->graph_mode == 1 && !want_losses && !tracing && c.steps > 0 && !la_prof_enabled();
+    split = replay && h->overlap == 1 && use_disc && use_lpips && h->side_stream && h->ev_fork && h->ev_join;
+    first_graph_step = 1;
+    return LA_OK;
+}
+
+int LoopRun::run_step(float* L, hipStream_t st, int step_index, int seg, int part) {
+    int rc;
+    const la_opt_config& c = h->cfg;
+    const bool segA = seg & 1, segP = seg & 2, segD = seg & 4, segZ = seg & 8;
+    const bool lo_part = part == 1 || part == 3;
+    struct BlocksGuard { la_synth* g; ~BlocksGuard() { (void)la_synth_set_launch_blocks(g, 0, 0); } } blocks_guard{h->g};
+    if (part && (rc = lo_part ? la_synth_set_launch_blocks(h->g, 0, k_split) : la_synth_set_launch_blocks(h->g, k_split, nblocks))) return rc;
+    hipEvent_t* tev = (h->time_trace && h->tev && L && step_index >= 0 && step_index < h->tev_steps) ? h->tev + (size_t)step_index * LA_TEV : nullptr;
+    auto mark = [&](int k) { if (tev) (void)hipEventRecord(tev[k], st); };
+    const float* img = la_synth_image(h->g);
+    if (segA && part != 3) {
+        mark(0);
+        const long wb = h->wplus ? (long)h->num_ws * wd : wd, wl = h->wplus ? wd : 0;
+        if ((rc = la_synth_forward(h->g, h->w_opt, wb, wl, B, c.loop_noise_mode, nullptr, nullptr, st))) return rc;
+        if (part == 1) return LA_OK;
+        img = la_synth_image(h->g);
+        mark(1);
+        if (L) {
+            if (h->Mw && (rc = la_l2_mean_from_bank(h->bankW, h->Mw, (long)h->num_ws * wd, h->w_opt, B, wb, h->wplus ? 0 : wd, h->yx,
+                                                    h->yy, h->xx, lat_coef, L + 0, 0, st)))
+                return rc;
+        }
+        mark(2);
+        if (L) {
+            if (h->Mx) {
+                if ((rc = la_center_crop_f32(img, h->xc, (long)B * h->imgc, h->R, cc, off, st))) return rc;
+                for (int ch = 0; ch < h->imgc; ++ch)
+                    if ((rc = la_l2_mean_from_bank(h->bankX + (long)ch * h->Mx * cc2, h->Mx, cc2, h->xc + (long)ch * cc2, B,
+                                                   (long)h->imgc * cc2, 0, h->yx, h->yy, h->xx, pix_coef, L + 1, ch > 0, st)))
+                        return rc;
             }
-            mark(2);
-            if (L) {
-                if (h->Mx) {
-                    if ((rc = la_center_crop_f32(img, h->xc, (long)B * h->imgc, h->R, cc, off, st))) return rc;
+        }
+    }
+    const float* dws = nullptr;
+    if (img_crit) {
+        if (segA && part != 3) {
+            if (c.w_pix != 0.f &&
+                (rc = la_pix_grad(img, h->colsumX, h->g_img, B, h->imgc, h->R, cc, off, -2.f * pix_coef, (float)h->Mx, st)))
+                return rc;
+            mark(3);
+        }
+        const bool fork = seg == 15 && part == 0 && h->overlap == 2 && use_disc && use_lpips && !L && !tev && !la_prof_enabled() && h->side_stream && h->ev_fork && h->ev_join;
+        hipStream_t sl = fork ? h->side_stream : st;
+        if (fork) {
+            LA_HIP(hipEventRecord(h->ev_fork, st));
+            LA_HIP(hipStreamWaitEvent(h->side_stream, h->ev_fork, 0));
+        }
+        if (use_disc && segD && part != 3) {
+            if ((rc = la_disc_forward(h->d, img, B, st))) return rc;
+            if ((rc = la_disc_loss(h->d, c.w_disc, c.norm_batch, L ? L + 2 : nullptr, st))) return rc;
+            if ((rc = la_disc_backward(h->d, nullptr, h->g_img, c.w_pix != 0.f, st))) return rc;
+        }
+        if (segD) mark(4);
+        if (use_lpips && part != 3) {
+            const int N = h->imgc * B;
+            const long FF = h->F;
+            if (segP) {
+                if (c.w_pix == 0.f && !use_disc) LA_HIP(hipMemsetAsync(h->g_img, 0, sizeof(float) * (size_t)B * h->imgc * h->R * h->R, st));
+                if ((rc = la_crop_repeat(img, h->l_xc, B, h->imgc, h->R, h->S, h->crop_y, h->crop_x, h->crop_dev, 3, h->pre_scale, h->pre_shift, sl))) return rc;
+                if ((rc = la_feat_forward(h->f, h->l_xc, N, h->l_feat, sl))) return rc;
+                if (L) {
                     for (int ch = 0; ch < h->imgc; ++ch)
-                        if ((rc = la_l2_mean_from_bank(h->bankX + (long)ch * h->Mx * cc2, h->Mx, cc2, h->xc + (long)ch * cc2, B,
-                                                       (long)h->imgc * cc2, 0, h->yx, h->yy, h->xx, pix_coef, L + 1, ch > 0, st)))
+                        if ((rc = la_l2_mean_from_bank(h->bankF + (long)ch * h->Mf * FF, h->Mf, FF, h->l_feat + (long)ch * B * FF, B, FF, 0,
+                                                       h->l_yx, h->l_yy, h->l_xx, lp_coef, L + 3, ch > 0, st)))
                             return rc;
                 }
+                const long total = (long)N * FF;
+                hipLaunchKernelGGL(la_lpips_gfeat_kernel, dim3(la_cdiv(total, 256)), dim3(256), 0, sl, h->l_feat, h->l_colsum, h->l_gfeat,
+                                   B, (int)FF, -2.f * lp_coef, (float)h->Mf, total);
+                if ((rc = la_feat_backward(h->f, h->l_gfeat, h->l_gxc, sl))) return rc;
             }
-        }
-        const float* dws = nullptr;
-        if (img_crit) {
-            if (segA) {
-                if (c.w_pix != 0.f &&
-                    (rc = la_pix_grad(img, h->colsumX, h->g_img, B, h->imgc, h->R, cc, off, -2.f * pix_coef, (float)h->Mx, st)))
-                    return rc;
-                mark(3);
+            if (fork) {
+                LA_HIP(hipEventRecord(h->ev_join, h->side_stream));
+                LA_HIP(hipStreamWaitEvent(st, h->ev_join, 0));
             }
-            const bool fork = seg == 15 && h->overlap == 2 && use_disc && use_lpips && !L && !tev && !la_prof_enabled() && h->side_stream && h->ev_fork && h->ev_join;
-            hipStream_t sl = fork ? h->side_stream : st;
-            if (fork) {
-                LA_HIP(hipEventRecord(h->ev_fork, st));
-                LA_HIP(hipStreamWaitEvent(h->side_stream, h->ev_fork, 0));
-            }
-            if (use_disc && segD) {
-                if ((rc = la_disc_forward(h->d, img, B, st))) return rc;
-                if ((rc = la_disc_loss(h->d, c.w_disc, c.norm_batch, L ? L + 2 : nullptr, st))) return rc;
-                if ((rc = la_disc_backward(h->d, nullptr, h->g_img, c.w_pix != 0.f, st))) return rc;
-            }
-            if (segD) mark(4);
-            if (use_lpips) {
-                const int N = h->imgc * B;
-                const long FF = h->F;
-                if (segP) {
-                    if (c.w_pix == 0.f && !use_disc) LA_HIP(hipMemsetAsync(h->g_img, 0, sizeof(float) * (size_t)B * h->imgc * h->R * h->R, st));
-                    if ((rc = la_crop_repeat(img, h->l_xc, B, h->imgc, h->R, h->S, h->crop_y, h->crop_x, h->crop_dev, 3, h->pre_scale, h->pre_shift, sl))) return rc;
-                    if ((rc = la_feat_forward(h->f, h->l_xc, N, h->l_feat, sl))) return rc;
-                    if (L) {
-                        for (int ch = 0; ch < h->imgc; ++ch)
-                            if ((rc = la_l2_mean_from_bank(h->bankF + (long)ch * h->Mf * FF, h->Mf, FF, h->l_feat + (long)ch * B * FF, B, FF, 0,
-                                                           h->l_yx, h->l_yy, h->l_xx, lp_coef, L + 3, ch > 0, st)))
-                                return rc;
-                    }
-                    const long total = (long)N * FF;
-                    hipLaunchKernelGGL(la_lpips_gfeat_kernel, dim3(la_cdiv(total, 256)), dim3(256), 0, sl, h->l_feat, h->l_colsum, h->l_gfeat,
-                                       B, (int)FF, -2.f * lp_coef, (float)h->Mf, total);
-                    if ((rc = la_feat_backward(h->f, h->l_gfeat, h->l_gxc, sl))) return rc;
-                }
-                if (fork) {
-                    LA_HIP(hipEventRecord(h->ev_join, h->side_stream));
-                    LA_HIP(hipStreamWaitEvent(st, h->ev_join, 0));
-                }
-                if (segZ && (rc = la_crop_repeat_grad(h->l_gxc, h->g_img, B, h->imgc, h->R, h->S, h->crop_y, h->crop_x, h->crop_dev, 3, h->pre_scale, st)))
-                    return rc;
-            }
-            if (segZ) {
-                mark(5);
-                if ((rc = la_synth_backward(h->g, h->g_img, h->dws, st))) return rc;
-            }
-            dws = h->dws;
-        } else if (segZ) { mark(3); mark(4); mark(5); }
-        if (!segZ) return LA_OK;
-        if (h->wplus)
-            rc = la_wplus_step_tail(dws, h->Mw ? h->colsumW : nullptr, h->dw, h->w_opt, h->m, h->v, B, h->num_ws, wd, -2.f * lat_coef,
-                                    (float)h->Mw, c.lr, c.beta1, c.beta2, c.eps, h->adam_tab, h->step_ctr, h->step_ctr + 8, st);
-        else
-            rc = la_step_tail(dws, h->Mw ? h->colsumW : nullptr, h->dw, h->w_opt, h->m, h->v, B, h->num_ws, wd, -2.f * lat_coef, (float)h->Mw,
-                              c.lr, c.beta1, c.beta2, c.eps, h->adam_tab, h->step_ctr, h->step_ctr + 8, st);
-        mark(6);
-        return rc;
-    };
-
-    const bool tracing = h->trace_w || h->trace_img || h->trace_dw;
-    const bool replay = h->graph_mode == 1 && !want_losses && !tracing && c.steps > 0 && !la_prof_enabled();
-    int first_graph_step = 1;
-    const bool split = replay && h->overlap == 1 && use_disc && use_lpips && h->side_stream && h->ev_fork && h->ev_join;
-    auto capture = [&](int seg, hipGraph_t* g, hipGraphExec_t* e) -> bool {
-        bool ok = hipStreamBeginCapture(h->cap_stream, hipStreamCaptureModeRelaxed) == hipSuccess;
-        if (ok) {
-            const int rcs = run_step(nullptr, h->cap_stream, -1, seg);
-            const hipError_t er = hipStreamEndCapture(h->cap_stream, g);
-            ok = rcs == LA_OK && er == hipSuccess && *g;
-        }
-        if (ok) ok = hipGraphInstantiate(e, *g, nullptr, nullptr, 0) == hipSuccess;
-        return ok;
-    };
+            if (segZ && (rc = la_crop_repeat_grad(h->l_gxc, h->g_img, B, h->imgc, h->R, h->S, h->crop_y, h->crop_x, h->crop_dev, 3, h->pre_scale, st)))
+                return rc;
+        }
+        if (segZ) {
+            mark(5);
+            if ((rc = la_synth_backward(h->g, h->g_img, h->dws, st))) return rc;
+        }
+        dws = h->dws;
+    } else if (segZ) { mark(3); mark(4); mark(5); }
+    if (!segZ || part == 2) return LA_OK;
+    if (h->wplus)
+        rc = la_wplus_step_tail(dws, h->Mw ? h->colsumW : nullptr, h->dw, h->w_opt, h->m, h->v, B, h->num_ws, wd, -2.f * lat_coef,
+                                (float)h->Mw, c.lr, c.beta1, c.beta2, c.eps, h->adam_tab, h->step_ctr, h->step_ctr + 8, st);
+    else
+        rc = la_step_tail(dws, h->Mw ? h->colsumW : nullptr, h->dw, h->w_opt, h->m, h->v, B, h->num_ws, wd, -2.f * lat_coef, (float)h->Mw,
+                          c.lr, c.beta1, c.beta2, c.eps, h->adam_tab, h->step_ctr, h->step_ctr + 8, st);
+    mark(6);
+    return rc;
+}
+
+bool LoopRun::capture(int seg, int part, hipGraph_t* g, hipGraphExec_t* e) {
+    bool ok = hipStreamBeginCapture(h->cap_stream, hipStreamCaptureModeRelaxed) == hipSuccess;
+    if (ok) {
+        const int rcs = run_step(nullptr, h->cap_stream, -1, seg, part);
+        const hipError_t er = hipStreamEndCapture(h->cap_stream, g);
+        ok = rcs == LA_OK && er == hipSuccess && *g;
+    }
+    if (ok) ok = hipGraphInstantiate(e, *g, nullptr, nullptr, 0) == hipSuccess;
+    return ok;
+}
+
+int LoopRun::prepare(bool want_parts) {
+    int rc;
+    const la_opt_config& c = h->cfg;
     const bool have = split ? (h->seg_valid != 0) : (h->graph_exec != nullptr);
     if (replay && (!have || h->graph_B != B || h->graph_win != (int)windowed)) {
         drop_graph(h);
@@ -464,32 +514,53 @@
         bool ok = c.steps >= 2;
         if (ok && !h->cap_stream) ok = hipStreamCreateWithFlags(&h->cap_stream, hipStreamNonBlocking) == hipSuccess;
         if (ok && split) {
-            for (int k = 0; k < 4 && ok; ++k) ok = capture(1 << k, &h->seg_graph[k], &h->seg_exec[k]);
+            for (int k = 0; k < 4 && ok; ++k) ok = capture(1 << k, 0, &h->seg_graph[k], &h->seg_exec[k]);
             if (ok) h->seg_valid = 1;
-        } else if (ok) ok = capture(15, &h->graph, &h->graph_exec);
+        } else if (ok) ok = capture(15, 0, &h->graph, &h->graph_exec);
         if (ok) { h->graph_B = B; h->graph_win = (int)windowed; }
         else { drop_graph(h); (void)hipGetLastError(); if (c.steps >= 2) { h->graph_mode = 0; h->graph_refused = 1; } }
     }
-    for (int step = first_graph_step; step <= c.steps; ++step) {
-        if (replay && split && h->seg_valid && h->graph_B == B) {
-            LA_HIP(hipGraphLaunch(h->seg_exec[0], stream));
-            LA_HIP(hipEventRecord(h->ev_fork, stream));
-            LA_HIP(hipStreamWaitEvent(h->side_stream, h->ev_fork, 0));
-            LA_HIP(hipGraphLaunch(h->seg_exec[1], h->side_stream));
-            LA_HIP(hipEventRecord(h->ev_join, h->side_stream));
-            LA_HIP(hipGraphLaunch(h->seg_exec[2], stream));
-            LA_HIP(hipStreamWaitEvent(stream, h->ev_join, 0));
-            LA_HIP(hipGraphLaunch(h->seg_exec[3], stream));
-        } else if (replay && !split && h->graph_exec && h->graph_B == B) LA_HIP(hipGraphLaunch(h->graph_exec, stream));
+    if (want_parts && replay && !split && h->graph_exec && h->graph_B == B && !h->part_valid && k_split > 0 && k_split < nblocks) {
+        bool ok = true;
+        for (int k = 0; k < 3 && ok; ++k) ok = capture(15, k + 1, &h->part_graph[k], &h->part_exec[k]);
+        if (ok) h->part_valid = 1;
         else {
-            if ((rc = run_step(want_losses ? h->losses + (size_t)(step - 1) * 4 : nullptr, stream, step - 1))) return rc;
-            if (h->trace_img)
-                LA_HIP(hipMemcpyAsync(h->trace_img + (size_t)(step - 1) * B * h->imgc * h->R * h->R, la_synth_image(h->g),
-                                      sizeof(float) * (size_t)B * h->imgc * h->R * h->R, hipMemcpyDeviceToDevice, stream));
-            if (h->trace_w) LA_HIP(hipMemcpyAsync(h->trace_w + (size_t)(step - 1) * nw, h->w_opt, sizeof(float) * nw, hipMemcpyDeviceToDevice, stream));
-            if (h->trace_dw) LA_HIP(hipMemcpyAsync(h->trace_dw + (size_t)(step - 1) * nw, h->dw, sizeof(float) * nw, hipMemcpyDeviceToDevice, stream));
-        }
-    }
+            for (int k = 0; k < 3; ++k) {
+                if (h->part_exec[k]) { (void)hipGraphExecDestroy(h->part_exec[k]); h->part_exec[k] = nullptr; }
+                if (h->part_graph[k]) { (void)hipGraphDestroy(h->part_graph[k]); h->part_graph[k] = nullptr; }
+            }
+            (void)hipGetLastError();
+        }
+    }
+    return LA_OK;
+}
+
+int LoopRun::enqueue_step(int step) {
+    int rc;
+    if (replay && split && h->seg_valid && h->graph_B == B) {
+        LA_HIP(hipGraphLaunch(h->seg_exec[0], stream));
+        LA_HIP(hipEventRecord(h->ev_fork, stream));
+        LA_HIP(hipStreamWaitEvent(h->side_stream, h->ev_fork, 0));
+        LA_HIP(hipGraphLaunch(h->seg_exec[1], h->side_stream));
+        LA_HIP(hipEventRecord(h->ev_join, h->side_stream));
+        LA_HIP(hipGraphLaunch(h->seg_exec[2], stream));
+        LA_HIP(hipStreamWaitEvent(stream, h->ev_join, 0));
+        LA_HIP(hipGraphLaunch(h->seg_exec[3], stream));
+    } else if (replay && !split && h->graph_exec && h->graph_B == B) LA_HIP(hipGraphLaunch(h->graph_exec, stream));
+    else {
+        if ((rc = run_step(want_losses ? h->losses + (size_t)(step - 1) * 4 : nullptr, stream, step - 1))) return rc;
+        if (h->trace_img)
+            LA_HIP(hipMemcpyAsync(h->trace_img + (size_t)(step - 1) * B * h->imgc * h->R * h->R, la_synth_image(h->g),
+                                  sizeof(float) * (size_t)B * h->imgc * h->R * h->R, hipMemcpyDeviceToDevice, stream));
+        if (h->trace_w) LA_HIP(hipMemcpyAsync(h->trace_w + (size_t)(step - 1) * nw, h->w_opt, sizeof(float) * nw, hipMemcpyDeviceToDevice, stream));
+        if (h->trace_dw) LA_HIP(hipMemcpyAsync(h->trace_dw + (size_t)(step - 1) * nw, h->dw, sizeof(float) * nw, hipMemcpyDeviceToDevice, stream));
+    }
+    return LA_OK;
+}
+
+int LoopRun::finish() {
+    int rc;
+    const la_opt_config& c = h->cfg;
     if ((rc = h->wplus ? la_wplus_gate(h->w_opt, w0, w_aug_out, B, h->num_ws, wd, c.alpha, c.soft_aug, stream)
                        : la_broadcast_mix(h->w_opt, w0, w_aug_out, B, h->num_ws, wd, c.alpha, c.soft_aug, stream)))
         return rc;
@@ -500,3 +571,76 @@
         LA_HIP(hipMemcpyAsync(losses_out, h->losses, (size_t)c.steps * 4 * sizeof(float), hipMemcpyDeviceToDevice, stream));
     return LA_OK;
 }
+
+extern "C" int la_latent_opt_run(la_latent_opt* h, const float* w0, int B, const float* const* final_noises,
+                                 float* img_out, float* w_aug_out, float* losses_out, hipStream_t stream) {
+    LoopRun r;
+    int rc;
+    if ((rc = r.begin(h, w0, B, final_noises, img_out, w_aug_out, losses_out, stream))) return rc;
+    if ((rc = r.prepare(false))) return rc;
+    for (int step = r.first_graph_step; step <= h->cfg.steps; ++step)
+        if ((rc = r.enqueue_step(step))) return rc;
+    return r.finish();
+}
+
+extern "C" int la_latent_opt_run_pair(la_latent_opt* ha, la_latent_opt* hb, const float* w0_a, const float* w0_b, int B,
+                                      const float* const* final_noises_a, const float* const* final_noises_b, float* img_out_a,
+                                      float* img_out_b, float* w_aug_out_a, float* w_aug_out_b, float* losses_out_a, float* losses_out_b,
+                                      hipStream_t stream_a, hipStream_t stream_b, int schedule) {
+    LA_CHECK_ARG(ha && hb && ha != hb && ha->g != hb->g, "latent_opt_run_pair: two different handles with synthesis engines of their own");
+    LA_CHECK_ARG(schedule == 0 || schedule == 1, "latent_opt_run_pair: schedule must be 0 (free) or 1 (alternate)");
+    int rc;
+    auto lane_plain = [](const la_latent_opt* h, const float* losses) {
+        const bool both = h->cfg.w_disc != 0.f && h->cfg.w_lpips != 0.f;
+        return !losses && !h->trace_w && !h->trace_img && !h->trace_dw && h->graph_mode == 1 && h->cfg.steps >= 2 && !(both && h->overlap);
+    };
+    const int ks = la_synth_split_block(ha->g), nbk = la_synth_num_blocks(ha->g);
+    const bool alternate = schedule == 1 && stream_a != stream_b && !la_prof_enabled() && lane_plain(ha, losses_out_a) && lane_plain(hb, losses_out_b) &&
+                           ha->cfg.steps == hb->cfg.steps && ks > 0 && ks < nbk && la_synth_split_block(hb->g) == ks && la_synth_num_blocks(hb->g) == nbk;
+    if (!alternate) {
+        if ((rc = la_latent_opt_run(ha, w0_a, B, final_noises_a, img_out_a, w_aug_out_a, losses_out_a, stream_a))) return rc;
+        return la_latent_opt_run(hb, w0_b, B, final_noises_b, img_out_b, w_aug_out_b, losses_out_b, stream_b);
+    }
+    const int steps = ha->cfg.steps;
+    la_latent_opt* hs[2] = {ha, hb};
+    for (la_latent_opt* h : hs) {
+        if (h->pair_ev) continue;
+        h->pair_ev = (hipEvent_t*)calloc((size_t)steps, sizeof(hipEvent_t));
+        LA_CHECK_ARG(h->pair_ev, "latent_opt_run_pair: out of host memory");
+        for (h->pair_nev = 0; h->pair_nev < steps; ++h->pair_nev) LA_HIP(hipEventCreateWithFlags(&h->pair_ev[h->pair_nev], hipEventDisableTiming));
+    }
+    LoopRun ra, rb;
+    if ((rc = ra.begin(ha, w0_a, B, final_noises_a, img_out_a, w_aug_out_a, losses_out_a, stream_a))) return rc;
+    if ((rc = rb.begin(hb, w0_b, B, final_noises_b, img_out_b, w_aug_out_b, losses_out_b, stream_b))) return rc;
+    if ((rc = ra.prepare(true)) || (rc = rb.prepare(true))) return rc;
+    if (ra.parts_ready() && rb.parts_ready() && ha->pair_nev == steps && hb->pair_nev == steps) {
+        int last_b = -1;
+        const int first = ra.first_graph_step < rb.first_graph_step ? ra.first_graph_step : rb.first_graph_step;
+        for (int step = first; step <= steps; ++step) {
+            if (step >= ra.first_graph_step) {
+                LA_HIP(hipGraphLaunch(ha->part_exec[0], stream_a));
+                if (last_b >= 0) LA_HIP(hipStreamWaitEvent(stream_a, hb->pair_ev[last_b], 0));
+                LA_HIP(hipGraphLaunch(ha->part_exec[1], stream_a));
+                LA_HIP(hipEventRecord(ha->pair_ev[step - 1], stream_a));
+                LA_HIP(hipGraphLaunch(ha->part_exec[2], stream_a));
+            }
+            if (step >= rb.first_graph_step) {
+                LA_HIP(hipGraphLaunch(hb->part_exec[0], stream_b));
+                if (step >= ra.first_graph_step) LA_HIP(hipStreamWaitEvent(stream_b, ha->pair_ev[step - 1], 0));
+                LA_HIP(hipGraphLaunch(hb->part_exec[1], stream_b));
+                LA_HIP(hipEventRecord(hb->pair_ev[step - 1], stream_b));
+                LA_HIP(hipGraphLaunch(hb->part_exec[2], stream_b));
+                last_b = step - 1;
+            }
+        }
+    } else {
+        for (int step = ra.first_graph_step; step <= steps; ++step)
+            if ((rc = ra.enqueue_step(step))) return rc;
+        for (int step = rb.first_graph_step; step <= steps; ++step)
+            if ((rc = rb.enqueue_step(step))) return rc;
+    }
+    if ((rc = ra.finish())) return rc;
+    return rb.finish();
+}
+
+extern "C" int la_latent_opt_parts_state(const la_latent_opt* h) { return (h && h->part_valid) ? 1 : 0; }
diff --git a/latentaugment_amd/csrc/la_synth.hip b/latentaugment_amd/csrc/la_synth.hip
--- a/latentaugment_amd/csrc/la_synth.hip
+++ b/latentaugment_amd/csrc/la_synth.hip
@@ -61,6 +61,7 @@
     int wcol_lo, wcol_hi;
     int fw_c0, fw_c1;
     int fw_lo[2 * MAX_BLOCKS], fw_hi[2 * MAX_BLOCKS];
+    int lb_lo, lb_hi;
 };
 
 static LaLayerEpi layer_epi(const la_synth* h, const ConvLayer& L) {
@@ -301,6 +302,19 @@
     return LA_OK;
 }
 
+extern "C" int la_synth_set_launch_blocks(la_synth* h, int k_lo, int k_hi) {
+    LA_CHECK_ARG(h && k_lo >= 0 && (k_hi == 0 ? k_lo == 0 : (k_hi > k_lo && k_hi <= h->nblocks)), "synth_set_launch_blocks: bad block range");
+    h->lb_lo = k_lo; h->lb_hi = k_hi;
+    return LA_OK;
+}
+extern "C" int la_synth_num_blocks(const la_synth* h) { return h ? h->nblocks : 0; }
+extern "C" int la_synth_split_block(const la_synth* h) {
+    if (!h) return 0;
+    for (int k = 0; k < h->nblocks; ++k)
+        if ((long)(4 << k) * (4 << k) > la_conv_splitk_max_points()) return k;
+    return h->nblocks;
+}
+
 #ifdef LA_DEV
 extern "C" const float* la_synth_dev_zt(const la_synth* h) { return h ? h->zT : nullptr; }
 #endif
@@ -318,12 +332,14 @@
     LA_CHECK_ARG(noise_mode >= 0 && noise_mode <= 2, "synth_forward: noise_mode must be 0 (none), 1 (const), 2 (explicit)");
     LA_CHECK_ARG(noise_mode != 2 || noises, "synth_forward: explicit noise requested but no noise tensors given");
     int rc;
-    if ((rc = la_affine_forward(h->st, ws, ws_bstride, ws_lstride, B, h->wdim, h->s_all, stream))) return rc;
-    if ((rc = la_demod_forward(h->dt, h->s_all, h->S, B, h->d_all, stream))) return rc;
+    const int lb_lo = h->lb_hi > 0 ? h->lb_lo : 0, lb_hi = h->lb_hi > 0 ? h->lb_hi : h->nblocks;
+    auto on = [&](int k) { return k >= lb_lo && k < lb_hi; };
+    if (on(0) && (rc = la_affine_forward(h->st, ws, ws_bstride, ws_lstride, B, h->wdim, h->s_all, stream))) return rc;
+    if (on(0) && (rc = la_demod_forward(h->dt, h->s_all, h->S, B, h->d_all, stream))) return rc;
     h->lastB = B;
     const bool f16 = h->precision == LA_PREC_F16X2;
     static const bool zt_dense = la_dev_env("LA_NO_ZT_PITCH") != nullptr;
-    if (f16 && (rc = la_xscale_from_bounds(h->dt, h->s_all, h->S, h->cst, h->channels[0] * 16, h->xs_fwd, h->xs_mult, B, stream, h->xs_bwd))) return rc;
+    if (f16 && on(0) && (rc = la_xscale_from_bounds(h->dt, h->s_all, h->S, h->cst, h->channels[0] * 16, h->xs_fwd, h->xs_mult, B, stream, h->xs_bwd))) return rc;
     auto fwd_row = [&](int conv_index) { return (f16 && conv_index < h->nconv) ? h->xs_fwd + (long)conv_index * B * LA_XS_FAN : nullptr; };
     auto fwd_mult = [&](int conv_index) { return (f16 && conv_index < h->nconv) ? h->xs_mult + (long)conv_index * B : nullptr; };
     int wlo[2 * MAX_BLOCKS], whi[2 * MAX_BLOCKS], ilo[MAX_BLOCKS], ihi[MAX_BLOCKS];
@@ -372,7 +388,7 @@
         const float* skip = nullptr;
         if (k > 0 && fuse_rgb) {
             RgbLayer& P = h->rgb[k - 1];
-            if ((rc = la_upfirdn2d_ex(P.img, T.g_img, B, h->imgc, res / 2, res / 2, h->fir, la_fir_up2(), stream)))
+            if (on(k) && (rc = la_upfirdn2d_ex(P.img, T.g_img, B, h->imgc, res / 2, res / 2, h->fir, la_fir_up2(), stream)))
                 return rc;
             skip = T.g_img;
         }
@@ -387,7 +403,8 @@
             LaModconvFwdOpts o;
             o.xscale = fwd_row(ci); o.xs_out = fwd_row(ci + 1); o.xs_mult = fwd_mult(ci + 1);
             o.win.row_lo = wlo[ci]; o.win.row_hi = whi[ci];
-            if (!L.up) {
+            if (!on(k)) rc = LA_OK;
+            else if (!L.up) {
                 if (fuse_rgb && q == nl - 1) o.rgb = &rf;
                 if (ci == h->nconv - 1) { o.win.col_lo = c1lo; o.win.col_hi = c1hi; }
                 rc = la_modconv3x3_fwd_ex(x, x_bstride, layer_conv(h, L, B, false), layer_epi(h, L), L.y, stream, o);
@@ -399,7 +416,7 @@
             if (rc) return rc;
             x = L.y; x_bstride = (long)L.cout * res * res;
         }
-        if (!fuse_rgb) {
+        if (!fuse_rgb && on(k)) {
             const float* skip_lo = k > 0 ? h->rgb[k - 1].img : nullptr;
             const bool iw = ihi[k] > 0 && (long)res * res > 4096;
             if ((rc = la_torgb_forward(x, layer_rgb(h, T, nullptr, rgb_dst), B, T.cin, res, res, stream, nullptr, iw ? ilo[k] : 0, iw ? ihi[k] : 0,
@@ -416,6 +433,8 @@
     LA_CHECK_ARG(h->lastB >= 1, "synth_backward: no forward pass to differentiate");
     const int B = h->lastB;
     int rc;
+    const int lb_lo = h->lb_hi > 0 ? h->lb_lo : 0, lb_hi = h->lb_hi > 0 ? h->lb_hi : h->nblocks;
+    auto on = [&](int k) { return k >= lb_lo && k < lb_hi; };
     const float* gi = g_img;
     int ci = h->nconv - 1;
     const float* gx_next = nullptr;
@@ -467,7 +486,7 @@
             if (xs_hand) { s.xs_out = xs_slot(ci); s.xs_mult = 1.f; }
             else if (f16) s.pmax_out = h->pmax;
             if (win) { s.p_lo = (long)rw1.in.row_lo * res; s.p_hi = (long)rw1.in.row_hi * res; }
-            if ((rc = la_seam_backward(s, B, h->imgc, stream))) return rc;
+            if (on(k) && (rc = la_seam_backward(s, B, h->imgc, stream))) return rc;
         }
         {
             LaStyleFinish::Rgb& r = fin.rgb[fin.nrgb++];
@@ -488,7 +507,7 @@
             LaModconvBwdOpts o;
             o.in_pmax = f16 ? (seam2_done ? h->pmax3 : h->pmax) : nullptr; o.in_nseg = nseg1;
             o.seam = fuse_seam ? &sf : nullptr; o.xscale = xs_slot(ci); o.rows = win ? &rw1 : nullptr;
-            if ((rc = la_modconv3x3_bwd_ex(h->G0, layer_conv(h, L1, B, true), xin, xin_bs, h->G1, L1.dsp, stream, o))) return rc;
+            if (on(k) && (rc = la_modconv3x3_bwd_ex(h->G0, layer_conv(h, L1, B, true), xin, xin_bs, h->G1, L1.dsp, stream, o))) return rc;
             fin_conv(L1, tiles1, nseg1);
         }
         --ci;
@@ -501,15 +520,15 @@
             s.ddn_part = L0.ddnp;
             if (xs_hand) { s.xs_out = xs_slot(ci); s.xs_mult = up_mult; }
             else if (f16) s.pmax_out = h->pmax;
-            if ((rc = la_seam_backward(s, B, 0, stream))) return rc;
+            if (on(k) && (rc = la_seam_backward(s, B, 0, stream))) return rc;
         }
         RgbLayer& P = h->rgb[k - 1];
         if (!pyramid_done) {
-            if ((rc = la_upfirdn2d_ex(gi, P.g_img, B, h->imgc, res, res, h->fir, la_fir_down2_adjoint(), stream))) return rc;
+            if (on(k) && (rc = la_upfirdn2d_ex(gi, P.g_img, B, h->imgc, res, res, h->fir, la_fir_down2_adjoint(), stream))) return rc;
             if (k >= 2 && res / 2 <= 256) {
                 float* outs[MAX_BLOCKS];
                 for (int q = k - 2; q >= 0; --q) outs[k - 2 - q] = h->rgb[q].g_img;
-                if ((rc = la_image_grad_pyramid(P.g_img, outs, k - 1, B * h->imgc, res / 2, h->fir, stream))) return rc;
+                if (on(k) && (rc = la_image_grad_pyramid(P.g_img, outs, k - 1, B * h->imgc, res / 2, h->fir, stream))) return rc;
                 pyramid_done = true;
             }
         }
@@ -531,7 +550,7 @@
             LaModconvBwdOpts o;
             o.in_pmax = f16 ? (fuse_seam ? h->pmax2 : h->pmax) : nullptr; o.in_nseg = nseg0;
             o.seam = fuse_seam2 ? &sf2 : nullptr; o.xscale = xs_slot(ci); o.rows = win ? &rw0 : nullptr;
-            if ((rc = la_modconv3x3_up2_bwd_ex(h->G1, layer_conv(h, L0, B, true), h->conv[ci - 1].y, (long)L0.cin * hin * hin, h->fir, h->zT, h->G0, L0.dsp,
+            if (on(k) && (rc = la_modconv3x3_up2_bwd_ex(h->G1, layer_conv(h, L0, B, true), h->conv[ci - 1].y, (long)L0.cin * hin * hin, h->fir, h->zT, h->G0, L0.dsp,
                                                stream, o)))
                 return rc;
             fin_conv(L0, tiles, nseg0);
@@ -541,6 +560,7 @@
         gi = P.g_img;
         seam2_done = fuse_seam2;
     }
+    if (!on(0)) return LA_OK;
     if ((rc = la_style_backward_all(fin, B, stream))) return rc;
     return la_affine_backward(h->st, h->ds_all, B, h->wdim, dws, h->num_ws, h->aff_part, stream);
 }
diff --git a/latentaugment_amd/latent_aug.py b/latentaugment_amd/latent_aug.py
--- a/latentaugment_amd/latent_aug.py
+++ b/latentaugment_amd/latent_aug.py
@@ -134,6 +134,7 @@
 
 
 LATENT_SPACES = {'w': 0, 'w+': 1}
+LANE_SCHEDULE_DEFAULT = 'free'
 
 
 class LatentAug:
@@ -275,6 +276,8 @@
         self._opt, self._discriminator, self._feature_net = opt, discriminator, feature_net
         self.stream_lanes = getattr(opt, 'stream_lanes', 'auto')
         assert self.stream_lanes in ('auto', 1, 2), "opt.stream_lanes: 'auto', 1 or 2"
+        self.lane_schedule = getattr(opt, 'lane_schedule', LANE_SCHEDULE_DEFAULT)
+        assert self.lane_schedule in ('alternate', 'free'), "opt.lane_schedule: 'alternate' or 'free'"
         self._lanes = None
         self._lane_stream = None
         self.lanes_active = False
@@ -482,9 +485,19 @@
         side = self._lane_stream if concurrent else main
         if concurrent:
             side.wait_stream(main)
-        self._lanes[0].run_local(parts[0], fns[0], crop_pos=crop_pos, out=outs[0])
-        with torch.cuda.stream(side):
-            self._lanes[1].run_local(parts[1], fns[1], crop_pos=crop_pos, out=outs[1])
+        ptrs = []
+        for k in (0, 1):
+            lane = self._lanes[k]
+            if lane.feat is not None:
+                ax, ay = lane.crop_window(crop_pos)
+                _lib.check(self._lib.la_latent_opt_set_crop_pos(lane._h, ax, ay), 'la_latent_opt_set_crop_pos')
+            ptrs.append(lane.engine.noise_pointer_array(fns[k]) if self._cfg.final_noise_mode == 2 else None)
+            lane._keep = fns[k]
+        with torch.cuda.device(self.device):
+            _lib.check(self._lib.la_latent_opt_run_pair(
+                self._lanes[0]._h, self._lanes[1]._h, _lib.ptr(parts[0]), _lib.ptr(parts[1]), b // 2, ptrs[0], ptrs[1],
+                _lib.ptr(outs[0][0]), _lib.ptr(outs[1][0]), _lib.ptr(outs[0][1]), _lib.ptr(outs[1][1]), None, None,
+                C.c_void_p(main.cuda_stream), C.c_void_p(side.cuda_stream), int(self.lane_schedule == 'alternate')), 'la_latent_opt_run_pair')
         if concurrent:
             main.wait_stream(side)
         img = torch.empty([b, self.engine.img_channels, self.res, self.res], device=self.device, dtype=torch.float32)
diff --git a/latentaugment_amd/synthesis.py b/latentaugment_amd/synthesis.py
--- a/latentaugment_amd/synthesis.py
+++ b/latentaugment_amd/synthesis.py
@@ -207,6 +207,17 @@
     def style_grads(self, batch):
         rows = self._lib.la_synth_style_rows(self._h)
         return self._view(self._lib.la_synth_style_grads(self._h), [batch, rows])
+
+    def block_image(self, k, batch):
+        r = self.block_resolutions[k]
+        return self._view(self._lib.la_synth_block_image(self._h, k), [batch, self.img_channels, r, r])
+
+    def set_launch_blocks(self, k_lo=0, k_hi=0):
+        _lib.check(self._lib.la_synth_set_launch_blocks(self._h, int(k_lo), int(k_hi)), 'la_synth_set_launch_blocks')
+
+    @property
+    def split_block(self):
+        return self._lib.la_synth_split_block(self._h)
 
 
 class _SynthesisFn(torch.autograd.Function):
```
